# OpenRL-Lab/openrl

Hardware: AMD Instinct MI355X
Metric: env-steps/sec (collect+PPO update), 4096-env CartPole-shape (higher is better)
Workload: dtype f32

## Files before the change

include/orl_hip.h:

```cpp
#ifndef ORL_HIP_H
#define ORL_HIP_H

#include <stdint.h>

#ifdef __cplusplus
extern "C" {
#endif

#define ORL_VERSION 306

#define ORL_E_INVALID (-1)
#define ORL_E_UNSUPPORTED (-2)

#define ORL_HEAD_VALUE 0
#define ORL_HEAD_CATEGORICAL 1
#define ORL_HEAD_GAUSSIAN 2

typedef struct orl_net_desc {
  int32_t obs_dim;
  int32_t hidden;
  int32_t n_out;
  int32_t head_kind;
} orl_net_desc;

// ... 50 lines not shown
                          const uint8_t* bad_transition, const float* next_action_masks, float* h_policy_next,
                          float* h_critic_next, int hidden, void* stream);

#define ORL_COPY_MAX 8
typedef struct orl_copy_desc {
  const float* src[ORL_COPY_MAX];
  float* dst[ORL_COPY_MAX];
  int64_t n[ORL_COPY_MAX];
  int32_t count;
} orl_copy_desc;
int orl_multi_copy(const orl_copy_desc* desc, void* stream);

#define ORL_GATHER_MAX 12
typedef struct orl_gather_desc {
  const float* src[ORL_GATHER_MAX];
  float* dst[ORL_GATHER_MAX];
  int32_t width[ORL_GATHER_MAX];
  int32_t count;
} orl_gather_desc;
int orl_gather_minibatch(const orl_gather_desc* desc, const int64_t* idx, int n_rows, void* stream);

int orl_perm_feistel(int64_t* idx, int64_t n, uint64_t seed, uint64_t stream_id, void* stream);
int orl_perm_feistel_vn(int64_t* idx, int64_t n, uint64_t seed, uint64_t stream_id, float* vn_state,
                        const double* moments, double beta, void* stream);

int orl_act_step(const orl_net_desc* pnet, const float* ptheta, const orl_net_desc* cnet,
                 const float* ctheta, const float* policy_obs, const float* critic_obs,
                 const float* action_masks, int B, int deterministic, uint64_t seed, uint64_t row0,
                 uint64_t rng_step, const uint64_t* rng_step_dev, const float* forced_u, float* values,
                 float* actions, float* logp, void* stream);
int orl_act_step_grouped(const orl_net_desc* pnet, const float* pthetas, int64_t theta_stride, int rows_per_group,
                         const float* policy_obs, const float* action_masks, int B, int deterministic, uint64_t seed,
                         uint64_t row0, uint64_t rng_step, const uint64_t* rng_step_dev, float* actions, float* logp,
                         void* stream);

int orl_act_step_pool(const orl_net_desc* pnet, const float* pthetas, int64_t theta_stride, int n_policies,
                      const int32_t* opp_index, const float* policy_obs, const float* action_masks, int B,
                      int deterministic, uint64_t seed, uint64_t row0, uint64_t rng_step, const uint64_t* rng_step_dev,
                      float* actions, float* logp, void* stream);
int orl_opponent_sample(int32_t* opp_index, const uint8_t* dones, int N, int n_filled, int last_slot, int strategy,
                        int per_tile, uint64_t seed, uint64_t draw_id, const uint64_t* draw_id_dev, void* stream);


int orl_evaluate_actions(const orl_net_desc* pnet, const float* ptheta, const orl_net_desc* cnet,
                         const float* ctheta, const float* policy_obs, const float* critic_obs,
                         const float* actions, const float* action_masks, const float* active_masks, int B,
                         float* values, float* action_log_probs, float* entropy_rows, float* dist_entropy,
                         void* stream);

typedef struct orl_ppo_hparams {
  float clip_param;
  float entropy_coef;
  float value_loss_coef;
  float huber_delta;
  float dual_clip_coeff;
  float max_grad_norm;
  int32_t use_clipped_value_loss;
  int32_t use_huber_loss;
  int32_t use_value_active_masks;
  int32_t use_policy_active_masks;
  int32_t use_valuenorm;
  int32_t dual_clip_ppo;
  int32_t use_max_grad_norm;
  int32_t reserved;
} orl_ppo_hparams;

int orl_raw_grad_count(const orl_net_desc* net);
#define ORL_N_STATS 16
int orl_ppo_max_blocks(void);

int orl_ppo_fwd_bwd(const orl_net_desc* pnet, const float* ptheta, const orl_net_desc* cnet,
                    const float* ctheta, const float* records, int rec_width, const int64_t* idx,
                    int mb, const float* vn_state, const orl_ppo_hparams* hp, float* partials,
                    int* n_blocks_out, void* stream);

typedef struct orl_adam_state {
  float* theta;
  float* grad;
  float* m;
  float* v;
  float lr, eps, weight_decay;
  int32_t step;
} orl_adam_state;

int orl_ppo_reduce(const float* partials, int n_blocks, int width, float* sums, void* stream);
int orl_ppo_reduce_pair(const float* partials, int n_blocks_policy, int width_policy, int n_blocks_critic,
                        int width_critic, float* sums, void* stream);
int orl_ppo_apply(const orl_net_desc* pnet, const orl_net_desc* cnet, const float* sums,
                  const orl_ppo_hparams* hp, const orl_adam_state* padam, const orl_adam_state* cadam,
                  float* train_info_accum, void* stream);
int orl_ppo_apply_perm(const orl_net_desc* pnet, const orl_net_desc* cnet, const float* sums,
                       const orl_ppo_hparams* hp, const orl_adam_state* padam, const orl_adam_state* cadam,
                       float* train_info_accum, int64_t* next_idx, int64_t n, uint64_t seed, uint64_t stream_id,
                       float* vn_state, const double* moments, double beta, void* stream);

typedef struct orl_comm orl_comm;
#define ORL_IPC_HANDLE_BYTES 64
int orl_comm_create(int rank, int world, int64_t capacity_floats, orl_comm** comm_out, unsigned char* handle_out);
int orl_comm_connect(orl_comm* comm, const unsigned char* all_handles);
int orl_comm_destroy(orl_comm* comm);
int orl_comm_error(orl_comm* comm, void* stream);
int orl_comm_error_copy(orl_comm* comm, int* err_out_dev, void* stream);
int orl_allreduce_small(orl_comm* comm, float* data, int n, void* stream);
int orl_ppo_reduce_pair_comm(orl_comm* comm, const float* partials, int n_blocks_policy, int width_policy,
                             int n_blocks_critic, int width_critic, float* sums, void* stream);
int orl_ppo_apply_comm(orl_comm* comm, const orl_net_desc* pnet, const orl_net_desc* cnet, float* sums,
                       const orl_ppo_hparams* hp, const orl_adam_state* padam, const orl_adam_state* cadam,
                       float* train_info_accum, int64_t* next_idx, int64_t n, uint64_t seed, uint64_t stream_id,
                       float* vn_state, const double* moments, double beta, void* stream);

int orl_ppo_reduce_apply(orl_comm* comm, const float* partials, int n_blocks_policy, int width_policy,
                         int n_blocks_critic, int width_critic, float* sums, const orl_net_desc* pnet,
                         const orl_net_desc* cnet, const orl_ppo_hparams* hp, const orl_adam_state* padam,
                         const orl_adam_state* cadam, float* train_info_accum, int64_t* next_idx, int64_t n, uint64_t seed,
                         uint64_t stream_id, float* vn_state, const double* moments, double beta, uint32_t* sync_ctr,
                         void* stream);

int orl_ppo_step(orl_comm* comm, const float* partials, int n_blocks_policy, int width_policy, int n_blocks_critic,
                 int width_critic, float* sums, const orl_net_desc* pnet, const orl_net_desc* cnet,
                 const orl_ppo_hparams* hp, const orl_adam_state* padam, const orl_adam_state* cadam,
                 float* train_info_accum, int64_t* next_idx, int64_t n, uint64_t seed, uint64_t stream_id, float* vn_state,
                 const double* moments, double beta, uint32_t* sync_ctr, void* stream);

int orl_valuenorm_update(float* vn_state, const double* moments, double beta, void* stream);
int orl_minibatch_moments(const float* records, int rec_width, int ret_col, const int64_t* idx, int mb,
                          double* scratch, double* moments, void* stream);

#define ORL_ENV_SYNTH 0
#define ORL_ENV_CARTPOLE 1
#define ORL_ENV_TTT 2
#define ORL_ENV_TTT_POOL 3
#define ORL_ENV_PENDULUM 5
#define ORL_ENV_ACROBOT 6
#define ORL_ENV_MOUNTAINCAR 7
#define ORL_ENV_MOUNTAINCAR_CONT 8

typedef struct orl_rollout_args {
  orl_buffer_ptrs buf;
  float* value_preds;
  float* actions;
  float* action_log_probs;
  float* env_state;
  float* ep_stats;
  int32_t env_kind;
  int32_t episode_limit;
  uint64_t env_seed;
  uint64_t act_seed;
  uint64_t rng_step0;
  const float* opp_thetas;
  int64_t opp_theta_stride;
  int32_t opp_group_rows;
  int32_t opp_reserved;
  uint64_t opp_seed;
  uint64_t opp_rng_step0;
  const int32_t* opp_index;
  int32_t opp_per_reset;
  int32_t opp_n_policies;
  int32_t opp_n_filled;
  int32_t opp_last_slot;
  int32_t opp_strategy;
  int32_t opp_pad;
  uint64_t opp_sample_seed;
  uint64_t opp_draw_id0;
} orl_rollout_args;

int orl_build_experiments(void);
// ... 221 lines not shown
```

openrl_amd/_native.py:

```python
from __future__ import annotations

import ctypes as C
import os
from typing import Optional

import torch

_HERE = os.path.dirname(os.path.abspath(__file__))
LIB_PATH = os.path.join(_HERE, "csrc", "liborl_hip.so")

ORL_HEAD_VALUE, ORL_HEAD_CATEGORICAL, ORL_HEAD_GAUSSIAN = 0, 1, 2
ORL_ENV_SYNTH, ORL_ENV_CARTPOLE, ORL_ENV_TTT, ORL_ENV_TTT_POOL, ORL_ENV_MPE_SPREAD = 0, 1, 2, 3, 4
ORL_ENV_PENDULUM = 5
ORL_ENV_ACROBOT, ORL_ENV_MOUNTAINCAR = 6, 7
ORL_ENV_MOUNTAINCAR_CONT = 8
ORL_GATHER_MAX = 12
ORL_IPC_HANDLE_BYTES = 64
ORL_VERSION = 306
ORL_N_STATS = 16

c_f32p = C.c_void_p


class NativeError(RuntimeError):
    pass


class NetDesc(C.Structure):
    _fields_ = [("obs_dim", C.c_int32), ("hidden", C.c_int32), ("n_out", C.c_int32), ("head_kind", C.c_int32)]


class PackSrc(C.Structure):
    _fields_ = [("policy_obs", C.c_void_p), ("critic_obs", C.c_void_p), ("actions", C.c_void_p),
                ("action_log_probs", C.c_void_p), ("value_preds", C.c_void_p), ("returns", C.c_void_p),
                ("active_masks", C.c_void_p), ("action_masks", C.c_void_p),
                ("Dp", C.c_int32), ("Dc", C.c_int32), ("a", C.c_int32), ("K", C.c_int32)]


class BufferPtrs(C.Structure):
    _fields_ = [("policy_obs", C.c_void_p), ("critic_obs", C.c_void_p), ("rewards", C.c_void_p),
                ("masks", C.c_void_p), ("bad_masks", C.c_void_p), ("active_masks", C.c_void_p),
                ("action_masks", C.c_void_p),
                ("T", C.c_int32), ("N", C.c_int32), ("A", C.c_int32), ("Dp", C.c_int32), ("Dc", C.c_int32),
                ("K", C.c_int32)]


class CopyDesc(C.Structure):
    _fields_ = [("src", C.c_void_p * 8), ("dst", C.c_void_p * 8), ("n", C.c_int64 * 8), ("count", C.c_int32)]


class GatherDesc(C.Structure):
    _fields_ = [("src", C.c_void_p * ORL_GATHER_MAX), ("dst", C.c_void_p * ORL_GATHER_MAX),
                ("width", C.c_int32 * ORL_GATHER_MAX), ("count", C.c_int32)]


class PPOHParams(C.Structure):
    _fields_ = [("clip_param", C.c_float), ("entropy_coef", C.c_float), ("value_loss_coef", C.c_float),
                ("huber_delta", C.c_float), ("dual_clip_coeff", C.c_float), ("max_grad_norm", C.c_float),
                ("use_clipped_value_loss", C.c_int32), ("use_huber_loss", C.c_int32),
                ("use_value_active_masks", C.c_int32), ("use_policy_active_masks", C.c_int32),
                ("use_valuenorm", C.c_int32), ("dual_clip_ppo", C.c_int32), ("use_max_grad_norm", C.c_int32),
                ("reserved", C.c_int32)]


class AdamState(C.Structure):
    _fields_ = [("theta", C.c_void_p), ("grad", C.c_void_p), ("m", C.c_void_p), ("v", C.c_void_p),
                ("lr", C.c_float), ("eps", C.c_float), ("weight_decay", C.c_float), ("step", C.c_int32)]


class RolloutArgs(C.Structure):
    _fields_ = [("buf", BufferPtrs), ("value_preds", C.c_void_p), ("actions", C.c_void_p),
                ("action_log_probs", C.c_void_p), ("env_state", C.c_void_p), ("ep_stats", C.c_void_p),
                ("env_kind", C.c_int32), ("episode_limit", C.c_int32), ("env_seed", C.c_uint64),
                ("act_seed", C.c_uint64), ("rng_step0", C.c_uint64), ("opp_thetas", C.c_void_p),
                ("opp_theta_stride", C.c_int64), ("opp_group_rows", C.c_int32), ("opp_reserved", C.c_int32),
                ("opp_seed", C.c_uint64), ("opp_rng_step0", C.c_uint64), ("opp_index", C.c_void_p),
                ("opp_per_reset", C.c_int32), ("opp_n_policies", C.c_int32), ("opp_n_filled", C.c_int32),
                ("opp_last_slot", C.c_int32), ("opp_strategy", C.c_int32), ("opp_pad", C.c_int32),
                ("opp_sample_seed", C.c_uint64), ("opp_draw_id0", C.c_uint64)]


class RnnBatch(C.Structure):
    _fields_ = [("records", C.c_void_p), ("rows", C.c_void_p), ("masks", C.c_void_p), ("h_policy", C.c_void_p),
                ("h_critic", C.c_void_p), ("rec_width", C.c_int32), ("n_chunks", C.c_int32), ("L", C.c_int32),
                ("n_chunks_critic", C.c_int32), ("rows_critic", C.c_void_p)]


class RnnRolloutArgs(C.Structure):
    _fields_ = [("buf", BufferPtrs), ("value_preds", C.c_void_p), ("actions", C.c_void_p),
                ("action_log_probs", C.c_void_p), ("rnn_states", C.c_void_p), ("rnn_states_critic", C.c_void_p),
                ("env_state", C.c_void_p), ("ep_stats", C.c_void_p), ("obs_policy_out", C.c_void_p),
                ("obs_critic_out", C.c_void_p), ("next_value", C.c_void_p), ("env_kind", C.c_int32),
                ("world_length", C.c_int32), ("deterministic", C.c_int32), ("reserved", C.c_int32),
                ("env_seed", C.c_uint64), ("act_seed", C.c_uint64), ("rng_step0", C.c_uint64),
                ("rng_step_dev", C.c_void_p), ("sync_flags", C.c_void_p), ("env_step0", C.c_uint64)]


class HeadDesc(C.Structure):
    _fields_ = [("kind", C.c_int32), ("n_out", C.c_int32), ("n_heads", C.c_int32), ("nvec", C.c_int32 * 8)]


ORL_GEN_MLP_MAX_LAYERS = 14


class GenMlpLayer(C.Structure):
    _fields_ = [("W", C.c_void_p), ("bias", C.c_void_p), ("gamma", C.c_void_p), ("beta", C.c_void_p),
                ("n_in", C.c_int32), ("n_out", C.c_int32), ("act", C.c_int32), ("reserved", C.c_int32)]


class GenMlpDesc(C.Structure):
    _fields_ = [("n_layers", C.c_int32), ("n_heads", C.c_int32), ("fn_gamma", C.c_void_p), ("fn_beta", C.c_void_p),
                ("layer", GenMlpLayer * ORL_GEN_MLP_MAX_LAYERS)]


ORL_GT_MAX_LAYERS = 4


class GtDesc(C.Structure):
    _fields_ = [("theta", C.c_void_p), ("D", C.c_int32), ("H", C.c_int32), ("n_layers", C.c_int32), ("n_heads", C.c_int32),
                ("o_fn_g", C.c_int32), ("o_fn_be", C.c_int32),
                ("oW", C.c_int32 * ORL_GT_MAX_LAYERS), ("ob", C.c_int32 * ORL_GT_MAX_LAYERS),
                ("og", C.c_int32 * ORL_GT_MAX_LAYERS), ("obe", C.c_int32 * ORL_GT_MAX_LAYERS),
                ("act", C.c_int32 * ORL_GT_MAX_LAYERS),
                ("head_oW", C.c_int32 * 2), ("head_ob", C.c_int32 * 2), ("head_n", C.c_int32 * 2)]


class GtLoss(C.Structure):
    _fields_ = [("head", HeadDesc), ("logstd", C.c_void_p), ("den", C.c_void_p), ("vn_state", C.c_void_p),
                ("hp", PPOHParams), ("Dp", C.c_int32), ("Dc", C.c_int32), ("a_w", C.c_int32), ("K", C.c_int32),
                ("policy_head", C.c_int32), ("value_head", C.c_int32), ("policy_grad", C.c_int32), ("reserved", C.c_int32)]


ORL_ACT_NONE, ORL_ACT_TANH, ORL_ACT_RELU, ORL_ACT_LEAKY_RELU, ORL_ACT_ELU = -1, 0, 1, 2, 3
ORL_HEAD_MULTI_DISCRETE = 3
ORL_HEAD_MIXED = 4

_ABI_STRUCTS = (NetDesc, PackSrc, BufferPtrs, CopyDesc, GatherDesc, PPOHParams, AdamState, RolloutArgs, RnnBatch,
                RnnRolloutArgs, GenMlpDesc, GtDesc, GtLoss)

_P = C.c_void_p
_SIGNATURES = {
    "orl_version": (C.c_int, []),
    "orl_build_experiments": (C.c_int, []),
    "orl_tower_split_terms": (C.c_int, []),
    "orl_abi_struct_size": (C.c_int, [C.c_int]),
    "orl_last_error_string": (C.c_char_p, []),
    "orl_param_count": (C.c_int, [C.POINTER(NetDesc)]),
    "orl_raw_grad_count": (C.c_int, [C.POINTER(NetDesc)]),
    "orl_gae_scan": (C.c_int, [_P, _P, _P, _P, _P, _P, _P, C.c_int, C.c_int, C.c_double, C.c_double, C.c_int,
                               _P, _P, _P, C.POINTER(C.c_int), _P]),
    "orl_gae_max_partials": (C.c_int, [C.c_int, C.c_int]),
    "orl_adv_stats": (C.c_int, [_P, _P, _P, _P, C.c_int, C.c_int, _P, _P, C.POINTER(C.c_int), _P]),
    "orl_record_width": (C.c_int, [C.c_int, C.c_int, C.c_int, C.c_int]),
    "orl_adv_normalize_pack": (C.c_int, [_P, _P, C.c_int, C.c_int, C.c_int, C.c_int, _P, C.POINTER(PackSrc), _P, _P]),
    "orl_buffer_insert": (C.c_int, [C.POINTER(BufferPtrs), C.c_int, _P, _P, _P, _P, _P, _P, _P]),
    "orl_buffer_insert_rnn": (C.c_int, [C.POINTER(BufferPtrs), C.c_int, _P, _P, _P, _P, _P, _P, _P, _P, C.c_int, _P]),
    "orl_multi_copy": (C.c_int, [C.POINTER(CopyDesc), _P]),
    "orl_gather_minibatch": (C.c_int, [C.POINTER(GatherDesc), _P, C.c_int, _P]),
    "orl_perm_feistel": (C.c_int, [_P, C.c_int64, C.c_uint64, C.c_uint64, _P]),
    "orl_perm_feistel_vn": (C.c_int, [_P, C.c_int64, C.c_uint64, C.c_uint64, _P, _P, C.c_double, _P]),
    "orl_act_step": (C.c_int, [C.POINTER(NetDesc), _P, C.POINTER(NetDesc), _P, _P, _P, _P, C.c_int, C.c_int,
                               C.c_uint64, C.c_uint64, C.c_uint64, _P, _P, _P, _P, _P, _P]),
    "orl_ttt_state_width": (C.c_int, []),
    "orl_ttt_reset": (C.c_int, [_P, _P, _P, _P, C.c_int, C.c_uint64, _P]),
    "orl_ttt_step": (C.c_int, [_P, _P, _P, _P, _P, _P, _P, C.c_int, C.c_uint64, _P]),
    "orl_ttt_agent_move": (C.c_int, [_P, _P, _P, _P, _P, _P, C.c_int, _P]),
    "orl_ttt_opponent_move": (C.c_int, [_P, _P, _P, _P, _P, _P, _P, C.c_int, C.c_uint64, _P]),
    "orl_critic_values": (C.c_int, [C.POINTER(NetDesc), _P, _P, C.c_int64, _P, _P]),
    "orl_act_step_grouped": (C.c_int, [C.POINTER(NetDesc), _P, C.c_int64, C.c_int, _P, _P, C.c_int, C.c_int, C.c_uint64,
                                       C.c_uint64, C.c_uint64, _P, _P, _P, _P]),
    "orl_act_step_pool": (C.c_int, [C.POINTER(NetDesc), _P, C.c_int64, C.c_int, _P, _P, _P, C.c_int, C.c_int, C.c_uint64,
                                    C.c_uint64, C.c_uint64, _P, _P, _P, _P]),
    "orl_opponent_sample": (C.c_int, [_P, _P, C.c_int, C.c_int, C.c_int, C.c_int, C.c_int, C.c_uint64, C.c_uint64, _P,
                                      _P]),
    "orl_evaluate_actions": (C.c_int, [C.POINTER(NetDesc), _P, C.POINTER(NetDesc), _P, _P, _P, _P, _P, _P, C.c_int, _P,
                                       _P, _P, _P, _P]),
    "orl_ppo_max_blocks": (C.c_int, []),
    "orl_ppo_fwd_bwd": (C.c_int, [C.POINTER(NetDesc), _P, C.POINTER(NetDesc), _P, _P, C.c_int, _P, C.c_int, _P,
                                  C.POINTER(PPOHParams), _P, C.POINTER(C.c_int), _P]),
    "orl_ppo_reduce": (C.c_int, [_P, C.c_int, C.c_int, _P, _P]),
    "orl_ppo_reduce_pair": (C.c_int, [_P, C.c_int, C.c_int, C.c_int, C.c_int, _P, _P]),
    "orl_ppo_apply": (C.c_int, [C.POINTER(NetDesc), C.POINTER(NetDesc), _P, C.POINTER(PPOHParams),
                                C.POINTER(AdamState), C.POINTER(AdamState), _P, _P]),
    "orl_ppo_apply_perm": (C.c_int, [C.POINTER(NetDesc), C.POINTER(NetDesc), _P, C.POINTER(PPOHParams),
                                     C.POINTER(AdamState), C.POINTER(AdamState), _P, _P, C.c_int64, C.c_uint64,
                                     C.c_uint64, _P, _P, C.c_double, _P]),
    "orl_comm_create": (C.c_int, [C.c_int, C.c_int, C.c_int64, C.POINTER(_P), _P]),
    "orl_comm_connect": (C.c_int, [_P, _P]),
    "orl_comm_destroy": (C.c_int, [_P]),
    "orl_comm_error": (C.c_int, [_P, _P]),
    "orl_comm_error_copy": (C.c_int, [_P, _P, _P]),
    "orl_allreduce_small": (C.c_int, [_P, _P, C.c_int, _P]),
    "orl_ppo_reduce_pair_comm": (C.c_int, [_P, _P, C.c_int, C.c_int, C.c_int, C.c_int, _P, _P]),
    "orl_ppo_apply_comm": (C.c_int, [_P, C.POINTER(NetDesc), C.POINTER(NetDesc), _P, C.POINTER(PPOHParams),
                                     C.POINTER(AdamState), C.POINTER(AdamState), _P, _P, C.c_int64, C.c_uint64,
                                     C.c_uint64, _P, _P, C.c_double, _P]),
    "orl_ppo_reduce_apply": (C.c_int, [_P, _P, C.c_int, C.c_int, C.c_int, C.c_int, _P, C.POINTER(NetDesc),
                                       C.POINTER(NetDesc), C.POINTER(PPOHParams), C.POINTER(AdamState),
                                       C.POINTER(AdamState), _P, _P, C.c_int64, C.c_uint64, C.c_uint64, _P, _P, C.c_double,
                                       _P, _P]),
    "orl_ppo_step": (C.c_int, [_P, _P, C.c_int, C.c_int, C.c_int, C.c_int, _P, C.POINTER(NetDesc),
                               C.POINTER(NetDesc), C.POINTER(PPOHParams), C.POINTER(AdamState),
                               C.POINTER(AdamState), _P, _P, C.c_int64, C.c_uint64, C.c_uint64, _P, _P, C.c_double,
                               _P, _P]),
    "orl_gen_rollout_fused": (C.c_int, [_P, _P, _P, _P, _P, _P, _P, _P, _P, C.c_int, C.c_int, C.c_uint64, C.c_uint64,
                                        C.c_uint64, C.c_uint64, C.c_int, _P]),
    "orl_gemm": (C.c_int, [_P, C.c_int64, C.c_int64, _P, C.c_int64, C.c_int64, _P, C.c_int64, C.c_int, C.c_int, C.c_int,
                           C.c_int, _P, _P]),
    "orl_row_fwd": (C.c_int, [_P, _P, C.c_int, _P, _P, C.c_int, C.c_int, _P, _P, _P, _P, _P]),
    "orl_row_bwd": (C.c_int, [_P, _P, _P, _P, _P, C.c_int, C.c_int, C.c_int, _P, _P, C.c_int, C.POINTER(C.c_int), _P]),
    "orl_gen_layer_fwd": (C.c_int, [_P, C.c_int, C.c_int, _P, _P, C.c_int, _P, _P, C.c_int, _P, _P, _P, _P]),
    "orl_gt_supported": (C.c_int, [C.POINTER(GtDesc)]),
    "orl_gt_image_floats": (C.c_int64, [C.POINTER(GtDesc)]),
    "orl_gt_raw_floats": (C.c_int64, [C.POINTER(GtDesc)]),
    "orl_gt_prep": (C.c_int, [C.POINTER(GtDesc), _P, _P]),
    "orl_gt_fwd": (C.c_int, [C.POINTER(GtDesc), _P, _P, C.c_int, C.c_int, _P, C.c_int, _P, _P, _P]),
    "orl_gt_bwd": (C.c_int, [C.POINTER(GtDesc), _P, _P, C.c_int, C.c_int, _P, C.c_int, _P, _P, _P, C.c_int64, _P, _P, _P]),
    "orl_gt_train": (C.c_int, [C.POINTER(GtDesc), _P, _P, C.c_int, C.c_int, _P, C.c_int, C.POINTER(GtLoss), _P, C.c_int64, _P, _P,
                               _P, _P]),
    "orl_gen_mlp_fwd": (C.c_int, [C.POINTER(GenMlpDesc), _P, C.c_int, _P, _P, _P, _P]),
    "orl_gen_act": (C.c_int, [C.POINTER(GenMlpDesc), _P, C.POINTER(GenMlpDesc), _P, C.c_int, _P, _P, C.POINTER(HeadDesc), _P,
                              _P, C.c_int, C.c_uint64, C.c_uint64, C.c_uint64, _P, _P, C.c_int, _P, _P, _P]),
    "orl_gen_layer_bwd": (C.c_int, [_P, _P, _P, _P, C.c_int, C.c_int, C.c_int, _P, C.c_int, _P, _P, _P, C.c_int,
                                    C.POINTER(C.c_int), _P]),
    "orl_gen_wgrad": (C.c_int, [_P, _P, C.c_int, C.c_int, C.c_int, _P, _P, C.c_int64, _P]),
    "orl_gen_colsum": (C.c_int, [_P, C.c_int, C.c_int, _P, C.c_int, _P, C.c_int, _P, C.c_int, _P]),
    "orl_gather_cols": (C.c_int, [_P, C.c_int, C.c_int, C.c_int, _P, C.c_int, _P, _P]),
    "orl_gen_denoms": (C.c_int, [_P, C.c_int, C.c_int, C.c_int, C.c_int, _P, C.c_int, _P, _P, _P]),
    "orl_gen_policy_loss": (C.c_int, [C.POINTER(HeadDesc), _P, _P, _P, C.c_int, C.c_int, C.c_int, C.c_int, C.c_int, _P,
                                      C.c_int, _P, C.POINTER(PPOHParams), _P, _P, C.c_int, C.POINTER(C.c_int), _P, _P,
                                      _P]),
    "orl_gen_value_loss": (C.c_int, [_P, _P, C.c_int, C.c_int, C.c_int, C.c_int, C.c_int, _P, C.c_int, _P, _P,
                                     C.POINTER(PPOHParams), _P, _P, C.c_int, C.POINTER(C.c_int), _P]),
    "orl_gen_sample": (C.c_int, [C.POINTER(HeadDesc), _P, _P, _P, C.c_int, C.c_int, C.c_uint64, C.c_uint64, C.c_uint64,
                                 _P, _P, C.c_int, _P, _P, _P]),
    "orl_gen_adam": (C.c_int, [C.POINTER(AdamState), C.c_int64, C.c_float, C.c_int, C.c_int, _P, _P, C.c_int, C.c_int,
                               _P]),
    "orl_gen_matmul": (C.c_int, [_P, C.c_int, C.c_int, _P, C.c_int, _P, _P]),
    "orl_gen_colsum_rows": (C.c_int, [_P, C.c_int, C.c_int, _P, _P, C.c_int64, _P]),
    "orl_gen_gru_gate_fwd": (C.c_int, [_P, _P, _P, _P, C.c_int, C.c_int, _P, _P, _P, _P]),
    "orl_gen_gru_gate_bwd": (C.c_int, [_P, _P, _P, C.c_int, C.c_int, _P, _P, _P, _P]),
    "orl_gen_lstm_gate_fwd": (C.c_int, [_P, _P, _P, _P, C.c_int, C.c_int, _P, _P, _P, _P, _P, _P]),
    "orl_gen_lstm_gate_bwd": (C.c_int, [_P, _P, _P, _P, C.c_int, C.c_int, _P, _P, _P]),
    "orl_gen_row_affine": (C.c_int, [_P, _P, _P, _P, C.c_int, C.c_int, _P, _P]),
    "orl_vec_add": (C.c_int, [_P, _P, C.c_int64, _P]),
    "orl_gen_info": (C.c_int, [_P, _P, _P, C.POINTER(PPOHParams), C.c_float, C.c_float, _P, _P]),
    "orl_valuenorm_update": (C.c_int, [_P, _P, C.c_double, _P]),
    "orl_minibatch_moments": (C.c_int, [_P, C.c_int, C.c_int, _P, C.c_int, _P, _P, _P]),
    "orl_env_state_width": (C.c_int, [C.c_int]),
    "orl_env_reset": (C.c_int, [C.c_int, _P, _P, _P, C.c_int, C.c_int, C.c_uint64, C.c_int, _P]),
    "orl_env_step": (C.c_int, [C.c_int, _P, _P, _P, C.c_int, _P, _P, _P, C.c_int, C.c_int, C.c_uint64, C.c_int,
                               C.c_uint64, _P]),
    "orl_env_step_dev": (C.c_int, [C.c_int, _P, _P, _P, C.c_int, _P, _P, _P, C.c_int, C.c_int, C.c_uint64, C.c_int,
                                   C.c_uint64, _P, _P]),
    "orl_rollout_fused": (C.c_int, [C.POINTER(NetDesc), _P, C.POINTER(NetDesc), _P, C.POINTER(RolloutArgs), _P, _P]),
    "orl_mpe_state_width": (C.c_int, []),
    "orl_mpe_reset": (C.c_int, [_P, _P, _P, _P, C.c_int, C.c_uint64, _P]),
    "orl_mpe_step": (C.c_int, [_P, _P, _P, _P, _P, _P, _P, C.c_int, C.c_uint64, C.c_int, _P]),
    "orl_rnn_param_count": (C.c_int, [C.POINTER(NetDesc)]),
    "orl_rnn_raw_grad_count": (C.c_int, [C.POINTER(NetDesc)]),
    "orl_rnn_act_step": (C.c_int, [C.POINTER(NetDesc), _P, C.POINTER(NetDesc), _P, _P, _P, _P, _P, _P, _P, C.c_int,
                                   C.c_int, C.c_uint64, C.c_uint64, C.c_uint64, _P, _P, _P, _P, _P, _P, _P, _P]),
    "orl_rnn_eval_step": (C.c_int, [C.POINTER(NetDesc), _P, C.POINTER(NetDesc), _P, _P, _P, _P, _P, _P, _P, _P, C.c_int, _P,
                                    _P, _P, _P, _P, _P]),
    "orl_rnn_rollout_fused": (C.c_int, [C.POINTER(NetDesc), _P, C.POINTER(NetDesc), _P, C.POINTER(RnnRolloutArgs), _P]),
    "orl_rnn_chunk_rows": (C.c_int, [_P, C.c_int, C.c_int, C.c_int, C.c_int, _P, _P]),
    "orl_rnn_chunk_rows_v3": (C.c_int, [_P, C.c_int, C.c_int, C.c_int, C.c_int, C.c_int, C.c_int, _P, _P]),
    "orl_rnn_jrpo_records": (C.c_int, [_P, _P, C.c_int, C.c_int, C.c_int, C.c_int, _P, C.c_int, C.c_int, C.c_int, _P, _P]),
    "orl_rnn_workspace_floats": (C.c_int64, [C.POINTER(NetDesc), C.POINTER(NetDesc), C.c_int, C.c_int]),
# ... 117 lines not shown
```

openrl_amd/algorithms/ppo.py:

```python
from __future__ import annotations

from typing import Dict, Union

import numpy as np
import torch

from .. import _native as nat
from .. import distributed as dist_utils
from .. import ops, ops_rnn
from .base_algorithm import BaseAlgorithm

INFO_KEYS = ("value_loss", "policy_loss", "dist_entropy", "actor_grad_norm", "critic_grad_norm", "ratio")


class DeviceTrainInfo(dict):

    def __init__(self, keys, device_values: torch.Tensor, after_sync=None, scale=None):
        super().__init__()
        self._keys, self._dev, self._after_sync, self._scale = tuple(keys), device_values, after_sync, scale

    def _materialize(self) -> None:
        if self._dev is not None:
            raw, self._dev = self._dev.cpu().numpy(), None
            if self._scale is not None:
# ... 11 lines not shown

    def __iter__(self):
        self._materialize()
        return super().__iter__()

    def __len__(self):
        self._materialize()
        return super().__len__()

    def __contains__(self, k):
        self._materialize()
        return super().__contains__(k)

    def __repr__(self):
        self._materialize()
        return super().__repr__()

    def __eq__(self, other):
        self._materialize()
        return super().__eq__(other)

    def get(self, k, default=None):
        self._materialize()
        return super().get(k, default)

    def keys(self):
        self._materialize()
        return super().keys()

    def values(self):
        self._materialize()
        return super().values()

    def items(self):
        self._materialize()
        return super().items()

    def copy(self):
        self._materialize()
        return dict(self)

    def pop(self, *a):
        self._materialize()
        return super().pop(*a)

    def update(self, *a, **k):
        self._materialize()
        return super().update(*a, **k)

    def __setitem__(self, k, v):
        self._materialize()
        super().__setitem__(k, v)

    def __delitem__(self, k):
        self._materialize()
        super().__delitem__(k)


class PPOAlgorithm(BaseAlgorithm):
    info_keys = INFO_KEYS

    def __init__(self, cfg, init_module, agent_num: int = 1, device: Union[str, torch.device] = "cuda:0") -> None:
        if cfg.use_deepspeed or cfg.use_amp:
            raise NotImplementedError("deepspeed / amp are not built in this engine")
        if cfg.use_joint_action_loss and not cfg.use_recurrent_policy:
            raise NotImplementedError("use_joint_action_loss is built for recurrent policies (recurrent_generator_v3, "
                                      "the only generator the reference pairs it with, ppo.py:363-372)")
        super().__init__(cfg, init_module, agent_num, device)
        self.naive_recurrent = bool(cfg.use_naive_recurrent_policy) and not bool(cfg.use_recurrent_policy)
        self.train_list = [self.train_ppo]
        self.hp = ops.make_hparams(cfg, recurrent=bool(getattr(self.algo_module, "recurrent", False)))
        self.generic = bool(getattr(self.algo_module, "generic", False))
        self.use_joint_action_loss = bool(cfg.use_joint_action_loss)
        self.perm_mode = getattr(cfg, "amd_perm_mode", "reference")
        self._perm_counter = 0
        self._vn_in_perm = False
        self.last_indices = None
        self._info = torch.zeros(8, dtype=torch.float32, device=self.device)
        self._moments = torch.zeros(3, dtype=torch.float64, device=self.device)
        self._mom_scratch = torch.zeros(512, dtype=torch.float64, device=self.device)
        self._adv_stats = torch.zeros(11, dtype=torch.float64, device=self.device)
        self._moments_mb = self._moments
        self._full_batch_moments = False
        if self.generic:
            self.recurrent = bool(getattr(self.algo_module, "recurrent", False))
            self._rnn_rows = None
            self.fuse_next_perm = False
            self._comm = None
            self._gen_den4 = torch.zeros(4, dtype=torch.float32, device=self.device)
            self._gen_den = self._gen_den4[:2]
            self._gen_den_c = self._gen_den4[2:]
            self._gen_den_scratch = torch.zeros(257, dtype=torch.float32, device=self.device)
            self._gen_scratch = torch.zeros(256, dtype=torch.float32, device=self.device)
            self._gen_flat = self._gen_sums = None
            self._gen_den_stamp = None
            self._comm_watch = None
            if self.world_size > 1:
                nets = [m for m in self.algo_module.models.values()]
                n = sum(int(m.n_params) for m in nets) + 40
                self._gen_flat = torch.zeros(n, dtype=torch.float32, device=self.device)
                o = 0
                for m in nets:
                    m.grad = self._gen_flat[o:o + int(m.n_params)]
                    o += int(m.n_params)
                self._gen_sums = (self._gen_flat[o:o + 20], self._gen_flat[o + 20:o + 40])
                self._comm = dist_utils.make_small_allreduce(n, self.device, getattr(cfg, "amd_collective", "p2p")) \
                    if n <= self.P2P_MAX_FLOATS else None
                if self._comm is not None:
                    self._comm_watch = nat.DeviceErrorWatch("orl_comm: a peer's contribution did not arrive within 10 s - "
                                                            "the optimiser step ran on a partial gradient sum")
            return
        p, c = self.algo_module.models["policy"], self.algo_module.models["critic"]
        self.recurrent = bool(getattr(self.algo_module, "recurrent", False))
        raw = ops_rnn.rnn_raw_grad_count if self.recurrent else ops.raw_grad_count
        self._raw_p = raw(p.net) + ops.N_STATS
        self._raw_c = raw(c.net) + ops.N_STATS
        mb = ops.ppo_max_blocks()
        dev = self.device
        self._partials = None if self.recurrent else torch.empty(mb * (self._raw_p + self._raw_c), dtype=torch.float32,
                                                                 device=dev)
        self._rnn_ws = None
        self._rnn_rows = None
        self._rnn_scratch = torch.zeros(512, dtype=torch.float32, device=dev) if self.recurrent else None
        self._sums = torch.zeros(self._raw_p + self._raw_c, dtype=torch.float32, device=dev)
        self._optim_step = str(getattr(cfg, "amd_optim_step", "two_launch"))
        self._fused_step = self._optim_step in ("fused", "step")
        self._sync_ctr = torch.zeros(4, dtype=torch.int32, device=dev)
        self._comm = dist_utils.make_small_allreduce(self._sums.numel(), dev, getattr(cfg, "amd_collective", "p2p")) \
            if self.world_size > 1 else None
        self.fuse_next_perm = True
        self._comm_watch = nat.DeviceErrorWatch("orl_comm: a peer's contribution did not arrive within 10 s - the "
                                                "optimiser step ran on a partial gradient sum") \
            if self._comm is not None else None

    P2P_MAX_FLOATS = 1 << 16

    def _allreduce_vec(self, t: torch.Tensor) -> torch.Tensor:
        if self.world_size > 1:
            if self._comm is not None and t.dtype == torch.float32 and t.numel() <= self._comm.capacity:
                self._comm.allreduce_(t)
            else:
                dist_utils.allreduce_(t)
        return t

    def _advantages_and_records(self, buffer) -> None:
        T, N, A = buffer.episode_length, buffer.n_rollout_threads, buffer.num_agents
        L = N * A
        vn = self.algo_module.get_critic_value_normalizer() if (self._use_popart or self._use_valuenorm) else None
        vn_state = vn.state if vn is not None else None
        if not (buffer._adv_fresh and (getattr(buffer, "_adv_vn", None) is vn_state)):
            buffer.n_partials = ops.adv_stats(buffer.returns, buffer.value_preds, buffer.active_masks, vn_state, T, L,
                                              buffer.advantages, buffer.stat_partials)
        partials, n_part = buffer.stat_partials, buffer.n_partials
        if self.world_size > 1:
            row = dist_utils.allreduce_stat_rows(partials[:n_part])
            partials, n_part = row, 1
        ops.adv_normalize_pack(buffer.advantages, partials, n_part, T, L, self._use_adv_normalize, self._adv_stats,
                               buffer.pack_src(), buffer.ensure_records())
        buffer._adv_fresh = False

    def _update_minibatch(self, buffer, idx, mb: int, turn_on: bool, next_perm=None):
        if self.generic:
            from .ppo_generic import update_minibatch_generic

            return update_minibatch_generic(self, buffer, idx, mb, turn_on)
        mod = self.algo_module
        p, c = mod.models["policy"], mod.models["critic"]
        po, co = mod.optimizers["policy"], mod.optimizers["critic"]
        rec = buffer.records
        vn = mod.get_critic_value_normalizer() if self._use_valuenorm else None
        vn_state = None
        if vn is not None:
            if self._full_batch_moments:
                pass
            else:
                ret_col = buffer.Dp + buffer.Dc + 2 * buffer.act_shape + 2
                ops.minibatch_moments(rec, ret_col, idx, mb, self._mom_scratch, self._moments)
                if self.world_size > 1:
                    dist_utils.allreduce_(self._moments)
            if self._vn_in_perm:
                self._vn_in_perm = False
            else:
                ops.valuenorm_update(vn.state, self._moments, vn.beta)
            vn_state = vn.state
        ev = getattr(self, "profile_events", None)
        if ev is not None:
            e0, e1 = torch.cuda.Event(enable_timing=True), torch.cuda.Event(enable_timing=True)
            e0.record()
        nb_p, nb_c = ops.ppo_fwd_bwd(p.net, p.theta, c.net, c.theta, rec, idx, mb, vn_state, self.hp, self._partials)
        if ev is not None:
            e1.record()
            ev.append((e0, e1))
        comm = self._comm
        fused = self._fused_step and (self.world_size == 1 or comm is not None)
        if not fused:
            ops.ppo_reduce_pair(self._partials, nb_p, self._raw_p, nb_c, self._raw_c, self._sums, comm=comm)
            if self.world_size > 1 and comm is None:
                dist_utils.allreduce_(self._sums)
        po.step_count += 1 if turn_on else 0
        co.step_count += 1
        hp = self.hp
        first = getattr(self, "_info_first", False)
        if not turn_on or first:
            hp = nat.PPOHParams.from_buffer_copy(self.hp)
            if not turn_on:
                hp.reserved |= 1
            if first:
                hp.reserved |= 32
                self._info_first = False
        if fused:
            return ops.ppo_reduce_apply(self._partials, nb_p, self._raw_p, nb_c, self._raw_c, self._sums, p.net, c.net, hp,
                                        po.native_state(max(po.step_count, 1)), co.native_state(co.step_count),
                                        self._info, self._sync_ctr, next_perm, comm=comm,
                                        entry="orl_ppo_reduce_apply" if self._optim_step == "fused" else "orl_ppo_step")
        return ops.ppo_apply(p.net, c.net, self._sums, hp, po.native_state(max(po.step_count, 1)),
                             co.native_state(co.step_count), self._info, next_perm, comm=comm)

    def _update_minibatch_jrpo(self, buffer, chunks, n_chunks: int, turn_on: bool) -> None:
        if self.generic:
            return self._update_minibatch_jrpo_generic(buffer, chunks, n_chunks, turn_on)
        mod = self.algo_module
        p, c = mod.models["policy"], mod.models["critic"]
        po, co = mod.optimizers["policy"], mod.optimizers["critic"]
        T, N, A, L = buffer.episode_length, buffer.n_rollout_threads, buffer.num_agents, self.data_chunk_length
        lanes, H = N * A, p.net.hidden
        rec = buffer.records
        Dp, Dc, a_w, K = buffer.Dp, buffer.Dc, buffer.act_shape, buffer.K
        ns = n_chunks * A
        dev = self.device
        if getattr(self, "_jr", None) is None or self._jr["ns"] < ns or self._jr["L"] != L:
            f = lambda *sh: torch.empty(*sh, dtype=torch.float32, device=dev)
            self._jr = dict(ns=ns, L=L, rows_p=torch.empty(L * ns, dtype=torch.int64, device=dev),
                            rows_c=torch.empty(L * n_chunks, dtype=torch.int64, device=dev), x=f(ns, Dp), act=f(ns, a_w),
                            mk=f(ns), am=f(ns, K) if K else None, h=f(ns, H), logp=f(L * ns, a_w), rec2=torch.empty_like(rec))
        j = self._jr
        rows_p, rows_c = j["rows_p"][:L * ns], j["rows_c"][:L * n_chunks]
        ops_rnn.rnn_chunk_rows_v3(chunks, n_chunks, L, T, N, A, False, rows_p)
        ops_rnn.rnn_chunk_rows_v3(chunks, n_chunks, L, T, N, A, True, rows_c)
        vn = mod.get_critic_value_normalizer() if self._use_valuenorm else None
        vn_state = None
        if vn is not None:
            ret_col = Dp + Dc + 2 * a_w + 2
            ops.minibatch_moments(rec, ret_col, rows_c, n_chunks * L, self._mom_scratch, self._moments_mb)
            if self.world_size > 1:
                dist_utils.allreduce_(self._moments_mb)
            ops.valuenorm_update(vn.state, self._moments_mb, vn.beta)
            self._vn_in_perm = False
            vn_state = vn.state
        from .. import ops_gen

        x, act, mk, am, h = j["x"][:ns], j["act"][:ns], j["mk"][:ns], (j["am"][:ns] if K else None), j["h"][:ns]
        o_act = Dp + Dc
        masks_flat = buffer.masks.view(-1, 1)
        hflat = buffer.rnn_states.view(-1, H)
        ops_gen.gather_cols(hflat, 0, H, rows_p[:ns], ns, h)
        for s in range(L):
            r = rows_p[s * ns:(s + 1) * ns]
            ops_gen.gather_cols(rec, 0, Dp, r, ns, x)
            ops_gen.gather_cols(rec, o_act, a_w, r, ns, act)
            ops_gen.gather_cols(masks_flat, 0, 1, r, ns, mk.view(ns, 1))
            if K:
                ops_gen.gather_cols(rec, o_act + 2 * a_w + 4, K, r, ns, am)
            ops_rnn.rnn_eval_step(p.net, p.theta, None, None, x, None, h, None, mk, am, act, ns, None,
                                  j["logp"][s * ns:(s + 1) * ns], None, h, None)
        rec2 = j["rec2"]
        if self._jr.get("stamp") is not buffer.records or self._jr.get("fresh") != self._jrpo_epoch_id:
            rec2.copy_(rec)
            self._jr["stamp"], self._jr["fresh"] = buffer.records, self._jrpo_epoch_id
        ops_rnn.rnn_jrpo_records(rec, rec2, Dp, Dc, a_w, rows_p, n_chunks, L, A, j["logp"])
        need = ops_rnn.rnn_workspace_floats(p.net, c.net, ns, L)
        if self._rnn_ws is None or self._rnn_ws.numel() < need:
            self._rnn_ws = torch.empty(need, dtype=torch.float32, device=dev)
        ops_rnn.rnn_ppo_fwd_bwd(p.net, p.theta, c.net, c.theta, rec2, rows_p, buffer.masks, buffer.rnn_states,
                                buffer.rnn_states_critic, ns, L, vn_state, self.hp, self._rnn_ws, self._sums,
                                rows_critic=rows_c, n_chunks_critic=n_chunks)
        if self.world_size > 1:
            if self._comm is not None:
                self._comm.allreduce_(self._sums)
            else:
                dist_utils.allreduce_(self._sums)
        po.step_count += 1 if turn_on else 0
        co.step_count += 1
        hp = self.hp
        if not turn_on:
            hp = nat.PPOHParams.from_buffer_copy(self.hp)
            hp.reserved |= 1
        ops_rnn.rnn_ppo_apply(p.net, c.net, self._sums, hp, po.native_state(max(po.step_count, 1)),
                              co.native_state(co.step_count), self._info, self._rnn_scratch)

    def _update_minibatch_jrpo_generic(self, buffer, chunks, n_chunks: int, turn_on: bool) -> None:
        from .. import ops_gen
        from .ppo_generic import update_minibatch_generic
# ... 72 lines not shown
                ops.minibatch_moments(rec, ret_col, rows, n_chunks * L, self._mom_scratch, self._moments)
                if self.world_size > 1:
                    dist_utils.allreduce_(self._moments)
            if self._vn_in_perm:
                self._vn_in_perm = False
            else:
                ops.valuenorm_update(vn.state, self._moments, vn.beta)
            vn_state = vn.state
        need = ops_rnn.rnn_workspace_floats(p.net, c.net, n_chunks, L)
        if self._rnn_ws is None or self._rnn_ws.numel() < need:
            self._rnn_ws = torch.empty(need, dtype=torch.float32, device=self.device)
        ev = getattr(self, "profile_events", None)
        if ev is not None:
            e0, e1 = torch.cuda.Event(enable_timing=True), torch.cuda.Event(enable_timing=True)
            e0.record()
        ops_rnn.rnn_ppo_fwd_bwd(p.net, p.theta, c.net, c.theta, rec, rows, buffer.masks, buffer.rnn_states,
                                buffer.rnn_states_critic, n_chunks, L, vn_state, self.hp, self._rnn_ws, self._sums)
        if ev is not None:
            e1.record()
            ev.append((e0, e1))
        if self.world_size > 1:
            if self._comm is not None:
                self._comm.allreduce_(self._sums)
            else:
                dist_utils.allreduce_(self._sums)
        po.step_count += 1 if turn_on else 0
        co.step_count += 1
        hp = self.hp
        if not turn_on:
            hp = nat.PPOHParams.from_buffer_copy(self.hp)
            hp.reserved |= 1
        ops_rnn.rnn_ppo_apply(p.net, c.net, self._sums, hp, po.native_state(max(po.step_count, 1)),
                              co.native_state(co.step_count), self._info, self._rnn_scratch)

    def _chunk_batches(self, M: int):
        L = self.data_chunk_length
        if self.use_joint_action_loss:
            M = M // self.agent_num
        assert M >= L, "PPO requires n_rollout_threads * num_agents * episode_length >= data_chunk_length"
        data_chunks = M // L
        mbs = data_chunks // self.num_mini_batch
        if self.perm_mode == "device":
            n, seed, sid, vn = self._perm_job(data_chunks)
            self._vn_in_perm = vn is not None
            rand = ops.perm_feistel(n, seed, sid, self.device, vn)
        elif self.perm_mode == "identity":
            rand = torch.arange(data_chunks, dtype=torch.int64, device=self.device)
        else:
            rand = torch.randperm(data_chunks).to(self.device, non_blocking=True)
        return [rand[i * mbs:(i + 1) * mbs] for i in range(self.num_mini_batch)], mbs

    def _perm_job(self, M: int):
        self._perm_counter += 1
        vn = None
        if self._full_batch_moments and self._use_valuenorm:
            v = self.algo_module.get_critic_value_normalizer()
            vn = (v.state, self._moments, v.beta)
        return M, int(self.cfg.seed), self._perm_counter, vn

    def _minibatch_indices(self, M: int, perm=None):
        mbs = M // self.num_mini_batch
        n_batches = M // mbs
        if self.perm_mode == "identity":
            if self.num_mini_batch == 1:
                return [None], mbs
            order = torch.arange(M, dtype=torch.int64, device=self.device)
            return [order[b * mbs:(b + 1) * mbs] for b in range(n_batches)], mbs
        if perm is not None:
            self._vn_in_perm = self._full_batch_moments and self._use_valuenorm
        elif self.perm_mode == "device":
            n, seed, sid, vn = self._perm_job(M)
            self._vn_in_perm = vn is not None
            perm = ops.perm_feistel(n, seed, sid, self.device, vn)
        else:
            perm = torch.randperm(M).to(self.device, non_blocking=True)
        return [perm[b * mbs:(b + 1) * mbs] for b in range(n_batches)], mbs

    def train_ppo(self, buffer, turn_on: bool = True) -> Dict[str, float]:
        if self.naive_recurrent:
            self.data_chunk_length = buffer.episode_length
        if getattr(self, "_comm_watch", None) is not None:
            self._comm_watch.poll()
        self._advantages_and_records(buffer)
        M = buffer.episode_length * buffer.n_rollout_threads * buffer.num_agents
        self._full_batch_moments = self.num_mini_batch == 1 and (not self.recurrent or M % self.data_chunk_length == 0)
        self._moments = self._adv_stats[8:11] if self._full_batch_moments else self._moments_mb
        self._info = torch.empty(8, dtype=torch.float32, device=self.device)
        num_updates = self.ppo_epoch * self.num_mini_batch
        if num_updates <= 0:
            raise ValueError("train_ppo: ppo_epoch * num_mini_batch must be positive (got %d x %d)"
                             % (self.ppo_epoch, self.num_mini_batch))
        self._info_first = not (self.generic or self.recurrent)
        if not self._info_first:
            self._info.zero_()
        self.last_indices = []
        next_perm = None
        self._jrpo_epoch_id = getattr(self, "_jrpo_epoch_id", 0) + 1
        if self.use_joint_action_loss:
            self._full_batch_moments = False
            self._moments = self._moments_mb
        for epoch in range(self.ppo_epoch):
            if self.recurrent:
                batches, mbs = self._chunk_batches(M)
                for chunks in batches:
                    self.last_indices.append(chunks)
                    self._update_minibatch_rnn(buffer, chunks, mbs, turn_on)
                continue
            batches, mbs = self._minibatch_indices(M, next_perm)
            next_perm = None
            for k, idx in enumerate(batches):
                self.last_indices.append(idx)
                job = None
                if (self.fuse_next_perm and k == len(batches) - 1 and epoch + 1 < self.ppo_epoch
                        and self.perm_mode == "device"):
                    job = self._perm_job(M)
                next_perm = self._update_minibatch(buffer, idx, mbs, turn_on, job)
        self._info_first = False
        keys = self.info_keys
        scale = np.full(len(keys), np.float32(1.0) / np.float32(num_updates), dtype=np.float32)
        if self.use_joint_action_loss:
            scale[1] /= np.float32(buffer.num_agents * buffer.act_shape)
        watch = getattr(self, "_comm_watch", None)
        if watch is None:
            return DeviceTrainInfo(keys, self._info[:len(keys)], scale=scale)
        watch.post(self._comm.error_flag())
        return DeviceTrainInfo(keys, self._info[:len(keys)], after_sync=lambda: watch.poll(wait=True), scale=scale)

    def train(self, buffer, turn_on: bool = True) -> Dict[str, float]:
        if len(self.train_list) == 1:
            return self.train_list[0](buffer, turn_on)
        train_info = {}
        for train_func in self.train_list:
            train_info.update(train_func(buffer, turn_on))
        return train_info
```

openrl_amd/configs/config.py:

```python
from __future__ import annotations

import argparse
from typing import Any, List, Optional

from ._flag_table import FLAGS

AMD_FLAGS = [
    ("amd_perm_mode", "str", "reference", "opt", ["reference", "device", "identity"]),
    ("amd_rollout_mode", "str", "auto", "opt", ["auto", "fused", "stepwise"]),
    ("amd_rollout_kernel", "str", "chain", "opt", ["chain", "lockstep"]),
    ("amd_use_graph", "bool", True, "opt", None),
    ("amd_collective", "str", "p2p", "opt", ["p2p", "rccl"]),
    ("amd_rnn_rollout_chase", "bool", True, "opt", None),
    ("amd_tower_gemm", "str", "split", "opt", ["split", "fp32", "split_two_image"]),
    ("amd_rnn_gemm", "str", "fp32", "opt", ["fp32", "fp32_recompute", "split", "split_w4"]),
    ("amd_optim_step", "str", "two_launch", "opt", ["two_launch", "step", "fused"]),
    ("amd_gen_update", "str", "fused", "opt", ["fused", "layerwise"]),
]


def _str2bool(v: Any) -> bool:
    if isinstance(v, bool):
        return v
    s = str(v).strip().lower()
    if s in ("1", "true", "t", "yes", "y"):
        return True
    if s in ("0", "false", "f", "no", "n"):
        return False
    raise argparse.ArgumentTypeError("expected a boolean, got %r" % (v,))


def _identity(v):
    return v


_TYPES = {"int": int, "float": float, "str": str, "bool": _str2bool, "any": _identity}


class _YamlConfigAction(argparse.Action):

    def __call__(self, parser, namespace, values, option_string=None):
        import yaml

        with open(values, "r") as fh:
            text = fh.read()
        try:
            head = yaml.safe_load(text.split("\n\n")[0]) if text.lstrip().startswith("globals:") else None
        except Exception:
            head = None
        if isinstance(head, dict) and "globals" in head:
            import jinja2

            text = jinja2.Template(text).render(**head["globals"])
        data = yaml.safe_load(text) or {}
        data.pop("globals", None)
        types = {a.dest: a.type for a in parser._actions if a.type is not None}
        for k, v in _flatten(data).items():
            conv = types.get(k)
            if conv is not None and isinstance(v, (str, int, float, bool)) and v is not None:
                v = conv(v)
            setattr(namespace, k, v)
        setattr(namespace, self.dest, values)


def _flatten(d, prefix=""):
    out = {}
    for k, v in d.items():
        key = prefix + str(k)
        if isinstance(v, dict) and key in ("selfplay_api", "reward_class", "vec_info_class", "env"):
            out.update(_flatten(v, key + "."))
        else:
            out[key] = v
    return out


def create_config_parser() -> argparse.ArgumentParser:
    parser = argparse.ArgumentParser(description="openrl_amd", formatter_class=argparse.RawDescriptionHelpFormatter)
    parser.add_argument("--config", action=_YamlConfigAction, default=None)
    for name, tname, default, kind, choices in list(FLAGS) + AMD_FLAGS:
        if kind == "flag":
            parser.add_argument("--" + name, dest=name, action="store_false" if default is True else "store_true",
                                default=default)
        elif kind == "pos":
            parser.add_argument(name, type=_TYPES[tname], default=default, nargs="?")
        else:
            kw = dict(dest=name, type=_TYPES[tname], default=default)
            if choices:
                kw["choices"] = choices
            parser.add_argument("--" + name, **kw)
    return parser


def default_cfg(argv: Optional[List[str]] = None):
    return create_config_parser().parse_args(list(argv or []))
```

openrl_amd/csrc/orl_apply.hip:

```cpp
#include <stdlib.h>
#include <string.h>
#include "orl_common.h"
#include "orl_perm.h"
#include "orl_comm.h"
#include "orl_mlp.h"
#undef ORL_PROF
#include "orl_ppo_tower.h"

namespace orl {

__global__ __launch_bounds__(256) void ppo_reduce_kernel(const float* __restrict__ partials, int n_blocks, int width,
                                                         float* __restrict__ sums) {
  __shared__ float sh[4][64];
  const int col = blockIdx.x * 64 + (threadIdx.x & 63);
  const int rg = threadIdx.x >> 6;
  float s0 = 0.f, s1 = 0.f;
  if (col < width) {
    int b = rg;
    for (; b + 4 < n_blocks; b += 8) {
      s0 += partials[(size_t)b * width + col];
      s1 += partials[(size_t)(b + 4) * width + col];
    }
    if (b < n_blocks) s0 += partials[(size_t)b * width + col];
  }
  sh[rg][threadIdx.x & 63] = s0 + s1;
  __syncthreads();
  if (rg == 0 && col < width)
    sums[col] = (sh[0][threadIdx.x] + sh[1][threadIdx.x]) + (sh[2][threadIdx.x] + sh[3][threadIdx.x]);
}

struct ApplyTower {
  orl_net_desc net;
  orl_adam_state ad;
  int sums_off;
};

__device__ inline void stage_dma(float* lds_dst, const float* __restrict__ src, int n) {
  const int lane = threadIdx.x & 63;
#pragma unroll 1
  for (int e0 = (threadIdx.x & ~63); e0 < n; e0 += blockDim.x) {
    if (e0 + lane < n)
      __builtin_amdgcn_global_load_lds((const __attribute__((address_space(1))) void*)(src + e0 + lane),
                                       (__attribute__((address_space(3))) void*)(lds_dst + e0), 4, 0, 0);
  }
}

__device__ inline float block_sum_1024(float v, float* sh) {
  v = wave_sum_dpp(v);
  const int w = threadIdx.x >> 6;
  if ((threadIdx.x & 63) == 0) sh[w] = v;
  __syncthreads();
  float t = 0.f;
  for (int k = 0; k < 16; ++k) t += sh[k];
  __syncthreads();
  return t;
}

__device__ inline float raw_to_grad(const float* __restrict__ raw, const float* __restrict__ theta,
                                    const TowerLayout& tl, const RawLayout& rl, int p, float inv_den) {
  const int H = HID;
  float g;
  if (p < tl.ob1) g = raw[rl.odW1 + (p - tl.oW1)];
  else if (p < tl.og1) g = raw[rl.odb1 + (p - tl.ob1)];
  else if (p < tl.obe1) {
    const int i = p - tl.og1;
    g = 0.f;
#pragma unroll 8
    for (int o = 0; o < H; ++o) g += theta[tl.oW2 + o * H + i] * raw[rl.oG + o * H + i];
  } else if (p < tl.oW2) {
    const int i = p - tl.obe1;
    g = 0.f;
#pragma unroll 8
    for (int o = 0; o < H; ++o) g += theta[tl.oW2 + o * H + i] * raw[rl.odb2 + o];
  } else if (p < tl.ob2) {
    const int e = p - tl.oW2, o = e / H, i = e - o * H;
    g = theta[tl.og1 + i] * raw[rl.oG + e] + theta[tl.obe1 + i] * raw[rl.odb2 + o];
  } else if (p < tl.og2) g = raw[rl.odb2 + (p - tl.ob2)];
  else if (p < tl.obe2) {
    const int f = p - tl.og2;
    g = 0.f;
    for (int c = 0; c < tl.n_out; ++c) g += theta[tl.oW3 + c * H + f] * raw[rl.oS3 + c * H + f];
  } else if (p < tl.oW3) {
    const int f = p - tl.obe2;
    g = 0.f;
    for (int c = 0; c < tl.n_out; ++c) g += theta[tl.oW3 + c * H + f] * raw[rl.odb3 + c];
  } else if (p < tl.ob3) {
    const int e = p - tl.oW3, c = e / H, f = e - c * H;
    g = theta[tl.og2 + f] * raw[rl.oS3 + e] + theta[tl.obe2 + f] * raw[rl.odb3 + c];
  } else if (p < tl.ologstd) g = raw[rl.odb3 + (p - tl.ob3)];
  else g = raw[rl.odlogstd + (p - tl.ologstd)];
  return g * inv_den;
}

__device__ inline bool apply_tower_block(const int t, const ApplyTower& P, const ApplyTower& Cc, float* __restrict__ sums,
                                         const orl_ppo_hparams& hp, float* __restrict__ info, const int stage_mv,
                                         const CommDev& CM, const int use_comm, float* s_apply, float* sh,
                                         unsigned* __restrict__ wait_ctr = nullptr, const unsigned wait_target = 0u) {
  const TowerLayout tlp(P.net), tlc(Cc.net);
  const RawLayout rlp(P.net), rlc(Cc.net);
  float norms[2] = {0.f, 0.f};
  float* raw = s_apply;
  const float* st;
  float den_p = 1.f, den_v = 1.f;
  const bool policy_off = t == 0 && (hp.reserved & 1);
  bool params_staged = false;
  {
    const RawLayout& rl0 = t == 0 ? rlp : rlc;
    const int off = t == 0 ? P.sums_off : Cc.sums_off;
    const int nraw = rl0.total + ORL_N_STATS;
    if (wait_ctr != nullptr) {
      if (!policy_off) {
        const ApplyTower& W0 = t == 0 ? P : Cc;
        const TowerLayout& tl0 = t == 0 ? tlp : tlc;
        float* th0 = s_apply + rl0.total + ORL_N_STATS;
        stage_dma(th0, W0.ad.theta, tl0.total);
        if (stage_mv) {
          stage_dma(th0 + 2 * tl0.total, W0.ad.m, tl0.total);
          stage_dma(th0 + 3 * tl0.total, W0.ad.v, tl0.total);
        }
        params_staged = true;
      }
      __shared__ int s_wait_ok;
      if (threadIdx.x == 0) {
        int ok = 1;
        unsigned spins = 0;
        while (__hip_atomic_load(wait_ctr, __ATOMIC_RELAXED, __HIP_MEMORY_SCOPE_AGENT) < wait_target) {
          __builtin_amdgcn_s_sleep(2);
          if (++spins > (1u << 22)) { ok = 0; break; }
        }
        s_wait_ok = ok;
        if (ok) __hip_atomic_store(wait_ctr, 0u, __ATOMIC_RELAXED, __HIP_MEMORY_SCOPE_AGENT);
      }
      __syncthreads();
      if (!s_wait_ok) {
        if (threadIdx.x == 0 && info != nullptr)
          for (int k = 0; k < 6; ++k) info[k] = __builtin_bit_cast(float, 0x7fc00000u);
        return false;
      }
#pragma unroll 1
      for (int e = threadIdx.x; e < nraw; e += blockDim.x) {
        float v = __hip_atomic_load(sums + off + e, __ATOMIC_RELAXED, __HIP_MEMORY_SCOPE_SYSTEM);
        if (use_comm) {
          v = comm_sum(CM, off + e, v);
          sums[off + e] = v;
        }
        raw[e] = v;
      }
    } else if (use_comm) {
#pragma unroll 1
      for (int e = threadIdx.x; e < nraw; e += blockDim.x) {
        const float v = comm_sum(CM, off + e, sums[off + e]);
        sums[off + e] = v;
        raw[e] = v;
      }
    } else {
      stage_dma(raw, sums + off, nraw);
    }
    st = raw + rl0.total;
  }
  {
    const ApplyTower& W = t == 0 ? P : Cc;
    const TowerLayout& tl = t == 0 ? tlp : tlc;
    const RawLayout& rl = t == 0 ? rlp : rlc;
    if (policy_off) {
      asm volatile("s_waitcnt vmcnt(0)" ::: "memory");
      __syncthreads();
      den_p = hp.use_policy_active_masks ? st[ST_ACTIVE_SUM] : st[ST_ROWS];
      const float* stp = st;
      for (int p = threadIdx.x; p < tl.total; p += blockDim.x) W.ad.grad[p] = 0.f;
      if (threadIdx.x == 0 && info != nullptr) {
        if (hp.reserved & 32) info[1] = info[2] = info[3] = info[5] = 0.f;
        info[1] += stp[ST_PLOSS_SUM] / den_p;
        float ent_den0 = den_p;
        if (!hp.use_policy_active_masks && P.net.head_kind == ORL_HEAD_GAUSSIAN) ent_den0 = den_p * (float)P.net.n_out;
        info[2] += stp[ST_ENT_SUM] / ent_den0;
        const float aw0 = P.net.head_kind == ORL_HEAD_GAUSSIAN ? (float)P.net.n_out : 1.f;
        info[5] += stp[ST_RATIO_SUM] / (stp[ST_ROWS] * aw0);
      }
      return true;
    }
    float* th_s = s_apply + rl.total + ORL_N_STATS;
    float* g_s = th_s + tl.total;
    float* m_s = g_s + tl.total;
    float* v_s = m_s + tl.total;
    if (!params_staged) {
      stage_dma(th_s, W.ad.theta, tl.total);
      if (stage_mv) {
        stage_dma(m_s, W.ad.m, tl.total);
        stage_dma(v_s, W.ad.v, tl.total);
      }
    }
    const double b1d = 0.9, b2d = 0.999;
    const float b2 = (float)b2d, omb1 = (float)(1.0 - b1d), omb2 = (float)(1.0 - b2d);
    const double bc1 = 1.0 - powi_d(b1d, (long long)W.ad.step);
    const double bc2 = 1.0 - powi_d(b2d, (long long)W.ad.step);
    const float step_size = (float)((double)W.ad.lr / bc1);
    const float bc2_sqrt = (float)sqrt(bc2);
    asm volatile("s_waitcnt vmcnt(0)" ::: "memory");
    __syncthreads();
    den_p = hp.use_policy_active_masks ? st[ST_ACTIVE_SUM] : st[ST_ROWS];
    den_v = hp.use_value_active_masks ? st[ST_ACTIVE_SUM] : st[ST_ROWS];
    const float inv_den = 1.0f / (t == 0 ? den_p : den_v);
    float ss = 0.f;
#pragma unroll 1
    for (int p = threadIdx.x; p < tl.total; p += blockDim.x) {
      const float g = raw_to_grad(raw, th_s, tl, rl, p, inv_den);
      g_s[p] = g;
      ss += g * g;
    }
    const float total = sqrtf(block_sum_1024(ss, sh));
    norms[t] = total;
    float coef = 1.f;
    if (hp.use_max_grad_norm) coef = fminf(hp.max_grad_norm / (total + 1e-6f), 1.f);
    auto adam = [&](int p, float m, float v) {
      float g = g_s[p] * coef;
      W.ad.grad[p] = g;
      float th = th_s[p];
      if (W.ad.weight_decay != 0.f) g += W.ad.weight_decay * th;
      m = m + (g - m) * omb1;
      v = v * b2 + omb2 * (g * g);
      const float denom = sqrtf(v) / bc2_sqrt + W.ad.eps;
      th = th - step_size * (m / denom);
      W.ad.m[p] = m; W.ad.v[p] = v; W.ad.theta[p] = th;
    };
    if (stage_mv) {
#pragma unroll 1
      for (int p = threadIdx.x; p < tl.total; p += blockDim.x) adam(p, m_s[p], v_s[p]);
    } else {
#pragma unroll 1
      for (int p = threadIdx.x; p < tl.total; p += blockDim.x) adam(p, W.ad.m[p], W.ad.v[p]);
    }
  }
  if (threadIdx.x == 0 && info != nullptr) {
    const float* stp = st;
    const float* stc = st;
    const bool first = (hp.reserved & 32) != 0;
    auto acc = [&](int k, float x) {
      if (first) info[k] = x;
      else unsafeAtomicAdd(info + k, x);
    };
    if (t == 0) {
      float ent_den = den_p;
      if (!hp.use_policy_active_masks && P.net.head_kind == ORL_HEAD_GAUSSIAN) ent_den = den_p * (float)P.net.n_out;
      acc(1, stp[ST_PLOSS_SUM] / den_p);
      acc(2, stp[ST_ENT_SUM] / ent_den);
      acc(3, norms[0]);
      const float a_w = P.net.head_kind == ORL_HEAD_GAUSSIAN ? (float)P.net.n_out : 1.f;
      acc(5, stp[ST_RATIO_SUM] / (stp[ST_ROWS] * a_w));
    } else {
      acc(0, stc[ST_VLOSS_SUM] / den_v);
      acc(4, norms[1]);
    }
  }
  return true;
}

__global__ __launch_bounds__(1024) void ppo_apply_kernel(ApplyTower P, ApplyTower Cc, float* __restrict__ sums,
                                                         orl_ppo_hparams hp, float* __restrict__ info, PermJob J,
                                                         int stage_mv, CommDev CM, int use_comm) {
  extern __shared__ __attribute__((aligned(16))) float s_apply[];
  if (blockIdx.x >= 2) {
    perm_job_block(J, (int)blockIdx.x - 2, (int)gridDim.x - 2);
    return;
  }
  __shared__ float sh[16];
  apply_tower_block((int)blockIdx.x, P, Cc, sums, hp, info, stage_mv, CM, use_comm, s_apply, sh);
}

template <bool PUBLISH = false>
__device__ inline void reduce_columns_block(const float* __restrict__ partials, int n_blocks, int width, int col0,
                                            float* __restrict__ out, int comm_off, const CommDev& CM, int use_comm,
                                            float (*sh)[64]) {
  const int lc = threadIdx.x & 63;
  const int col = col0 + lc;
  const int rg = threadIdx.x >> 6;
  float s0 = 0.f, s1 = 0.f, s2 = 0.f, s3 = 0.f;
  if (col < width) {
    if (n_blocks <= 256) {
      float v[16];
#pragma unroll
      for (int k = 0; k < 16; ++k) {
        const int b = rg + 16 * k;
        v[k] = b < n_blocks ? partials[(size_t)b * width + col] : 0.f;
      }
#pragma unroll
      for (int g = 0; g < 4; ++g) {
        if (rg + 64 * g + 48 < n_blocks) {
          s0 += v[4 * g]; s1 += v[4 * g + 1]; s2 += v[4 * g + 2]; s3 += v[4 * g + 3];
        } else {
#pragma unroll
          for (int k = 0; k < 4; ++k)
            if (rg + 64 * g + 16 * k < n_blocks) s0 += v[4 * g + k];
        }
      }
    } else {
      int b = rg;
      for (; b + 48 < n_blocks; b += 64) {
        s0 += partials[(size_t)b * width + col];
        s1 += partials[(size_t)(b + 16) * width + col];
        s2 += partials[(size_t)(b + 32) * width + col];
        s3 += partials[(size_t)(b + 48) * width + col];
      }
      for (; b < n_blocks; b += 16) s0 += partials[(size_t)b * width + col];
    }
  }
  sh[rg][lc] = (s0 + s1) + (s2 + s3);
  __syncthreads();
  if (rg == 0 && col < width) {
    float t[4];
#pragma unroll
    for (int k = 0; k < 4; ++k) t[k] = (sh[4 * k][lc] + sh[4 * k + 1][lc]) + (sh[4 * k + 2][lc] + sh[4 * k + 3][lc]);
    const float v = (t[0] + t[1]) + (t[2] + t[3]);
    if (PUBLISH) __hip_atomic_store(out + col, v, __ATOMIC_RELAXED, __HIP_MEMORY_SCOPE_SYSTEM);
    else out[col] = v;
    if (use_comm) {
      for (int p = 0; p < CM.world; ++p)
        if (p != CM.rank) comm_push(CM, p, comm_off + col, v);
    }
  }
}

#if ORL_BUILD_EXPERIMENTS
__global__ __launch_bounds__(1024) void ppo_reduce_apply_kernel(const float* __restrict__ pp, int nb_p, int wp, int gp,
                                                                const float* __restrict__ pc, int nb_c, int wc, int gc,
                                                                ApplyTower P, ApplyTower Cc, float* __restrict__ sums,
                                                                orl_ppo_hparams hp, float* __restrict__ info, PermJob J,
                                                                int stage_mv, CommDev CM, int use_comm,
                                                                unsigned* __restrict__ ctr) {
  extern __shared__ __attribute__((aligned(16))) float s_apply[];
  __shared__ float sh[16];
  __shared__ unsigned s_ticket;
  const int b = blockIdx.x;
  if (b < gp + gc) {
    const bool pol = b < gp;
    reduce_columns_block(pol ? pp : pc, pol ? nb_p : nb_c, pol ? wp : wc, (pol ? b : b - gp) * 64, pol ? sums : sums + wp,
                         pol ? 0 : wp, CM, use_comm, (float(*)[64])s_apply);
    if (threadIdx.x < 64) {
      __builtin_amdgcn_fence(__ATOMIC_RELEASE, "agent");
      if (threadIdx.x == 0) s_ticket = atomicAdd(ctr + (pol ? 0 : 1), 1u);
    }
    __syncthreads();
    if (s_ticket == (unsigned)((pol ? gp : gc) - 1)) {
      if (threadIdx.x == 0) ctr[pol ? 0 : 1] = 0u;
      __builtin_amdgcn_fence(__ATOMIC_ACQUIRE, "agent");
      apply_tower_block(pol ? 0 : 1, P, Cc, sums, hp, info, stage_mv, CM, use_comm, s_apply, sh);
      return;
    }
  }
  if (J.idx == nullptr) return;
  const unsigned shares = gridDim.x - 2u;
  __syncthreads();
  if (threadIdx.x == 0) s_ticket = atomicAdd(ctr + 2, 1u);
  __syncthreads();
  const unsigned k = s_ticket;
  if (k == shares - 1u && threadIdx.x == 0) ctr[2] = 0u;
  perm_job_block(J, (int)k, (int)shares);
}

#endif

__global__ __launch_bounds__(1024) void ppo_step_kernel(const float* __restrict__ pp, int nb_p, int wp, int gp,
                                                        const float* __restrict__ pc, int nb_c, int wc, int gc, ApplyTower P,
                                                        ApplyTower Cc, float* __restrict__ sums, orl_ppo_hparams hp,
                                                        float* __restrict__ info, PermJob J, int stage_mv, CommDev CM,
                                                        int use_comm, unsigned* __restrict__ ctr) {
  extern __shared__ __attribute__((aligned(16))) float s_apply[];
  __shared__ float sh[16];
  const int b = blockIdx.x;
  if (b < gp + gc) {
    const bool pol = b < gp;
    reduce_columns_block<true>(pol ? pp : pc, pol ? nb_p : nb_c, pol ? wp : wc, (pol ? b : b - gp) * 64, pol ? sums : sums + wp,
                               pol ? 0 : wp, CM, use_comm, (float(*)[64])s_apply);
    if (threadIdx.x < 64) {
      asm volatile("s_waitcnt vmcnt(0)" ::: "memory");
      if (threadIdx.x == 0) __hip_atomic_fetch_add(ctr + (pol ? 0 : 1), 1u, __ATOMIC_RELAXED, __HIP_MEMORY_SCOPE_AGENT);
    }
    return;
  }
  if (b < gp + gc + 2) {
    const int t = b - gp - gc;
    apply_tower_block(t, P, Cc, sums, hp, info, stage_mv, CM, use_comm, s_apply, sh, ctr + t, (unsigned)(t == 0 ? gp : gc));
    return;
  }
  perm_job_block(J, b - (gp + gc + 2), (int)gridDim.x - (gp + gc + 2));
}

__global__ __launch_bounds__(1024) void ppo_reduce_pair_kernel(const float* __restrict__ pp, int nb_p, int wp, int gp,
                                                               const float* __restrict__ pc, int nb_c, int wc,
                                                               float* __restrict__ sums, CommDev CM, int use_comm) {
  __shared__ float sh[16][64];
  const bool pol = (int)blockIdx.x < gp;
  reduce_columns_block(pol ? pp : pc, pol ? nb_p : nb_c, pol ? wp : wc, (pol ? blockIdx.x : blockIdx.x - gp) * 64,
                       pol ? sums : sums + wp, pol ? 0 : wp, CM, use_comm, sh);
}

static int check_tower(const orl_net_desc* n, const char* who) {
  if (!n) return fail(ORL_E_INVALID, "%s: null net descriptor", who);
  if (n->hidden != HID) return fail(ORL_E_UNSUPPORTED, "%s: hidden_size %d not built (only 64)", who, n->hidden);
  if (n->obs_dim < 1 || n->obs_dim > 64) return fail(ORL_E_UNSUPPORTED, "%s: obs_dim %d outside [1,64]", who, n->obs_dim);
  if (n->n_out < 1 || n->n_out > 16) return fail(ORL_E_UNSUPPORTED, "%s: n_out %d outside [1,16]", who, n->n_out);
  return 0;
}


}

using namespace orl;

extern "C" {

int orl_ppo_reduce(const float* partials, int n_blocks, int width, float* sums, void* stream) {
  ORL_REQUIRE(partials && sums && n_blocks > 0 && width > 0, "orl_ppo_reduce: bad arguments");
  const int grid = (width + 63) / 64;
  hipLaunchKernelGGL(ppo_reduce_kernel, dim3(grid), dim3(256), 0, (hipStream_t)stream, partials, n_blocks, width, sums);
  return launch_status("orl_ppo_reduce");
}

static int launch_apply(const char* what, const orl_net_desc* pnet, const orl_net_desc* cnet, float* sums,
                        const orl_ppo_hparams* hp, const orl_adam_state* padam, const orl_adam_state* cadam,
                        float* train_info_accum, const PermJob& J, void* stream, orl_comm* comm = nullptr) {
  int rc = check_tower(pnet, what);
  if (rc) return rc;
  rc = check_tower(cnet, what);
  if (rc) return rc;
  ORL_REQUIRE(sums && hp && padam && cadam, "%s: null pointer", what);
  ORL_REQUIRE(padam->theta && padam->grad && padam->m && padam->v && cadam->theta && cadam->grad && cadam->m && cadam->v,
              "%s: null optimizer buffer", what);
  ORL_REQUIRE(padam->step >= 1 && cadam->step >= 1, "%s: Adam step counts are 1-based", what);
  ApplyTower P, Cc;
  P.net = *pnet; P.ad = *padam; P.sums_off = 0;
  Cc.net = *cnet; Cc.ad = *cadam; Cc.sums_off = RawLayout(*pnet).total + ORL_N_STATS;
  auto need = [&](int k) {
    const size_t lp = (size_t)(RawLayout(*pnet).total + ORL_N_STATS + k * TowerLayout(*pnet).total) * sizeof(float);
    const size_t lc = (size_t)(RawLayout(*cnet).total + ORL_N_STATS + k * TowerLayout(*cnet).total) * sizeof(float);
    return lp > lc ? lp : lc;
  };
  const int stage_mv = need(4) <= 160 * 1024;
  const size_t lds = need(stage_mv ? 4 : 2);
  ORL_REQUIRE(lds <= 160 * 1024, "%s: tower needs %zu B of LDS", what, lds);
  int perm_blocks = 0;
  if (J.idx != nullptr) {
    perm_blocks = (int)((J.n + 1023) / 1024);
    if (perm_blocks > 254) perm_blocks = 254;
  }
  CommDev CM;
  memset(&CM, 0, sizeof(CM));
  int use_comm = 0;
  if (comm != nullptr) {
    const int total = Cc.sums_off + RawLayout(*cnet).total + ORL_N_STATS;
    ORL_REQUIRE(total <= orl_comm_capacity(comm), "%s: the sums vector (%d floats) exceeds the comm's capacity %d", what,
                total, orl_comm_capacity(comm));
    rc = orl_comm_current(comm, &CM);
    if (rc) return rc;
    use_comm = CM.world > 1;
  }
  (void)hipFuncSetAttribute((const void*)ppo_apply_kernel, hipFuncAttributeMaxDynamicSharedMemorySize, (int)lds);
  hipLaunchKernelGGL(ppo_apply_kernel, dim3(2 + perm_blocks), dim3(1024), lds, (hipStream_t)stream, P, Cc, sums, *hp,
                     train_info_accum, J, stage_mv, CM, use_comm);
  return launch_status(what);
}

int orl_ppo_apply(const orl_net_desc* pnet, const orl_net_desc* cnet, const float* sums, const orl_ppo_hparams* hp,
                  const orl_adam_state* padam, const orl_adam_state* cadam, float* train_info_accum, void* stream) {
  PermJob J;
  memset(&J, 0, sizeof(J));
  return launch_apply("orl_ppo_apply", pnet, cnet, (float*)sums, hp, padam, cadam, train_info_accum, J, stream);
}

int orl_ppo_apply_comm(orl_comm* comm, const orl_net_desc* pnet, const orl_net_desc* cnet, float* sums,
                       const orl_ppo_hparams* hp, const orl_adam_state* padam, const orl_adam_state* cadam,
                       float* train_info_accum, int64_t* next_idx, int64_t n, uint64_t seed, uint64_t stream_id,
                       float* vn_state, const double* moments, double beta, void* stream) {
  ORL_REQUIRE(comm, "orl_ppo_apply_comm: null comm");
  PermJob J;
  memset(&J, 0, sizeof(J));
  if (next_idx != nullptr) {
    ORL_REQUIRE(n > 0 && n <= ((int64_t)1 << 62), "orl_ppo_apply_comm: bad permutation arguments");
    ORL_REQUIRE(!vn_state || moments, "orl_ppo_apply_comm: vn_state needs moments");
    J = make_perm_job(next_idx, n, seed, stream_id, vn_state, moments, beta);
  }
  return launch_apply("orl_ppo_apply_comm", pnet, cnet, sums, hp, padam, cadam, train_info_accum, J, stream, comm);
}

int orl_ppo_apply_perm(const orl_net_desc* pnet, const orl_net_desc* cnet, const float* sums, const orl_ppo_hparams* hp,
                       const orl_adam_state* padam, const orl_adam_state* cadam, float* train_info_accum,
                       int64_t* next_idx, int64_t n, uint64_t seed, uint64_t stream_id, float* vn_state,
                       const double* moments, double beta, void* stream) {
  ORL_REQUIRE(next_idx && n > 0 && n <= ((int64_t)1 << 62), "orl_ppo_apply_perm: bad permutation arguments");
  ORL_REQUIRE(!vn_state || moments, "orl_ppo_apply_perm: vn_state needs moments");
  const PermJob J = make_perm_job(next_idx, n, seed, stream_id, vn_state, moments, beta);
  return launch_apply("orl_ppo_apply_perm", pnet, cnet, (float*)sums, hp, padam, cadam, train_info_accum, J, stream);
}

int orl_ppo_reduce_apply(orl_comm* comm, const float* partials, int n_blocks_policy, int width_policy,
                         int n_blocks_critic, int width_critic, float* sums, const orl_net_desc* pnet,
                         const orl_net_desc* cnet, const orl_ppo_hparams* hp, const orl_adam_state* padam,
                         const orl_adam_state* cadam, float* train_info_accum, int64_t* next_idx, int64_t n, uint64_t seed,
                         uint64_t stream_id, float* vn_state, const double* moments, double beta, uint32_t* sync_ctr,
                         void* stream) {
  const char* what = "orl_ppo_reduce_apply";
#if !ORL_BUILD_EXPERIMENTS
  return fail(ORL_E_UNSUPPORTED, "%s: the ticketed one-launch optimiser step lost its A/B (15.7 us against 4.4 + 9.3 us for "
              "orl_ppo_reduce_pair + orl_ppo_apply) and is only present in an ORL_BUILD_EXPERIMENTS library", what);
#else
  int rc = check_tower(pnet, what);
  if (rc) return rc;
  rc = check_tower(cnet, what);
  if (rc) return rc;
  ORL_REQUIRE(partials && sums && hp && padam && cadam && sync_ctr, "%s: null pointer", what);
  ORL_REQUIRE(n_blocks_policy > 0 && n_blocks_critic > 0, "%s: bad arguments", what);
  ORL_REQUIRE(padam->theta && padam->grad && padam->m && padam->v && cadam->theta && cadam->grad && cadam->m && cadam->v,
              "%s: null optimizer buffer", what);
  ORL_REQUIRE(padam->step >= 1 && cadam->step >= 1, "%s: Adam step counts are 1-based", what);
  ApplyTower P, Cc;
  P.net = *pnet; P.ad = *padam; P.sums_off = 0;
  Cc.net = *cnet; Cc.ad = *cadam; Cc.sums_off = RawLayout(*pnet).total + ORL_N_STATS;
  ORL_REQUIRE(width_policy == Cc.sums_off && width_critic == RawLayout(*cnet).total + ORL_N_STATS,
              "%s: partial widths %d / %d do not match the towers' raw vectors (%d / %d)", what, width_policy, width_critic,
              Cc.sums_off, RawLayout(*cnet).total + ORL_N_STATS);
  PermJob J;
  memset(&J, 0, sizeof(J));
  if (next_idx != nullptr) {
    ORL_REQUIRE(n > 0 && n <= ((int64_t)1 << 62), "%s: bad permutation arguments", what);
    ORL_REQUIRE(!vn_state || moments, "%s: vn_state needs moments", what);
    J = make_perm_job(next_idx, n, seed, stream_id, vn_state, moments, beta);
  }
  auto need = [&](int k) {
    const size_t lp = (size_t)(RawLayout(*pnet).total + ORL_N_STATS + k * TowerLayout(*pnet).total) * sizeof(float);
    const size_t lc = (size_t)(RawLayout(*cnet).total + ORL_N_STATS + k * TowerLayout(*cnet).total) * sizeof(float);
    return lp > lc ? lp : lc;
  };
  const int stage_mv = need(4) <= 156 * 1024;
  const size_t lds = need(stage_mv ? 4 : 2);
  ORL_REQUIRE(lds <= 156 * 1024 && lds >= 16 * 64 * sizeof(float), "%s: tower needs %zu B of LDS", what, lds);
  const int gp = (width_policy + 63) / 64, gc = (width_critic + 63) / 64;
  int extra = 0;
  if (J.idx != nullptr) {
    extra = (int)((J.n + 1023) / 1024) - (gp + gc - 2);
    if (extra > 256 - gp - gc) extra = 256 - gp - gc;
    if (extra < (gp + gc == 2 ? 1 : 0)) extra = gp + gc == 2 ? 1 : 0;
  }
  CommDev CM;
  memset(&CM, 0, sizeof(CM));
  int use_comm = 0;
  if (comm != nullptr) {
    ORL_REQUIRE(width_policy + width_critic <= orl_comm_capacity(comm), "%s: %d floats exceed the comm's capacity %d", what,
                width_policy + width_critic, orl_comm_capacity(comm));
    rc = orl_comm_next(comm, &CM);
    if (rc) return rc;
    use_comm = CM.world > 1;
  }
  (void)hipFuncSetAttribute((const void*)ppo_reduce_apply_kernel, hipFuncAttributeMaxDynamicSharedMemorySize, (int)lds);
  hipLaunchKernelGGL(ppo_reduce_apply_kernel, dim3(gp + gc + extra), dim3(1024), lds, (hipStream_t)stream, partials,
                     n_blocks_policy, width_policy, gp, partials + (size_t)PPO_MAX_BLOCKS * width_policy, n_blocks_critic,
                     width_critic, gc, P, Cc, sums, *hp, train_info_accum, J, stage_mv, CM, use_comm, sync_ctr);
  return launch_status(what);
#endif
}

int orl_ppo_step(orl_comm* comm, const float* partials, int n_blocks_policy, int width_policy, int n_blocks_critic,
                 int width_critic, float* sums, const orl_net_desc* pnet, const orl_net_desc* cnet,
                 const orl_ppo_hparams* hp, const orl_adam_state* padam, const orl_adam_state* cadam,
                 float* train_info_accum, int64_t* next_idx, int64_t n, uint64_t seed, uint64_t stream_id, float* vn_state,
                 const double* moments, double beta, uint32_t* sync_ctr, void* stream) {
  const char* what = "orl_ppo_step";
  int rc = check_tower(pnet, what);
  if (rc) return rc;
  rc = check_tower(cnet, what);
  if (rc) return rc;
  ORL_REQUIRE(partials && sums && hp && padam && cadam && sync_ctr, "%s: null pointer", what);
  ORL_REQUIRE(n_blocks_policy > 0 && n_blocks_critic > 0, "%s: bad arguments", what);
  ORL_REQUIRE(padam->theta && padam->grad && padam->m && padam->v && cadam->theta && cadam->grad && cadam->m && cadam->v,
              "%s: null optimizer buffer", what);
  ORL_REQUIRE(padam->step >= 1 && cadam->step >= 1, "%s: Adam step counts are 1-based", what);
  ApplyTower P, Cc;
  P.net = *pnet; P.ad = *padam; P.sums_off = 0;
  Cc.net = *cnet; Cc.ad = *cadam; Cc.sums_off = RawLayout(*pnet).total + ORL_N_STATS;
  ORL_REQUIRE(width_policy == Cc.sums_off && width_critic == RawLayout(*cnet).total + ORL_N_STATS,
              "%s: partial widths %d / %d do not match the towers' raw vectors (%d / %d)", what, width_policy, width_critic,
              Cc.sums_off, RawLayout(*cnet).total + ORL_N_STATS);
  PermJob J;
  memset(&J, 0, sizeof(J));
  if (next_idx != nullptr) {
    ORL_REQUIRE(n > 0 && n <= ((int64_t)1 << 62), "%s: bad permutation arguments", what);
    ORL_REQUIRE(!vn_state || moments, "%s: vn_state needs moments", what);
    J = make_perm_job(next_idx, n, seed, stream_id, vn_state, moments, beta);
  }
  auto need = [&](int k) {
    const size_t lp = (size_t)(RawLayout(*pnet).total + ORL_N_STATS + k * TowerLayout(*pnet).total) * sizeof(float);
    const size_t lc = (size_t)(RawLayout(*cnet).total + ORL_N_STATS + k * TowerLayout(*cnet).total) * sizeof(float);
    return lp > lc ? lp : lc;
  };
  const int stage_mv = need(4) <= 160 * 1024;
  const size_t lds = need(stage_mv ? 4 : 2);
  ORL_REQUIRE(lds <= 160 * 1024 && lds >= 16 * 64 * sizeof(float), "%s: tower needs %zu B of LDS", what, lds);
  const int gp = (width_policy + 63) / 64, gc = (width_critic + 63) / 64;
  int perm_blocks = 0;
  if (J.idx != nullptr) {
    perm_blocks = (int)((J.n + 1023) / 1024);
    const int room = 254 - (gp + gc) > 8 ? 254 - (gp + gc) : 8;
    if (perm_blocks > room) perm_blocks = room;
  }
  CommDev CM;
  memset(&CM, 0, sizeof(CM));
  int use_comm = 0;
  if (comm != nullptr) {
    ORL_REQUIRE(width_policy + width_critic <= orl_comm_capacity(comm), "%s: %d floats exceed the comm's capacity %d", what,
                width_policy + width_critic, orl_comm_capacity(comm));
    rc = orl_comm_next(comm, &CM);
    if (rc) return rc;
    use_comm = CM.world > 1;
  }
  (void)hipFuncSetAttribute((const void*)ppo_step_kernel, hipFuncAttributeMaxDynamicSharedMemorySize, (int)lds);
  hipLaunchKernelGGL(ppo_step_kernel, dim3(gp + gc + 2 + perm_blocks), dim3(1024), lds, (hipStream_t)stream, partials,
                     n_blocks_policy, width_policy, gp, partials + (size_t)PPO_MAX_BLOCKS * width_policy, n_blocks_critic,
                     width_critic, gc, P, Cc, sums, *hp, train_info_accum, J, stage_mv, CM, use_comm, sync_ctr);
  return launch_status(what);
}

static int launch_reduce_pair(const char* what, orl_comm* comm, const float* partials, int n_blocks_policy,
                              int width_policy, int n_blocks_critic, int width_critic, float* sums, void* stream) {
  ORL_REQUIRE(partials && sums && n_blocks_policy > 0 && n_blocks_critic > 0 && width_policy > 0 && width_critic > 0,
              "%s: bad arguments", what);
  CommDev CM;
  memset(&CM, 0, sizeof(CM));
  int use_comm = 0;
  if (comm != nullptr) {
    ORL_REQUIRE(width_policy + width_critic <= orl_comm_capacity(comm), "%s: %d floats exceed the comm's capacity %d",
                what, width_policy + width_critic, orl_comm_capacity(comm));
    const int rc = orl_comm_next(comm, &CM);
    if (rc) return rc;
    use_comm = CM.world > 1;
  }
  const int gp = (width_policy + 63) / 64, gc = (width_critic + 63) / 64;
  hipLaunchKernelGGL(ppo_reduce_pair_kernel, dim3(gp + gc), dim3(1024), 0, (hipStream_t)stream, partials,
                     n_blocks_policy, width_policy, gp, partials + (size_t)PPO_MAX_BLOCKS * width_policy,
                     n_blocks_critic, width_critic, sums, CM, use_comm);
  return launch_status(what);
}

int orl_ppo_reduce_pair(const float* partials, int n_blocks_policy, int width_policy, int n_blocks_critic,
                        int width_critic, float* sums, void* stream) {
  return launch_reduce_pair("orl_ppo_reduce_pair", nullptr, partials, n_blocks_policy, width_policy, n_blocks_critic,
                            width_critic, sums, stream);
}

int orl_ppo_reduce_pair_comm(orl_comm* comm, const float* partials, int n_blocks_policy, int width_policy,
                             int n_blocks_critic, int width_critic, float* sums, void* stream) {
  ORL_REQUIRE(comm, "orl_ppo_reduce_pair_comm: null comm");
  return launch_reduce_pair("orl_ppo_reduce_pair_comm", comm, partials, n_blocks_policy, width_policy, n_blocks_critic,
                            width_critic, sums, stream);
}

}
```

openrl_amd/csrc/orl_ppo.hip:

```cpp
#include "orl_common.h"
#include "orl_mlp.h"
#include "orl_ppo_tower.h"

#ifndef ORL_TOWER_FIRST_VARIANT
#define ORL_TOWER_FIRST_VARIANT -1
#endif
#ifndef ORL_TOWER_TR
#define ORL_TOWER_TR 1
#endif
#ifndef ORL_ND_REM
#define ORL_ND_REM 4
#endif
#ifndef ORL_PAIR_WP_WIDE
#define ORL_PAIR_WP_WIDE 1.10
#endif
#ifndef ORL_PAIR_WP_WIDE_GAUSS
#define ORL_PAIR_WP_WIDE_GAUSS 1.30
#endif
#ifndef ORL_TOWER_TR_ND0
#define ORL_TOWER_TR_ND0 0
#endif
#ifndef ORL_TOWER_WGRAD_SPLIT
#define ORL_TOWER_WGRAD_SPLIT 1
#endif
#ifndef ORL_PAIR_WAVES
#define ORL_PAIR_WAVES 8
#endif

namespace orl {

static int check_tower(const orl_net_desc* n, const char* who) {
  if (!n) return fail(ORL_E_INVALID, "%s: null net descriptor", who);
  if (n->hidden != HID) return fail(ORL_E_UNSUPPORTED, "%s: hidden_size %d not built (only 64)", who, n->hidden);
  if (n->obs_dim < 1 || n->obs_dim > 64) return fail(ORL_E_UNSUPPORTED, "%s: obs_dim %d outside [1,64]", who, n->obs_dim);
  if (n->n_out < 1 || n->n_out > 16) return fail(ORL_E_UNSUPPORTED, "%s: n_out %d outside [1,16]", who, n->n_out);
  return 0;
}

template <int HEAD, int NO, int ND>
static int launch_tower_w(const PpoArgs& A, int waves, size_t lds, hipStream_t s) {
  const int n_tiles = (A.mb + TILE_B - 1) / TILE_B;
  int grid = (n_tiles + waves - 1) / waves;
  if (grid > PPO_MAX_BLOCKS) grid = PPO_MAX_BLOCKS;
  (void)hipFuncSetAttribute((const void*)ppo_tower_kernel<HEAD, NO, ND>, hipFuncAttributeMaxDynamicSharedMemorySize,
                            (int)lds);
  hipLaunchKernelGGL((ppo_tower_kernel<HEAD, NO, ND>), dim3(grid), dim3(waves * 64), lds, s, A);
  return grid;
}

template <int HEAD, int NO, int ND>
static int launch_tower(const PpoArgs& A, hipStream_t s) {
  constexpr int NOP = NO > 4 ? 16 : ((NO + 3) & ~3);
  static const int kWaves[4] = {8, 6, 4, 2};
  for (int k = 0; k < 4; ++k) {
    const int waves = kWaves[k];
#ifdef ORL_TOWER_MAXWAVES
    if (waves > ORL_TOWER_MAXWAVES) continue;
#endif
    for (int w2t = 1; w2t >= (ND == 0 ? 1 : 0); --w2t) {
      PpoArgs B = A;
      const int ring_nch = ring_chunks(B, ND > 0);
      const size_t lds = tower_lds_floats(A.net, A.R, NOP, waves, HEAD == ORL_HEAD_GAUSSIAN, w2t != 0, false, ring_nch) *
                         sizeof(float);
      if (lds > 160 * 1024) continue;
      B.use_w2t = w2t;
      B.lds_floats = (int)(lds / sizeof(float));
      const int grid = launch_tower_w<HEAD, NO, ND>(B, waves, lds, s);
      const int rc = launch_status("orl_ppo_fwd_bwd");
      return rc ? -1000 - rc : grid;
    }
  }
  fail(ORL_E_UNSUPPORTED, "orl_ppo_fwd_bwd: tower (obs %d, record %d floats) does not fit 160 KiB of LDS", A.net.obs_dim,
       A.R);
  return ORL_E_UNSUPPORTED;
}

template <int HEADP, int NOP_, int ND>
static int launch_pair_nd(const PpoArgs& P, const PpoArgs& Cc, int* gp_out, int* gc_out, hipStream_t s) {
  constexpr int NOPP = NOP_ > 4 ? 16 : ((NOP_ + 3) & ~3);
#if !ORL_BUILD_EXPERIMENTS
  if (P.hp.reserved & (4 | 8))
    return -1000 - fail(ORL_E_UNSUPPORTED, "orl_ppo_fwd_bwd: hparams.reserved & %d selects a comparison build (fp32-MFMA / two-image "
                        "tower pair) that this library was built without (ORL_BUILD_EXPERIMENTS)", P.hp.reserved & (4 | 8));
#endif
  for (int var = (P.hp.reserved & 4) ? 1 : ORL_TOWER_FIRST_VARIANT; var < 3; ++var) {
    const bool spt = var == -1;
    const bool sp = var <= 0;
    const int w2t = var == 0 || var == 1;
    if (var == 2 && ND == 0) break;
    if (spt && !(ND > 0 ? ORL_TOWER_TR : ORL_TOWER_TR_ND0)) continue;
    if (spt && (P.hp.reserved & 8)) continue;
    PpoArgs P2 = P, C2 = Cc;
    const int nch_p = ring_chunks(P2, ND > 0), nch_c = ring_chunks(C2, ND > 0);
    const size_t lp = tower_lds_floats(P.net, P.R, NOPP, ORL_PAIR_WAVES, HEADP == ORL_HEAD_GAUSSIAN, w2t != 0, sp, nch_p) *
                      sizeof(float);
    const size_t lc = tower_lds_floats(Cc.net, Cc.R, 4, ORL_PAIR_WAVES, false, w2t != 0, sp, nch_c) * sizeof(float);
    const size_t lds = lp > lc ? lp : lc;
    if (lds > 160 * 1024) continue;
    P2.use_w2t = w2t; C2.use_w2t = w2t;
    P2.lds_floats = C2.lds_floats = (int)(lds / sizeof(float));
    const int n_tiles = (P.mb + TILE_B - 1) / TILE_B;
    int gp = (n_tiles + 7) / 8, gc = gp;
    if (gp > PPO_MAX_BLOCKS) gp = gc = PPO_MAX_BLOCKS;
    const double w_p = NOP_ > 4 ? (HEADP == ORL_HEAD_GAUSSIAN ? ORL_PAIR_WP_WIDE_GAUSS : ORL_PAIR_WP_WIDE) : 1.05;
    const bool side_by_side = w_p < 1.1 || n_tiles <= 12 * 8 * PPO_MAX_BLOCKS;
    if (gp + gc > PPO_MAX_BLOCKS && side_by_side) {
      double best = 1e30;
      int best_g = PPO_MAX_BLOCKS / 2;
      for (int d = 0; d <= PPO_MAX_BLOCKS / 4; ++d) {
        for (int sgn = 1; sgn >= -1; sgn -= 2) {
          const int g = PPO_MAX_BLOCKS / 2 + sgn * d;
          const double tp = (double)((n_tiles + 8 * g - 1) / (8 * g)) * w_p;
          const double tc = (double)((n_tiles + 8 * (PPO_MAX_BLOCKS - g) - 1) / (8 * (PPO_MAX_BLOCKS - g)));
          const double t = tp > tc ? tp : tc;
          if (t < best - 1e-9) { best = t; best_g = g; }
          if (d == 0) break;
        }
      }
      gp = best_g;
      gc = PPO_MAX_BLOCKS - best_g;
    }
    constexpr bool HAVE_SPT = ND > 0 ? (ORL_TOWER_TR != 0) : (ORL_TOWER_TR_ND0 != 0);
    constexpr bool HAVE_SP2 = ND == 0 || ORL_BUILD_EXPERIMENTS;
    constexpr bool HAVE_FB = ND > 0 || ORL_BUILD_EXPERIMENTS;
    bool launched = false;
    if (spt) {
      if constexpr (HAVE_SPT) {
        (void)hipFuncSetAttribute((const void*)ppo_tower_pair_kernel<HEADP, NOP_, ND, 3>,
                                  hipFuncAttributeMaxDynamicSharedMemorySize, (int)lds);
        hipLaunchKernelGGL((ppo_tower_pair_kernel<HEADP, NOP_, ND, 3>), dim3(gp + gc), dim3(64 * ORL_PAIR_WAVES), lds, s, P2, C2, gp);
        launched = true;
      }
    } else if (sp) {
      if constexpr (HAVE_SP2) {
        (void)hipFuncSetAttribute((const void*)ppo_tower_pair_kernel<HEADP, NOP_, ND, 2>,
                                  hipFuncAttributeMaxDynamicSharedMemorySize, (int)lds);
        hipLaunchKernelGGL((ppo_tower_pair_kernel<HEADP, NOP_, ND, 2>), dim3(gp + gc), dim3(64 * ORL_PAIR_WAVES), lds, s, P2, C2, gp);
        launched = true;
      }
    } else {
      if (P.hp.reserved & 4) {
#if ORL_BUILD_EXPERIMENTS
        (void)hipFuncSetAttribute((const void*)ppo_tower_pair_kernel<HEADP, NOP_, ND, 0>,
                                  hipFuncAttributeMaxDynamicSharedMemorySize, (int)lds);
        hipLaunchKernelGGL((ppo_tower_pair_kernel<HEADP, NOP_, ND, 0>), dim3(gp + gc), dim3(64 * ORL_PAIR_WAVES), lds, s, P2, C2, gp);
        launched = true;
#endif
      } else if constexpr (HAVE_FB) {
        (void)hipFuncSetAttribute((const void*)ppo_tower_pair_kernel<HEADP, NOP_, ND, ORL_TOWER_WGRAD_SPLIT>,
                                  hipFuncAttributeMaxDynamicSharedMemorySize, (int)lds);
        hipLaunchKernelGGL((ppo_tower_pair_kernel<HEADP, NOP_, ND, ORL_TOWER_WGRAD_SPLIT>), dim3(gp + gc), dim3(64 * ORL_PAIR_WAVES), lds, s, P2, C2, gp);
        launched = true;
      }
    }
    if (!launched) continue;
    const int rc = launch_status("orl_ppo_fwd_bwd(pair)");
    if (rc) return -1000 - rc;
    *gp_out = gp; *gc_out = gc;
    return 1;
  }
  return 0;
}

template <int HEADP, int NOP_>
static int try_launch_pair(const PpoArgs& P, const PpoArgs& Cc, int* gp_out, int* gc_out, hipStream_t s) {
#ifdef ORL_TOWER_MAXWAVES
  return 0;
#endif
  auto nd_of = [](const PpoArgs& A) {
    const int D = A.net.obs_dim;
    return (D <= 4 && (A.o_x & 3) == 0) ? 0 : D <= 16 + ORL_ND_REM ? 1 : D <= 32 + ORL_ND_REM ? 2 : 4;
  };
  const int nd = nd_of(P);
  if (nd != nd_of(Cc)) return 0;
  if (nd == 0) return launch_pair_nd<HEADP, NOP_, 0>(P, Cc, gp_out, gc_out, s);
  if (nd == 1) return launch_pair_nd<HEADP, NOP_, 1>(P, Cc, gp_out, gc_out, s);
  if (nd == 2) return launch_pair_nd<HEADP, NOP_, 2>(P, Cc, gp_out, gc_out, s);
  return 0;
}

template <int HEAD, int NO>
static int launch_tower_nd(const PpoArgs& A, hipStream_t s) {
  const int D = A.net.obs_dim;
  if (D <= 4 && (A.o_x & 3) == 0) return launch_tower<HEAD, NO, 0>(A, s);
  if (D <= 16 + ORL_ND_REM) return launch_tower<HEAD, NO, 1>(A, s);
  if (D <= 32 + ORL_ND_REM) return launch_tower<HEAD, NO, 2>(A, s);
  return launch_tower<HEAD, NO, 4>(A, s);
}

}

using namespace orl;

extern "C" {

int orl_ppo_max_blocks(void) { return PPO_MAX_BLOCKS; }

#ifdef ORL_PROF
int orl_debug_prof(unsigned long long* out16) {
  unsigned long long zero[24] = {0};
  hipDeviceSynchronize();
  hipMemcpyFromSymbol(out16, HIP_SYMBOL(g_orl_prof), sizeof(zero));
  hipMemcpyToSymbol(HIP_SYMBOL(g_orl_prof), zero, sizeof(zero));
  return 0;
}
#endif

int orl_ppo_fwd_bwd(const orl_net_desc* pnet, const float* ptheta, const orl_net_desc* cnet, const float* ctheta,
                    const float* records, int rec_width, const int64_t* idx, int mb, const float* vn_state,
                    const orl_ppo_hparams* hp, float* partials, int* n_blocks_out, void* stream) {
  int rc = check_tower(pnet, "orl_ppo_fwd_bwd(policy)");
  if (rc) return rc;
  rc = check_tower(cnet, "orl_ppo_fwd_bwd(critic)");
  if (rc) return rc;
  ORL_REQUIRE(ptheta && ctheta && records && hp && partials, "orl_ppo_fwd_bwd: null pointer");
  ORL_REQUIRE(mb > 0, "orl_ppo_fwd_bwd: empty minibatch");
  ORL_REQUIRE(cnet->head_kind == ORL_HEAD_VALUE && cnet->n_out == 1, "orl_ppo_fwd_bwd: critic must be a value head");
  ORL_REQUIRE(pnet->head_kind == ORL_HEAD_CATEGORICAL || pnet->head_kind == ORL_HEAD_GAUSSIAN,
              "orl_ppo_fwd_bwd: policy head kind %d not built", pnet->head_kind);
  const int a_w = pnet->head_kind == ORL_HEAD_CATEGORICAL ? 1 : pnet->n_out;
  const int Dp = pnet->obs_dim, Dc = cnet->obs_dim;
  const int o_co = Dp, o_ac = o_co + Dc, o_lp = o_ac + a_w, o_adv = o_lp + a_w;
  PpoArgs A;
  A.records = records; A.idx = idx; A.vn_state = vn_state; A.hp = *hp; A.R = rec_width;
  A.o_act = o_ac; A.o_lp = o_lp; A.o_adv = o_adv; A.o_vp = o_adv + 1; A.o_rt = o_adv + 2; A.o_am = o_adv + 3;
  A.o_mk = o_adv + 4; A.a_w = a_w; A.mb = mb; A.use_w2t = 1; A.lds_floats = 0;
  A.K = pnet->head_kind == ORL_HEAD_CATEGORICAL ? pnet->n_out : 0;
  ORL_REQUIRE(orl_record_width(Dp, Dc, a_w, A.K) == rec_width, "orl_ppo_fwd_bwd: record width %d != %d", rec_width,
              orl_record_width(Dp, Dc, a_w, A.K));
  hipStream_t s = (hipStream_t)stream;
  const RawLayout rlp(*pnet);

  {
    PpoArgs P = A, Cc = A;
    P.net = *pnet; P.theta = ptheta; P.o_x = 0; P.partials = partials;
    Cc.net = *cnet; Cc.theta = ctheta; Cc.o_x = o_co;
    Cc.partials = partials + (size_t)PPO_MAX_BLOCKS * (rlp.total + ORL_N_STATS);
    int g1 = 0, g2 = 0, pr = 0;
    const int no_ = pnet->n_out;
    if (pnet->head_kind == ORL_HEAD_CATEGORICAL) {
      if (no_ <= 2) pr = try_launch_pair<ORL_HEAD_CATEGORICAL, 2>(P, Cc, &g1, &g2, s);
      else if (no_ <= 8) pr = try_launch_pair<ORL_HEAD_CATEGORICAL, 8>(P, Cc, &g1, &g2, s);
      else pr = try_launch_pair<ORL_HEAD_CATEGORICAL, 16>(P, Cc, &g1, &g2, s);
    } else {
      if (no_ <= 8) pr = try_launch_pair<ORL_HEAD_GAUSSIAN, 8>(P, Cc, &g1, &g2, s);
      else pr = try_launch_pair<ORL_HEAD_GAUSSIAN, 16>(P, Cc, &g1, &g2, s);
    }
    if (pr < 0) return -(pr + 1000);
    if (pr > 0) {
      if (n_blocks_out) { n_blocks_out[0] = g1; n_blocks_out[1] = g2; }
      return 0;
    }
  }
  A.net = *pnet; A.theta = ptheta; A.o_x = 0; A.partials = partials;
  const int no = pnet->n_out;
  int gp;
  if (pnet->head_kind == ORL_HEAD_CATEGORICAL) {
    if (no <= 2) gp = launch_tower_nd<ORL_HEAD_CATEGORICAL, 2>(A, s);
    else if (no <= 8) gp = launch_tower_nd<ORL_HEAD_CATEGORICAL, 8>(A, s);
    else gp = launch_tower_nd<ORL_HEAD_CATEGORICAL, 16>(A, s);
  } else {
    if (no <= 8) gp = launch_tower_nd<ORL_HEAD_GAUSSIAN, 8>(A, s);
    else gp = launch_tower_nd<ORL_HEAD_GAUSSIAN, 16>(A, s);
  }
  if (gp <= 0) return gp <= -1000 ? -(gp + 1000) : gp;
  A.net = *cnet; A.theta = ctheta; A.o_x = o_co;
  A.partials = partials + (size_t)PPO_MAX_BLOCKS * (rlp.total + ORL_N_STATS);
  const int gc = launch_tower_nd<ORL_HEAD_VALUE, 1>(A, s);
  if (gc <= 0) return gc <= -1000 ? -(gc + 1000) : gc;
  if (n_blocks_out) { n_blocks_out[0] = gp; n_blocks_out[1] = gc; }
  return 0;
}

}
```

openrl_amd/csrc/orl_ppo_tower.h:

```cpp
#pragma once
#include "orl_common.h"
#include "orl_mlp.h"

namespace orl {

#ifndef ORL_USE_SETPRIO
#define ORL_USE_SETPRIO 2
#endif
#if ORL_USE_SETPRIO >= 1
#define ORL_PRIO(x) __builtin_amdgcn_s_setprio(x)
#else
#define ORL_PRIO(x) ((void)0)
#endif
#if ORL_USE_SETPRIO >= 2
#define ORL_PRIO2(x)                                                           \
  do {                                                                         \
    if constexpr (ND == 0 || ORL_USE_SETPRIO >= 3) __builtin_amdgcn_s_setprio(x); \
  } while (0)
#else
#define ORL_PRIO2(x) ((void)0)
#endif

#ifdef ORL_PROF
__device__ unsigned long long g_orl_prof[24];
#define ORL_T(k)                                                                  \
  do {                                                                            \
    if (prof_on) {                                                                \
      const unsigned long long t_now = __builtin_readcyclecounter();              \
      if (l == 0) atomicAdd(&prof_lds[k], t_now - t_last);                        \
      t_last = t_now;                                                             \
    }                                                                             \
  } while (0)
#elif defined(ORL_MARK)
#define ORL_T(k) asm volatile("; ORL_PHASE " #k ::: "memory")
#else
#define ORL_T(k) ((void)0)
#endif

#ifndef ORL_TOWER_RUNSCALE
#define ORL_TOWER_RUNSCALE 1
#endif
#ifndef ORL_DMA_WAIT_DEP
#define ORL_DMA_WAIT_DEP 1
#endif
#ifndef ORL_WGRAD_HALVES
#define ORL_WGRAD_HALVES 1
#endif
#ifndef ORL_HMM_XH2_RELOAD
#define ORL_HMM_XH2_RELOAD 0
#endif
#ifndef ORL_DB3_ROWLANE
#define ORL_DB3_ROWLANE 1
#endif
constexpr int PPO_MAX_BLOCKS = 256;
constexpr int TS = 68;
constexpr int SLAB = TILE_B * TS;

struct PpoArgs {
  orl_net_desc net;
  const float* theta;
  const float* records;
  const int64_t* idx;
  const float* vn_state;
  float* partials;
  orl_ppo_hparams hp;
  int R;
  int o_x;
  int o_act, o_lp, o_adv, o_vp, o_rt, o_am, o_mk;
  int a_w;
  int K;
  int mb;
  int use_w2t;
  int c0_beg, c0_n, c1_beg;
  int lds_floats;
};

__host__ __device__ inline int ring_chunks(PpoArgs& A, bool compact) {
  const int nch = A.R >> 2;
  if (!compact) { A.c0_beg = 0; A.c0_n = nch; A.c1_beg = nch; return nch; }
  const int DP = (A.net.obs_dim + 3) & ~3;
  const int first_tail = A.net.head_kind == ORL_HEAD_VALUE ? A.o_vp : A.o_act;
  A.c0_beg = A.o_x >> 2;
  int c0_end = ((A.o_x + DP - 1) >> 2) + 1;
  if (c0_end > nch) c0_end = nch;
  A.c0_n = c0_end - A.c0_beg;
  A.c1_beg = first_tail >> 2;
  if (A.c1_beg < c0_end) A.c1_beg = c0_end;
  return A.c0_n + (nch - A.c1_beg);
}

__device__ inline float huber_or_mse(float e, float d, int use_huber, float& de) {
  if (use_huber) {
    const float ae = fabsf(e);
    if (ae <= d) { de = e; return e * e * 0.5f; }
    de = e > 0.f ? d : -d;
    return d * (ae - d * 0.5f);
  }
  de = e;
  return e * e * 0.5f;
}

__device__ inline void store_slab_T(float* __restrict__ slab, const f32x4 (&x)[4], int j, int q) {
#pragma unroll
  for (int m = 0; m < 4; ++m) *(f32x4*)(slab + j * TS + 16 * m + 4 * q) = x[m];
}
__device__ inline void load_slab_T(const float* __restrict__ slab, f32x4 (&x)[4], int j, int q) {
#pragma unroll
  for (int m = 0; m < 4; ++m) x[m] = *(const f32x4*)(slab + j * TS + 16 * m + 4 * q);
}

__device__ inline void ln_bwd_T(f32x4 (&d)[4], const f32x4 (&xhat)[4], float rstd) {
  float s1 = lane_sum16(d), s2 = lane_dot16(d, xhat);
  row_allsum2(s1, s2);
  const float k1 = -s1 * (1.0f / 64.0f) * rstd, k2 = -s2 * (1.0f / 64.0f) * rstd;
#pragma unroll
  for (int m = 0; m < 4; ++m) d[m] = xhat[m] * k2 + (d[m] * rstd + k1);
}

__device__ inline void mm64_T_wt(const float* __restrict__ Ws, const f32x4 (&in)[4], f32x4 (&acc)[4], int j, int q) {
  float a[2][4];
#pragma unroll
  for (int mo = 0; mo < 4; ++mo) a[0][mo] = Ws[(4 * q) * W2S + j + 16 * mo];
#pragma unroll
  for (int k = 0; k < 16; ++k) {
    const int mi = k >> 2, r = k & 3;
    if (k < 15) {
      const float* row = Ws + (16 * ((k + 1) >> 2) + 4 * q + ((k + 1) & 3)) * W2S + j;
#pragma unroll
      for (int mo = 0; mo < 4; ++mo) a[(k + 1) & 1][mo] = row[16 * mo];
    }
#pragma unroll
    for (int mo = 0; mo < 4; ++mo) acc[mo] = ORL_MFMA(a[k & 1][mo], in[mi][r], acc[mo]);
  }
}

template <int HEAD, int NO, int ND, int SP_ = 0>
__device__ __forceinline__ void ppo_tower_body(const PpoArgs& A, const int bid, const int nblk) {
  extern __shared__ __attribute__((aligned(16))) float smem[];
#ifdef ORL_PROF
  const unsigned long long t_entry = __builtin_readcyclecounter();
#endif
  const TowerLayout tl(A.net);
  const RawLayout rl(A.net);
  constexpr bool HMM = NO > 4;
  constexpr bool SP = SP_ >= 2;
  constexpr bool SPT = SP_ == 3;
  constexpr bool SPW = SP_ >= 1;
  const bool w2t = SPT ? false : (ND == 0 || SP || A.use_w2t);
  const TowerLds tw(ND == 0 ? 4 : A.net.obs_dim, NO <= 4 ? 4 : A.net.n_out, HEAD == ORL_HEAD_GAUSSIAN, w2t, HMM, SP);
  const int DP = tw.DP;
  const int D = A.net.obs_dim;
  const int n_out = A.net.n_out;
  constexpr int NOP = HMM ? 16 : ((NO + 3) & ~3);
  const int wave = threadIdx.x >> 6, l = threadIdx.x & 63, j = l & 15, q = l >> 4;
  const int nch = ND == 0 ? (A.R >> 2) : A.c0_n + ((A.R >> 2) - A.c1_beg);
  const int rts = ND == 0 ? ((nch + 3) >> 2) * 256 : nch * 64;
  const int per_wave = 2 * SLAB + 2 * rts + TILE_B * NOP;
  float* wl = smem + tw.total + wave * per_wave;
  float* X1 = wl;
  float* SS = wl + SLAB;
  float* RR = wl + 2 * SLAB;
  float* DH = RR + 2 * rts;

  const float* lw = smem;
  const orl_ppo_hparams hp = A.hp;

  f32x4 G[4][4];
#pragma unroll
  for (int a = 0; a < 4; ++a)
#pragma unroll
    for (int b = 0; b < 4; ++b) G[a][b] = f32x4{0.f, 0.f, 0.f, 0.f};
  f32x16 GS[2][2];
#pragma unroll
  for (int a = 0; a < 2; ++a)
#pragma unroll
    for (int b = 0; b < 2; ++b)
#pragma unroll
      for (int r = 0; r < 16; ++r) GS[a][b][r] = 0.f;
  float a_db2s[2] = {0.f, 0.f};
  constexpr bool W1S = SPW && ND == 1;
  f32x16 G1S[2];
#pragma unroll
  for (int a = 0; a < 2; ++a)
#pragma unroll
    for (int r = 0; r < 16; ++r) G1S[a][r] = 0.f;
  float a_db1s[2] = {0.f, 0.f};
  constexpr int NDA = ND > 0 ? ND : 1;
  f32x4 G1[4][NDA];
#pragma unroll
  for (int a = 0; a < 4; ++a)
#pragma unroll
    for (int b = 0; b < NDA; ++b) G1[a][b] = f32x4{0.f, 0.f, 0.f, 0.f};
  float w1v[4] = {0.f, 0.f, 0.f, 0.f};
  float a_db2 = 0.f, a_db1 = 0.f, a_db3 = 0.f, a_dls = 0.f;
  float a_db3r[NO];
#pragma unroll
  for (int c = 0; c < NO; ++c) a_db3r[c] = 0.f;
  constexpr int NS3 = HMM ? 1 : NO;
  float a_S3[NS3];
#pragma unroll
  for (int c = 0; c < NS3; ++c) a_S3[c] = 0.f;
  f32x4 S3acc[4];
#pragma unroll
  for (int mi = 0; mi < 4; ++mi) S3acc[mi] = f32x4{0.f, 0.f, 0.f, 0.f};
  float st_active = 0.f, st_rows = 0.f, st_loss = 0.f, st_ent = 0.f, st_ratio = 0.f;

  float vn_mean = 0.f, vn_sd = 1.f;
  if (HEAD == ORL_HEAD_VALUE && hp.use_valuenorm && A.vn_state != nullptr) {
    const float deb = fmaxf(A.vn_state[2], 1e-5f);
    vn_mean = A.vn_state[0] / deb;
    const float msq = A.vn_state[1] / deb;
    vn_sd = sqrtf(fmaxf(msq - vn_mean * vn_mean, 1e-2f));
  }

  const int n_tiles = (A.mb + TILE_B - 1) / TILE_B;
  const int nwv = blockDim.x >> 6;
  const int wave_g = bid * nwv + wave;
  const int n_waves = nblk * nwv;

  auto row_of = [&](int t) -> long long {
    const int ii = t * TILE_B + j;
    if (t >= n_tiles || ii >= A.mb) return 0;
    return (A.idx != nullptr) ? A.idx[ii] : (long long)ii;
  };
  auto issue_dma = [&](float* slot, long long row) {
    const float* src = A.records + (size_t)row * A.R;
#pragma unroll 1
    for (int g = 0; 4 * g < nch; ++g) {
      const int c = 4 * g + q;
      const int rc = ND == 0 ? c : (c < A.c0_n ? A.c0_beg + c : A.c1_beg + (c - A.c0_n));
      const unsigned lds_dst = __builtin_amdgcn_readfirstlane(
          (unsigned)(size_t)(__attribute__((address_space(3))) float*)(slot + g * 256));
      if (c < nch) {
        unsigned keep;
        asm volatile("s_mov_b32 %0, m0\n\ts_mov_b32 m0, %2\n\ts_nop 0\n\tglobal_load_lds_dwordx4 %1, off\n\t"
                     "s_mov_b32 m0, %0"
                     : "=&s"(keep)
                     : "v"(src + 4 * rc), "s"(lds_dst)
                     : "memory");
      }
    }
  };
  long long row_next = 0;
  int ring = 0;
  row_next = row_of(wave_g);
  issue_dma(RR, row_next);
  row_next = row_of(wave_g + n_waves);
  stage_tower(smem, A.theta, tl, tw, w2t, threadIdx.x, blockDim.x, HMM, SP, true);
  __syncthreads();
  constexpr bool F16W = SPW && ORL_TOWER_F16;
  constexpr bool F16G = SP && ORL_TOWER_F16;
  const int kw = F16G ? (int)smem[tw.wsc] : 0;
  const float w_scale = F16G ? smem[tw.wsc + 1] : 1.f, ln2_eps = F16G ? smem[tw.wsc + 3] : 1e-5f;
  int LS = 1000;
  int e_run = 0;

#ifdef ORL_PROF
  __shared__ unsigned long long prof_lds[16];
  const bool prof_on = bid == 0 && wave == 0;
  if (prof_on && l < 16) prof_lds[l] = 0ull;
  unsigned long long t_last = __builtin_readcyclecounter();
  const unsigned long long t_loop0 = t_last;
#endif
  for (int tile = wave_g; tile < n_tiles; tile += n_waves) {
    const int i = tile * TILE_B + j;
    const bool valid = i < A.mb;
    const float* RT = RR + ring * rts;
#if !defined(ORL_PROBE_NO_DMA_WAIT)
    if constexpr (ND == 0 && ORL_DMA_WAIT_DEP) asm volatile("s_waitcnt vmcnt(0)" : "+v"(RT));
    else asm volatile("s_waitcnt vmcnt(0)" ::: "memory");
#endif
    const long long row_cur = row_next;
    row_next = row_of(tile + 2 * n_waves);
    issue_dma(RR + (ring ^ 1) * rts, row_cur);
    ring ^= 1;
    const float* RTX = ND == 0 ? RT : RT - 64 * A.c0_beg;
    const float* RTT = ND == 0 ? RT : RT + 64 * (A.c0_n - A.c1_beg);
#define REC(col) RTT[(((col) >> 2) << 6) + (j << 2) + ((col) & 3)]
#define RECX(col) RTX[(((col) >> 2) << 6) + (j << 2) + ((col) & 3)]
#define REC_R(r, col) RTX[(((col) >> 2) << 6) + ((r) << 2) + ((col) & 3)]

    ORL_T(0);
    float rstd1, rstd2;
    unsigned long long relu_mask[16];
    float hd[NO];
    f32x4 hv = f32x4{0.f, 0.f, 0.f, 0.f};
    f32x4 xh2[4];
    {
      f32x4 z[4];
      load_vec_T(lw + tw.b1, q, z);
      if constexpr (ND == 0 || ND > 2) {
        fc1_T(lw + tw.W1, DP, [&](int s) -> float { return RECX(A.o_x + 4 * s + q); }, z, j, q);
      } else {
        constexpr int MAXS = 4 * ND + 1;
        const int nks = DP >> 2;
        float bq[MAXS], aq[MAXS][4];
#pragma unroll
        for (int s = 0; s < MAXS; ++s) {
          const bool on = s < nks;
          bq[s] = on ? RECX(A.o_x + 4 * s + q) : 0.f;
#pragma unroll
          for (int m = 0; m < 4; ++m) aq[s][m] = on ? lw[tw.W1 + (16 * m + j) * DP + 4 * s + q] : 0.f;
        }
#pragma unroll
        for (int s = 0; s < MAXS; ++s) {
          if (s < nks) {
#pragma unroll
            for (int m = 0; m < 4; ++m) z[m] = ORL_MFMA(aq[s][m], bq[s], z[m]);
          }
        }
      }
#pragma unroll
      for (int m = 0; m < 4; ++m)
#pragma unroll
        for (int r = 0; r < 4; ++r) {
          relu_mask[4 * m + r] = __builtin_amdgcn_ballot_w64(z[m][r] > 0.f);
          z[m][r] = fmaxf(z[m][r], 0.f);
        }
      ln_normalize_T(z, rstd1);
      store_slab_T(X1, z, j, q);
      load_vec_T(lw + tw.b2, q, xh2);
      ORL_T(1);
      ORL_PRIO(1);
      if constexpr (F16G) {
        u32x4 xs[2][2];
        split_Th(z, xs);
        mm64_T_h2((const unsigned short*)(lw + tw.W2), xs, xh2, j, q);
      } else if constexpr (SP) {
        u32x4 xs[2][3];
        split_T(z, xs);
        mm64_T_split((const unsigned short*)(lw + tw.W2), xs, xh2, j, q);
// ... 810 lines not shown
          for (int bo = 0; bo < 2; ++bo)
#pragma unroll
            for (int r = 0; r < 16; ++r) acc[w_idx(bo, r)] = first ? G1S[bo][r] : old[bo][r] + G1S[bo][r];
        }
      } else if (ND == 0) {
#pragma unroll
        for (int k = 0; k < 4; ++k)
          if (k < D) put(rl.odW1 + f * D + k, w1v[k]);
      } else {
#pragma unroll
        for (int mf = 0; mf < 4; ++mf)
#pragma unroll
          for (int mk = 0; mk < NDA; ++mk)
#pragma unroll
            for (int r = 0; r < 4; ++r) {
              const int kk = 16 * mk + j;
              if (kk < D) put(rl.odW1 + (16 * mf + 4 * q + r) * D + kk, G1[mf][mk][r]);
            }
#pragma unroll
        for (int k = 0; k < 4; ++k)
          if (16 * ND + k < D) put(rl.odW1 + f * D + 16 * ND + k, w1v[k]);
      }
      if (l == 0) {
        put(rl.total + ST_ACTIVE_SUM, st_active);
        put(rl.total + ST_ROWS, st_rows);
        if (HEAD == ORL_HEAD_VALUE) put(rl.total + ST_VLOSS_SUM, st_loss);
        else {
          put(rl.total + ST_PLOSS_SUM, st_loss);
          put(rl.total + ST_ENT_SUM, st_ent);
          put(rl.total + ST_RATIO_SUM, st_ratio);
        }
      }
    }
    __syncthreads();
  }
#ifdef ORL_PROF
  if (prof_on && l == 18) atomicAdd(&g_orl_prof[18], __builtin_readcyclecounter() - t_loop1);
#endif
  float* out = A.partials + (size_t)bid * PW;
  if (frag_g) {
    for (int k = threadIdx.x; k < GN / 4; k += blockDim.x) {
      const int Rq = k >> 6, ln = k & 63;
      f32x4 v[NREG_MAX];
#pragma unroll
      for (int w = 0; w < NREG_MAX; ++w)
        v[w] = w < nwv ? *(const f32x4*)(gimg + (size_t)w * GN + Rq * 256 + ln * 4) : f32x4{0.f, 0.f, 0.f, 0.f};
      f32x4 t = v[0];
#pragma unroll
      for (int w = 1; w < NREG_MAX; ++w) t += v[w];
      const int o0 = 32 * (Rq >> 3) + 8 * (Rq & 3) + 4 * (ln >> 5), i = 32 * ((Rq >> 2) & 1) + (ln & 31);
#pragma unroll
      for (int rr = 0; rr < 4; ++rr) out[(o0 + rr) * HID + i] = t[rr];
    }
  }
#pragma unroll 2
  for (int e = IOFF + threadIdx.x; e < PW; e += blockDim.x) {
    float v[NREG_MAX];
#pragma unroll
    for (int g = 0; g < NREG_MAX; ++g) v[g] = g < NREG ? img0[(size_t)g * PWI + e - IOFF] : 0.f;
    float t = v[0];
#pragma unroll
    for (int g = 1; g < NREG_MAX; ++g) t += v[g];
    out[e] = t;
  }
#ifdef ORL_PROF
  if (prof_on && l == 15) atomicAdd(&g_orl_prof[15], __builtin_readcyclecounter() - t_loop1);
#endif
}

template <int HEAD, int NO, int ND>
__global__ __launch_bounds__(512, 2) void ppo_tower_kernel(PpoArgs A) {
  ppo_tower_body<HEAD, NO, ND>(A, (int)blockIdx.x, (int)gridDim.x);
}

#ifndef ORL_PAIR_WAVES
#define ORL_PAIR_WAVES 8
#endif
template <int HEADP, int NOP_, int ND, int SP = 0>
__global__ __launch_bounds__(64 * ORL_PAIR_WAVES, (ORL_PAIR_WAVES + 3) / 4) void ppo_tower_pair_kernel(PpoArgs P, PpoArgs Cc, int gp) {
  if ((int)blockIdx.x < gp) ppo_tower_body<HEADP, NOP_, ND, SP>(P, (int)blockIdx.x, gp);
  else ppo_tower_body<ORL_HEAD_VALUE, 1, ND, SP>(Cc, (int)blockIdx.x - gp, (int)gridDim.x - gp);
}

inline size_t tower_lds_floats(const orl_net_desc& net, int R, int nop, int waves, bool gaussian, bool w2t = true,
                               bool split = false, int ring_nch = -1) {
  const TowerLds tw(net.obs_dim, net.n_out, gaussian, w2t, nop == 16, split);
  const RawLayout rl(net);
  if (ring_nch < 0) ring_nch = R >> 2;
  const int rts = net.obs_dim <= 4 ? (((R >> 2) + 3) >> 2) * 256 : ring_nch * 64;
  const size_t per_wave = 2 * SLAB + 2 * rts + TILE_B * nop;
  size_t fl = (size_t)tw.total + (size_t)waves * per_wave;
  const size_t pw = (size_t)rl.total + ORL_N_STATS;
  const size_t need_acc = pw;
  const size_t all_waves = (size_t)waves * pw;
  if (fl < all_waves && all_waves * sizeof(float) <= 160 * 1024) fl = all_waves;
  return fl > need_acc ? fl : need_acc;
}

}
```

openrl_amd/ops.py:

```python
from __future__ import annotations

import ctypes as C
from dataclasses import dataclass
from typing import List, Optional, Sequence, Tuple

import torch

from . import _native as nat
from ._native import (AdamState, BufferPtrs, GatherDesc, NetDesc, PackSrc, PPOHParams, RolloutArgs, fptr, ptr,
                      stream_ptr)

HEAD_VALUE, HEAD_CATEGORICAL, HEAD_GAUSSIAN = nat.ORL_HEAD_VALUE, nat.ORL_HEAD_CATEGORICAL, nat.ORL_HEAD_GAUSSIAN
ENV_SYNTH, ENV_CARTPOLE, ENV_PENDULUM = nat.ORL_ENV_SYNTH, nat.ORL_ENV_CARTPOLE, nat.ORL_ENV_PENDULUM
ENV_ACROBOT, ENV_MOUNTAINCAR = nat.ORL_ENV_ACROBOT, nat.ORL_ENV_MOUNTAINCAR
ENV_MOUNTAINCAR_CONT = nat.ORL_ENV_MOUNTAINCAR_CONT
N_STATS = nat.ORL_N_STATS


def _lib():
    return nat.load()


def net_desc(obs_dim: int, n_out: int, head_kind: int, hidden: int = 64) -> NetDesc:
    return NetDesc(int(obs_dim), int(hidden), int(n_out), int(head_kind))
# ... 105 lines not shown
    d.count = len(srcs)
    rc = _lib().orl_gather_minibatch(C.byref(d), ptr(idx), n, stream_ptr(dev))
    nat.check(rc, "orl_gather_minibatch")
    return outs


def perm_feistel(n: int, seed: int, stream_id: int, device, vn=None) -> torch.Tensor:
    dev = nat.require_gpu(device)
    idx = torch.empty(n, dtype=torch.int64, device=dev)
    if vn is None:
        rc = _lib().orl_perm_feistel(ptr(idx), n, seed & (2 ** 64 - 1), stream_id & (2 ** 64 - 1), stream_ptr(dev))
    else:
        rc = _lib().orl_perm_feistel_vn(ptr(idx), n, seed & (2 ** 64 - 1), stream_id & (2 ** 64 - 1), fptr(vn[0]),
                                        ptr(vn[1]), float(vn[2]), stream_ptr(dev))
    nat.check(rc, "orl_perm_feistel")
    return idx


def act_step(pnet: NetDesc, ptheta, cnet: Optional[NetDesc], ctheta, policy_obs, critic_obs, action_masks, B: int,
             deterministic: bool, seed: int, row0: int, rng_step: int, forced_u, values, actions, logp,
             rng_step_dev=None) -> None:
    dev = _dev(policy_obs if policy_obs is not None else critic_obs)
    rc = _lib().orl_act_step(C.byref(pnet), fptr(ptheta), C.byref(cnet) if cnet is not None else None, fptr(ctheta),
                             fptr(policy_obs), fptr(critic_obs), fptr(action_masks), B, int(bool(deterministic)),
                             seed & (2 ** 64 - 1), row0, rng_step, ptr(rng_step_dev), fptr(forced_u), fptr(values),
                             fptr(actions), fptr(logp), stream_ptr(dev))
    nat.check(rc, "orl_act_step")


def act_step_grouped(pnet: NetDesc, pthetas, rows_per_group: int, policy_obs, action_masks, B: int, deterministic: bool,
                     seed: int, row0: int, rng_step: int, actions, logp, rng_step_dev=None) -> None:
    dev = _dev(policy_obs)
    rc = _lib().orl_act_step_grouped(C.byref(pnet), fptr(pthetas), pthetas.stride(0), rows_per_group, fptr(policy_obs),
                                     fptr(action_masks), B, int(bool(deterministic)), seed & (2 ** 64 - 1), row0,
                                     rng_step, ptr(rng_step_dev), fptr(actions), fptr(logp), stream_ptr(dev))
    nat.check(rc, "orl_act_step_grouped")


def act_step_pool(pnet: NetDesc, pthetas, opp_index, policy_obs, action_masks, B: int, deterministic: bool, seed: int,
                  row0: int, rng_step: int, actions, logp, rng_step_dev=None) -> None:
    dev = _dev(policy_obs)
    assert opp_index.dtype == torch.int32
    rc = _lib().orl_act_step_pool(C.byref(pnet), fptr(pthetas), pthetas.stride(0), pthetas.shape[0], ptr(opp_index),
                                  fptr(policy_obs), fptr(action_masks), B, int(bool(deterministic)),
                                  seed & (2 ** 64 - 1), row0, rng_step, ptr(rng_step_dev), fptr(actions), fptr(logp),
                                  stream_ptr(dev))
    nat.check(rc, "orl_act_step_pool")


def opponent_sample(opp_index, dones, n_filled: int, last_slot: int, strategy: int, per_tile: bool, seed: int,
                    draw_id: int, draw_id_dev=None) -> None:
    dev = _dev(opp_index)
    rc = _lib().orl_opponent_sample(ptr(opp_index), ptr(dones), opp_index.numel(), n_filled, last_slot, strategy,
                                    int(bool(per_tile)), seed & (2 ** 64 - 1), draw_id, ptr(draw_id_dev),
                                    stream_ptr(dev))
    nat.check(rc, "orl_opponent_sample")


def critic_values(cnet: NetDesc, ctheta, critic_obs, values) -> None:
    dev = _dev(critic_obs)
    rows = critic_obs.numel() // cnet.obs_dim
    rc = _lib().orl_critic_values(C.byref(cnet), fptr(ctheta), fptr(critic_obs), rows, fptr(values), stream_ptr(dev))
    nat.check(rc, "orl_critic_values")


def evaluate_actions(pnet, ptheta, cnet, ctheta, policy_obs, critic_obs, actions, action_masks, active_masks, B: int,
                     values, logp, ent_rows, dist_entropy) -> None:
    dev = _dev(policy_obs)
    rc = _lib().orl_evaluate_actions(C.byref(pnet), fptr(ptheta), C.byref(cnet) if cnet is not None else None,
                                     fptr(ctheta), fptr(policy_obs), fptr(critic_obs), fptr(actions),
                                     fptr(action_masks), fptr(active_masks), B, fptr(values), fptr(logp),
                                     fptr(ent_rows), fptr(dist_entropy), stream_ptr(dev))
    nat.check(rc, "orl_evaluate_actions")


def ppo_fwd_bwd(pnet, ptheta, cnet, ctheta, records, idx, mb: int, vn_state, hp: PPOHParams, partials):
    dev = _dev(records)
    nb = (C.c_int * 2)(0, 0)
    rc = _lib().orl_ppo_fwd_bwd(C.byref(pnet), fptr(ptheta), C.byref(cnet), fptr(ctheta), fptr(records),
                                records.shape[1], ptr(idx), mb, fptr(vn_state), C.byref(hp), fptr(partials),
                                nb, stream_ptr(dev))
    nat.check(rc, "orl_ppo_fwd_bwd")
    return nb[0], nb[1]


def ppo_reduce(partials_ptr: int, n_blocks: int, width: int, sums_ptr: int, dev) -> None:
    rc = _lib().orl_ppo_reduce(partials_ptr, n_blocks, width, sums_ptr, stream_ptr(dev))
    nat.check(rc, "orl_ppo_reduce")


def ppo_reduce_pair(partials, nb_p: int, width_p: int, nb_c: int, width_c: int, sums, comm=None) -> None:
    dev = _dev(sums)
    if comm is None:
        rc = _lib().orl_ppo_reduce_pair(fptr(partials), nb_p, width_p, nb_c, width_c, fptr(sums), stream_ptr(dev))
    else:
        rc = _lib().orl_ppo_reduce_pair_comm(comm.handle, fptr(partials), nb_p, width_p, nb_c, width_c, fptr(sums),
                                             stream_ptr(dev))
    nat.check(rc, "orl_ppo_reduce_pair")


def ppo_apply(pnet, cnet, sums, hp: PPOHParams, padam: AdamState, cadam: AdamState, train_info_accum,
              next_perm=None, comm=None):
    dev = _dev(sums)
    if comm is not None:
        idx, n, seed, stream_id, vn = None, 0, 0, 0, None
        if next_perm is not None:
            n, seed, stream_id, vn = next_perm
            idx = torch.empty(n, dtype=torch.int64, device=dev)
        rc = _lib().orl_ppo_apply_comm(comm.handle, C.byref(pnet), C.byref(cnet), fptr(sums), C.byref(hp),
                                       C.byref(padam), C.byref(cadam), fptr(train_info_accum), ptr(idx), n,
                                       seed & (2 ** 64 - 1), stream_id & (2 ** 64 - 1), fptr(vn[0]) if vn else None,
                                       ptr(vn[1]) if vn else None, float(vn[2]) if vn else 0.0, stream_ptr(dev))
        nat.check(rc, "orl_ppo_apply_comm")
        return idx
    if next_perm is None:
        rc = _lib().orl_ppo_apply(C.byref(pnet), C.byref(cnet), fptr(sums), C.byref(hp), C.byref(padam),
                                  C.byref(cadam), fptr(train_info_accum), stream_ptr(dev))
        nat.check(rc, "orl_ppo_apply")
        return None
    n, seed, stream_id, vn = next_perm
    idx = torch.empty(n, dtype=torch.int64, device=dev)
    rc = _lib().orl_ppo_apply_perm(C.byref(pnet), C.byref(cnet), fptr(sums), C.byref(hp), C.byref(padam),
                                   C.byref(cadam), fptr(train_info_accum), ptr(idx), n, seed & (2 ** 64 - 1),
                                   stream_id & (2 ** 64 - 1), fptr(vn[0]) if vn else None, ptr(vn[1]) if vn else None,
                                   float(vn[2]) if vn else 0.0, stream_ptr(dev))
    nat.check(rc, "orl_ppo_apply_perm")
    return idx


def ppo_reduce_apply(partials, nb_p: int, width_p: int, nb_c: int, width_c: int, sums, pnet, cnet, hp: PPOHParams,
                     padam: AdamState, cadam: AdamState, train_info_accum, sync_ctr, next_perm=None, comm=None,
                     entry: str = "orl_ppo_reduce_apply"):
    dev = _dev(sums)
    idx, n, seed, stream_id, vn = None, 0, 0, 0, None
    if next_perm is not None:
        n, seed, stream_id, vn = next_perm
        idx = torch.empty(n, dtype=torch.int64, device=dev)
    rc = getattr(_lib(), entry)(comm.handle if comm is not None else None, fptr(partials), nb_p, width_p, nb_c,
                                width_c, fptr(sums), C.byref(pnet), C.byref(cnet), C.byref(hp), C.byref(padam),
                                C.byref(cadam), fptr(train_info_accum), ptr(idx), n, seed & (2 ** 64 - 1),
                                stream_id & (2 ** 64 - 1), fptr(vn[0]) if vn else None, ptr(vn[1]) if vn else None,
                                float(vn[2]) if vn else 0.0, ptr(sync_ctr), stream_ptr(dev))
    nat.check(rc, entry)
    return idx


def valuenorm_update(vn_state, moments, beta: float = 0.99999) -> None:
    dev = _dev(vn_state)
    rc = _lib().orl_valuenorm_update(fptr(vn_state), ptr(moments), float(beta), stream_ptr(dev))
    nat.check(rc, "orl_valuenorm_update")


def minibatch_moments(records, ret_col: int, idx, mb: int, scratch, moments) -> None:
    dev = _dev(records)
    rc = _lib().orl_minibatch_moments(fptr(records), records.shape[1], ret_col, ptr(idx), mb, ptr(scratch),
                                      ptr(moments), stream_ptr(dev))
    nat.check(rc, "orl_minibatch_moments")


def env_state_width(env_kind: int) -> int:
    n = _lib().orl_env_state_width(env_kind)
    if n < 0:
        nat.check(n, "orl_env_state_width")
    return n


# ... 42 lines not shown
```

Baseline: 257.4 million.

## Fold pending Adam step into next PPO fwd/bwd launch via double-buffered state

```diff
diff --git a/include/orl_hip.h b/include/orl_hip.h
--- a/include/orl_hip.h
+++ b/include/orl_hip.h
@@ -156,6 +156,26 @@
   float lr, eps, weight_decay;
   int32_t step;
 } orl_adam_state;
+
+typedef struct orl_adam_src {
+  const float* theta;
+  const float* m;
+  const float* v;
+} orl_adam_src;
+
+int orl_ppo_step_foldable(const orl_net_desc* pnet, const orl_net_desc* cnet, int rec_width);
+int orl_ppo_fwd_bwd_step(const orl_net_desc* pnet, const orl_net_desc* cnet, const float* records, int rec_width,
+                         const int64_t* idx, int mb, const float* vn_state, const orl_ppo_hparams* hp, float* partials,
+                         int* n_blocks_out, const float* sums, const float* step_coef, const orl_ppo_hparams* step_hp,
+                         const orl_adam_state* padam, const orl_adam_state* cadam, const orl_adam_src* psrc,
+                         const orl_adam_src* csrc, float* train_info_accum, void* stream);
+int orl_ppo_reduce_pair_step(const float* partials, int n_blocks_policy, int width_policy, int n_blocks_critic,
+                             int width_critic, float* sums, const orl_adam_state* padam, const orl_adam_state* cadam,
+                             float* step_coef, int64_t* next_idx, int64_t n, uint64_t seed, uint64_t stream_id,
+                             float* vn_state, const double* moments, double beta, void* stream);
+int orl_ppo_apply_from(const orl_net_desc* pnet, const orl_net_desc* cnet, const float* sums, const orl_ppo_hparams* hp,
+                       const orl_adam_state* padam, const orl_adam_state* cadam, const orl_adam_src* psrc,
+                       const orl_adam_src* csrc, float* train_info_accum, void* stream);
 
 int orl_ppo_reduce(const float* partials, int n_blocks, int width, float* sums, void* stream);
 int orl_ppo_reduce_pair(const float* partials, int n_blocks_policy, int width_policy, int n_blocks_critic,
diff --git a/openrl_amd/_native.py b/openrl_amd/_native.py
--- a/openrl_amd/_native.py
+++ b/openrl_amd/_native.py
@@ -66,6 +66,10 @@
 class AdamState(C.Structure):
     _fields_ = [("theta", C.c_void_p), ("grad", C.c_void_p), ("m", C.c_void_p), ("v", C.c_void_p),
                 ("lr", C.c_float), ("eps", C.c_float), ("weight_decay", C.c_float), ("step", C.c_int32)]
+
+
+class AdamSrc(C.Structure):
+    _fields_ = [("theta", C.c_void_p), ("m", C.c_void_p), ("v", C.c_void_p)]
 
 
 class RolloutArgs(C.Structure):
@@ -185,6 +189,17 @@
     "orl_ppo_apply_perm": (C.c_int, [C.POINTER(NetDesc), C.POINTER(NetDesc), _P, C.POINTER(PPOHParams),
                                      C.POINTER(AdamState), C.POINTER(AdamState), _P, _P, C.c_int64, C.c_uint64,
                                      C.c_uint64, _P, _P, C.c_double, _P]),
+    "orl_ppo_step_foldable": (C.c_int, [C.POINTER(NetDesc), C.POINTER(NetDesc), C.c_int]),
+    "orl_ppo_fwd_bwd_step": (C.c_int, [C.POINTER(NetDesc), C.POINTER(NetDesc), _P, C.c_int, _P, C.c_int, _P,
+                                       C.POINTER(PPOHParams), _P, C.POINTER(C.c_int), _P, _P, C.POINTER(PPOHParams),
+                                       C.POINTER(AdamState), C.POINTER(AdamState), C.POINTER(AdamSrc), C.POINTER(AdamSrc),
+                                       _P, _P]),
+    "orl_ppo_reduce_pair_step": (C.c_int, [_P, C.c_int, C.c_int, C.c_int, C.c_int, _P, C.POINTER(AdamState),
+                                           C.POINTER(AdamState), _P, _P, C.c_int64, C.c_uint64, C.c_uint64, _P, _P,
+                                           C.c_double, _P]),
+    "orl_ppo_apply_from": (C.c_int, [C.POINTER(NetDesc), C.POINTER(NetDesc), _P, C.POINTER(PPOHParams),
+                                     C.POINTER(AdamState), C.POINTER(AdamState), C.POINTER(AdamSrc), C.POINTER(AdamSrc),
+                                     _P, _P]),
     "orl_comm_create": (C.c_int, [C.c_int, C.c_int, C.c_int64, C.POINTER(_P), _P]),
     "orl_comm_connect": (C.c_int, [_P, _P]),
     "orl_comm_destroy": (C.c_int, [_P]),
diff --git a/openrl_amd/algorithms/ppo.py b/openrl_amd/algorithms/ppo.py
--- a/openrl_amd/algorithms/ppo.py
+++ b/openrl_amd/algorithms/ppo.py
@@ -117,6 +117,13 @@
         self._adv_stats = torch.zeros(11, dtype=torch.float64, device=self.device)
         self._moments_mb = self._moments
         self._full_batch_moments = False
+        self._apply_in_staging = bool(getattr(cfg, "amd_apply_in_staging", True))
+        self.apply_in_staging_active = False
+        self._pending = None
+        self._step_bufs = None
+        self._step_cur = 0
+        self._foldable = {}
+        self._step_coef = torch.zeros(16, dtype=torch.float32, device=self.device)
         if self.generic:
             self.recurrent = bool(getattr(self.algo_module, "recurrent", False))
             self._rnn_rows = None
@@ -194,6 +201,43 @@
                                buffer.pack_src(), buffer.ensure_records())
         buffer._adv_fresh = False
 
+    @staticmethod
+    def _adam_src(bufs) -> "nat.AdamSrc":
+        return nat.AdamSrc(nat.fptr(bufs[0]), nat.fptr(bufs[1]), nat.fptr(bufs[2]))
+
+    def _arm_apply_in_staging(self, buffer) -> None:
+        self.apply_in_staging_active = False
+        self._pending = None
+        self._step_cur = 0
+        if self.generic or self.recurrent or not self._apply_in_staging or self.world_size != 1:
+            return
+        if self._optim_step != "two_launch" or (self.hp.reserved & (4 | 8)):
+            return
+        mod = self.algo_module
+        p, c = mod.models["policy"], mod.models["critic"]
+        R = int(buffer.records.shape[1])
+        if R not in self._foldable:
+            self._foldable[R] = ops.ppo_step_foldable(p.net, c.net, R)
+        if not self._foldable[R]:
+            return
+        po, co = mod.optimizers["policy"], mod.optimizers["critic"]
+        canon = [(p.theta, po.exp_avg, po.exp_avg_sq), (c.theta, co.exp_avg, co.exp_avg_sq)]
+        sb = self._step_bufs
+        if sb is None or any(a is not b for x, y in zip(sb[0], canon) for a, b in zip(x, y)):
+            self._step_bufs = [canon, [tuple(torch.empty_like(t) for t in tw) for tw in canon]]
+        self.apply_in_staging_active = True
+
+    def _flush_pending_step(self) -> None:
+        if self._pending is None:
+            return
+        hp_s, pad, cad = self._pending
+        self._pending = None
+        p, c = self.algo_module.models["policy"], self.algo_module.models["critic"]
+        src = self._step_bufs[self._step_cur]
+        self._step_cur = 0
+        ops.ppo_apply_from(p.net, c.net, self._sums, hp_s, pad, cad, self._adam_src(src[0]), self._adam_src(src[1]),
+                           self._info)
+
     def _update_minibatch(self, buffer, idx, mb: int, turn_on: bool, next_perm=None):
         if self.generic:
             from .ppo_generic import update_minibatch_generic
@@ -222,13 +266,24 @@
         if ev is not None:
             e0, e1 = torch.cuda.Event(enable_timing=True), torch.cuda.Event(enable_timing=True)
             e0.record()
-        nb_p, nb_c = ops.ppo_fwd_bwd(p.net, p.theta, c.net, c.theta, rec, idx, mb, vn_state, self.hp, self._partials)
+        fold = self.apply_in_staging_active
+        if fold and self._pending is not None:
+            hp_s, pad, cad = self._pending
+            self._pending = None
+            src, dst = self._step_bufs[self._step_cur], self._step_bufs[1 - self._step_cur]
+            self._step_cur = 1 - self._step_cur
+            for ad, d in ((pad, dst[0]), (cad, dst[1])):
+                ad.theta, ad.m, ad.v = nat.fptr(d[0]), nat.fptr(d[1]), nat.fptr(d[2])
+            nb_p, nb_c = ops.ppo_fwd_bwd_step(p.net, c.net, rec, idx, mb, vn_state, self.hp, self._partials, self._sums,
+                                              self._step_coef, hp_s, pad, cad, self._adam_src(src[0]), self._adam_src(src[1]), self._info)
+        else:
+            nb_p, nb_c = ops.ppo_fwd_bwd(p.net, p.theta, c.net, c.theta, rec, idx, mb, vn_state, self.hp, self._partials)
         if ev is not None:
             e1.record()
             ev.append((e0, e1))
         comm = self._comm
         fused = self._fused_step and (self.world_size == 1 or comm is not None)
-        if not fused:
+        if not fold and not fused:
             ops.ppo_reduce_pair(self._partials, nb_p, self._raw_p, nb_c, self._raw_c, self._sums, comm=comm)
             if self.world_size > 1 and comm is None:
                 dist_utils.allreduce_(self._sums)
@@ -243,6 +298,12 @@
             if first:
                 hp.reserved |= 32
                 self._info_first = False
+        if fold:
+            pad, cad = po.native_state(max(po.step_count, 1)), co.native_state(co.step_count)
+            perm_idx = ops.ppo_reduce_pair_step(self._partials, nb_p, self._raw_p, nb_c, self._raw_c, self._sums, pad, cad,
+                                                self._step_coef, next_perm)
+            self._pending = (hp if hp is not self.hp else nat.PPOHParams.from_buffer_copy(self.hp), pad, cad)
+            return perm_idx
         if fused:
             return ops.ppo_reduce_apply(self._partials, nb_p, self._raw_p, nb_c, self._raw_c, self._sums, p.net, c.net, hp,
                                         po.native_state(max(po.step_count, 1)), co.native_state(co.step_count),
@@ -481,6 +542,7 @@
         if getattr(self, "_comm_watch", None) is not None:
             self._comm_watch.poll()
         self._advantages_and_records(buffer)
+        self._arm_apply_in_staging(buffer)
         M = buffer.episode_length * buffer.n_rollout_threads * buffer.num_agents
         self._full_batch_moments = self.num_mini_batch == 1 and (not self.recurrent or M % self.data_chunk_length == 0)
         self._moments = self._adv_stats[8:11] if self._full_batch_moments else self._moments_mb
@@ -514,6 +576,7 @@
                         and self.perm_mode == "device"):
                     job = self._perm_job(M)
                 next_perm = self._update_minibatch(buffer, idx, mbs, turn_on, job)
+        self._flush_pending_step()
         self._info_first = False
         keys = self.info_keys
         scale = np.full(len(keys), np.float32(1.0) / np.float32(num_updates), dtype=np.float32)
diff --git a/openrl_amd/configs/config.py b/openrl_amd/configs/config.py
--- a/openrl_amd/configs/config.py
+++ b/openrl_amd/configs/config.py
@@ -15,6 +15,7 @@
     ("amd_tower_gemm", "str", "split", "opt", ["split", "fp32", "split_two_image"]),
     ("amd_rnn_gemm", "str", "fp32", "opt", ["fp32", "fp32_recompute", "split", "split_w4"]),
     ("amd_optim_step", "str", "two_launch", "opt", ["two_launch", "step", "fused"]),
+    ("amd_apply_in_staging", "bool", False, "opt", None),
     ("amd_gen_update", "str", "fused", "opt", ["fused", "layerwise"]),
 ]
 
diff --git a/openrl_amd/csrc/orl_adam_step.h b/openrl_amd/csrc/orl_adam_step.h
--- /dev/null
+++ b/openrl_amd/csrc/orl_adam_step.h
@@ -0,0 +1,293 @@
+#pragma once
+#include "orl_common.h"
+#include "orl_mlp.h"
+
+namespace orl {
+
+#define ORL_STEP_FP _Pragma("clang fp reassociate(off)") _Pragma("clang fp reciprocal(off)") _Pragma("clang fp contract(off)")
+
+__device__ __forceinline__ float step_rn(float x) {
+  asm("" : "+v"(x));
+  return x;
+}
+
+__device__ inline float step_div(float a, float b) {
+  ORL_STEP_FP
+  bool f_den, f_num;
+  const float den = __builtin_amdgcn_div_scalef(a, b, false, &f_den);
+  const float num = __builtin_amdgcn_div_scalef(a, b, true, &f_num);
+  const float rcp = __builtin_amdgcn_rcpf(den);
+  const float nden = -den;
+  const float e0 = __builtin_fmaf(nden, rcp, 1.0f);
+  const float r1 = __builtin_fmaf(e0, rcp, rcp);
+  const float q0 = num * r1;
+  const float e1 = __builtin_fmaf(nden, q0, num);
+  const float q1 = __builtin_fmaf(e1, r1, q0);
+  const float e2 = __builtin_fmaf(nden, q1, num);
+  const float q = __builtin_amdgcn_div_fmasf(e2, r1, q1, f_num);
+  return __builtin_amdgcn_div_fixupf(q, b, a);
+}
+__device__ inline float step_sqrt(float x) {
+  ORL_STEP_FP
+  const bool scale = x < 0x1.0p-96f;
+  const float xs = scale ? x * 0x1.0p+32f : x;
+  float s = __builtin_amdgcn_sqrtf(xs);
+  const int si = __builtin_bit_cast(int, s);
+  const float s_dn = __builtin_bit_cast(float, si - 1), s_up = __builtin_bit_cast(float, si + 1);
+  const float r_dn = __builtin_fmaf(-s_dn, s, xs), r_up = __builtin_fmaf(-s_up, s, xs);
+  const unsigned xb = __builtin_bit_cast(unsigned, xs);
+  if (r_dn <= 0.f) s = s_dn;
+  if (r_up > 0.f) s = s_up;
+  if (scale) s = s * 0x1.0p-16f;
+  return ((xb << 1) == 0u || xb == 0x7f800000u) ? xs : s;
+}
+
+struct StepTower {
+  orl_net_desc net;
+  orl_adam_state ad;
+  const float* theta_src;
+  const float* m_src;
+  const float* v_src;
+  int sums_off;
+};
+
+struct PendingStep {
+  const float* sums;
+  const float* coef;
+  float* info;
+  orl_ppo_hparams hp;
+  StepTower P, Cc;
+  int th_off;
+};
+
+__device__ inline float step_wave_sum(float v) {
+  ORL_STEP_FP
+  v += __builtin_bit_cast(float, __builtin_amdgcn_update_dpp(0u, __builtin_bit_cast(unsigned, v), 0x121, 0xf, 0xf, false));
+  v += __builtin_bit_cast(float, __builtin_amdgcn_update_dpp(0u, __builtin_bit_cast(unsigned, v), 0x122, 0xf, 0xf, false));
+  v += __builtin_bit_cast(float, __builtin_amdgcn_update_dpp(0u, __builtin_bit_cast(unsigned, v), 0x124, 0xf, 0xf, false));
+  v += __builtin_bit_cast(float, __builtin_amdgcn_update_dpp(0u, __builtin_bit_cast(unsigned, v), 0x128, 0xf, 0xf, false));
+  float a = v, b = v;
+  asm volatile("s_nop 1\n\tv_permlane16_swap_b32 %0, %1\n\ts_nop 1" : "+v"(a), "+v"(b));
+  const float t = a + b;
+  a = t;
+  b = t;
+  asm volatile("s_nop 1\n\tv_permlane32_swap_b32 %0, %1\n\ts_nop 1" : "+v"(a), "+v"(b));
+  return a + b;
+}
+
+__device__ inline float step_sum16(const float* sh) {
+  ORL_STEP_FP
+  float t = 0.f;
+  for (int k = 0; k < 16; ++k) t += sh[k];
+  return t;
+}
+
+__device__ inline float raw_to_grad(const float* __restrict__ raw, const float* __restrict__ theta,
+                                    const TowerLayout& tl, const RawLayout& rl, int p, float inv_den) {
+  ORL_STEP_FP
+  const int H = HID;
+  float g;
+  if (p < tl.ob1) g = raw[rl.odW1 + (p - tl.oW1)];
+  else if (p < tl.og1) g = raw[rl.odb1 + (p - tl.ob1)];
+  else if (p < tl.obe1) {
+    const int i = p - tl.og1;
+    g = 0.f;
+#pragma unroll 8
+    for (int o = 0; o < H; ++o) g = __builtin_fmaf(theta[tl.oW2 + o * H + i], raw[rl.oG + o * H + i], g);
+  } else if (p < tl.oW2) {
+    const int i = p - tl.obe1;
+    g = 0.f;
+#pragma unroll 8
+    for (int o = 0; o < H; ++o) g = __builtin_fmaf(theta[tl.oW2 + o * H + i], raw[rl.odb2 + o], g);
+  } else if (p < tl.ob2) {
+    const int e = p - tl.oW2, o = e / H, i = e - o * H;
+    g = step_rn(theta[tl.og1 + i] * raw[rl.oG + e]) + step_rn(theta[tl.obe1 + i] * raw[rl.odb2 + o]);
+  } else if (p < tl.og2) g = raw[rl.odb2 + (p - tl.ob2)];
+  else if (p < tl.obe2) {
+    const int f = p - tl.og2;
+    g = 0.f;
+    for (int c = 0; c < tl.n_out; ++c) g = __builtin_fmaf(theta[tl.oW3 + c * H + f], raw[rl.oS3 + c * H + f], g);
+  } else if (p < tl.oW3) {
+    const int f = p - tl.obe2;
+    g = 0.f;
+    for (int c = 0; c < tl.n_out; ++c) g = __builtin_fmaf(theta[tl.oW3 + c * H + f], raw[rl.odb3 + c], g);
+  } else if (p < tl.ob3) {
+    const int e = p - tl.oW3, c = e / H, f = e - c * H;
+    g = step_rn(theta[tl.og2 + f] * raw[rl.oS3 + e]) + step_rn(theta[tl.obe2 + f] * raw[rl.odb3 + c]);
+  } else if (p < tl.ologstd) g = raw[rl.odb3 + (p - tl.ob3)];
+  else g = raw[rl.odlogstd + (p - tl.ologstd)];
+  return step_rn(g * inv_den);
+}
+
+struct AdamCoef {
+  float b2, omb1, omb2, step_size, bc2_sqrt;
+};
+__device__ inline AdamCoef adam_coef(float lr, int step) {
+  ORL_STEP_FP
+  const double b1d = 0.9, b2d = 0.999;
+  double p1 = 1.0, p2 = 1.0, q1 = b1d, q2 = b2d;
+  for (long long n = (long long)step; n > 0; n >>= 1) {
+    if (n & 1) { p1 *= q1; p2 *= q2; }
+    q1 *= q1;
+    q2 *= q2;
+  }
+  const double bc1 = 1.0 - p1, bc2 = 1.0 - p2;
+  AdamCoef K;
+  K.b2 = (float)b2d; K.omb1 = (float)(1.0 - b1d); K.omb2 = (float)(1.0 - b2d);
+  K.step_size = (float)((double)lr / bc1);
+  K.bc2_sqrt = (float)__builtin_sqrt(bc2);
+  return K;
+}
+
+__device__ inline float step_norm(float sum_sq) {
+  ORL_STEP_FP
+  return step_sqrt(sum_sq);
+}
+__device__ inline float clip_coef(const orl_ppo_hparams& hp, float total) {
+  ORL_STEP_FP
+  float coef = 1.f;
+  if (hp.use_max_grad_norm) coef = __builtin_fminf(step_div(hp.max_grad_norm, total + 1e-6f), 1.f);
+  return coef;
+}
+
+__device__ inline float adam_element(float gs, float coef, const orl_adam_state& ad, const AdamCoef& K, float& th, float& m,
+                                     float& v) {
+  ORL_STEP_FP
+  float g = step_rn(gs * coef);
+  const float g_out = g;
+  if (ad.weight_decay != 0.f) g = g + step_rn(ad.weight_decay * th);
+  m = m + step_rn((g - m) * K.omb1);
+  v = step_rn(v * K.b2) + step_rn(K.omb2 * step_rn(g * g));
+  const float denom = step_div(step_sqrt(v), K.bc2_sqrt) + ad.eps;
+  th = __builtin_fmaf(-step_div(m, denom), K.step_size, th);
+  return g_out;
+}
+
+__device__ inline void step_info(const int t, const orl_net_desc& pnet, const orl_ppo_hparams& hp, const float* st, float den_p,
+                                 float den_v, float norm, float* __restrict__ info) {
+  ORL_STEP_FP
+  const bool first = (hp.reserved & 32) != 0;
+  auto acc = [&](int k, float x) {
+    if (first) info[k] = x;
+    else unsafeAtomicAdd(info + k, x);
+  };
+  if (t == 0) {
+    float ent_den = den_p;
+    if (!hp.use_policy_active_masks && pnet.head_kind == ORL_HEAD_GAUSSIAN) ent_den = den_p * (float)pnet.n_out;
+    acc(1, step_div(st[ST_PLOSS_SUM], den_p));
+    acc(2, step_div(st[ST_ENT_SUM], ent_den));
+    acc(3, norm);
+    const float a_w = pnet.head_kind == ORL_HEAD_GAUSSIAN ? (float)pnet.n_out : 1.f;
+    acc(5, step_div(st[ST_RATIO_SUM], st[ST_ROWS] * a_w));
+  } else {
+    acc(0, step_div(st[ST_VLOSS_SUM], den_v));
+    acc(4, norm);
+  }
+}
+__device__ inline void step_info_policy_off(const orl_net_desc& pnet, const orl_ppo_hparams& hp, const float* stp, float den_p,
+                                            float* __restrict__ info) {
+  ORL_STEP_FP
+  if (hp.reserved & 32) info[1] = info[2] = info[3] = info[5] = 0.f;
+  info[1] += step_div(stp[ST_PLOSS_SUM], den_p);
+  float ent_den0 = den_p;
+  if (!hp.use_policy_active_masks && pnet.head_kind == ORL_HEAD_GAUSSIAN) ent_den0 = den_p * (float)pnet.n_out;
+  info[2] += step_div(stp[ST_ENT_SUM], ent_den0);
+  const float aw0 = pnet.head_kind == ORL_HEAD_GAUSSIAN ? (float)pnet.n_out : 1.f;
+  info[5] += step_div(stp[ST_RATIO_SUM], stp[ST_ROWS] * aw0);
+}
+
+constexpr int STEP_NT = 512;
+constexpr int STEP_KMAX = 12;
+
+__device__ inline void stage_dma(float* lds_dst, const float* __restrict__ src, int n) {
+  const int lane = threadIdx.x & 63;
+#pragma unroll 1
+  for (int e0 = (threadIdx.x & ~63); e0 < n; e0 += blockDim.x) {
+    if (e0 + lane < n)
+      __builtin_amdgcn_global_load_lds((const __attribute__((address_space(1))) void*)(src + e0 + lane),
+                                       (__attribute__((address_space(3))) void*)(lds_dst + e0), 4, 0, 0);
+  }
+}
+
+__device__ inline void pending_step_tower(const int t, const PendingStep& S, float* __restrict__ raw, float* __restrict__ g_s,
+                                          float* __restrict__ th_s, float* __restrict__ sh, const bool writer) {
+  ORL_STEP_FP
+  const StepTower& W = t == 0 ? S.P : S.Cc;
+  const orl_ppo_hparams& hp = S.hp;
+  const TowerLayout tl(W.net);
+  const RawLayout rl(W.net);
+  const int tid = threadIdx.x;
+  const bool policy_off = t == 0 && (hp.reserved & 1);
+  float m[STEP_KMAX], v[STEP_KMAX];
+#pragma unroll
+  for (int k = 0; k < STEP_KMAX; ++k) {
+    const int p = tid + k * STEP_NT;
+    const bool ok = p < tl.total && (writer || !policy_off);
+    m[k] = ok ? W.m_src[p] : 0.f;
+    v[k] = ok ? W.v_src[p] : 0.f;
+  }
+  stage_dma(raw, S.sums + W.sums_off, rl.total + ORL_N_STATS);
+  stage_dma(th_s, W.theta_src, tl.total);
+  AdamCoef K;
+  {
+    const float* kc = S.coef + 5 * t;
+    K.b2 = kc[0]; K.omb1 = kc[1]; K.omb2 = kc[2]; K.step_size = kc[3]; K.bc2_sqrt = kc[4];
+  }
+  asm volatile("s_waitcnt vmcnt(0)" ::: "memory");
+  __syncthreads();
+  const float* st = raw + rl.total;
+  const float den_p = hp.use_policy_active_masks ? st[ST_ACTIVE_SUM] : st[ST_ROWS];
+  const float den_v = hp.use_value_active_masks ? st[ST_ACTIVE_SUM] : st[ST_ROWS];
+  if (policy_off) {
+    if (writer) {
+#pragma unroll
+      for (int k = 0; k < STEP_KMAX; ++k) {
+        const int p = tid + k * STEP_NT;
+        if (p < tl.total) {
+          W.ad.grad[p] = 0.f;
+          W.ad.theta[p] = th_s[p]; W.ad.m[p] = m[k]; W.ad.v[p] = v[k];
+        }
+      }
+      if (tid == 0 && S.info != nullptr) step_info_policy_off(S.P.net, hp, st, den_p, S.info);
+    }
+    return;
+  }
+  const float inv_den = step_div(1.0f, t == 0 ? den_p : den_v);
+  float ss_a = 0.f, ss_b = 0.f;
+#pragma unroll 1
+  for (int p = tid; p < tl.total; p += 2 * STEP_NT) {
+    const float ga = raw_to_grad(raw, th_s, tl, rl, p, inv_den);
+    g_s[p] = ga;
+    ss_a = __builtin_fmaf(ga, ga, ss_a);
+    if (p + STEP_NT < tl.total) {
+      const float gb = raw_to_grad(raw, th_s, tl, rl, p + STEP_NT, inv_den);
+      g_s[p + STEP_NT] = gb;
+      ss_b = __builtin_fmaf(gb, gb, ss_b);
+    }
+  }
+  ss_a = step_wave_sum(ss_a);
+  ss_b = step_wave_sum(ss_b);
+  if ((tid & 63) == 0) {
+    sh[tid >> 6] = ss_a;
+    sh[(tid >> 6) + STEP_NT / 64] = ss_b;
+  }
+  __syncthreads();
+  const float total = step_norm(step_sum16(sh));
+  const float coef = clip_coef(hp, total);
+#pragma unroll
+  for (int k = 0; k < STEP_KMAX; ++k) {
+    const int p = tid + k * STEP_NT;
+    if (p < tl.total) {
+      float th = th_s[p];
+      const float gc = adam_element(g_s[p], coef, W.ad, K, th, m[k], v[k]);
+      th_s[p] = th;
+      if (writer) {
+        W.ad.grad[p] = gc;
+        W.ad.m[p] = m[k]; W.ad.v[p] = v[k]; W.ad.theta[p] = th;
+      }
+    }
+  }
+  if (writer && tid == 0 && S.info != nullptr) step_info(t, S.P.net, hp, st, den_p, den_v, total, S.info);
+}
+
+}
diff --git a/openrl_amd/csrc/orl_apply.hip b/openrl_amd/csrc/orl_apply.hip
--- a/openrl_amd/csrc/orl_apply.hip
+++ b/openrl_amd/csrc/orl_apply.hip
@@ -29,67 +29,26 @@
     sums[col] = (sh[0][threadIdx.x] + sh[1][threadIdx.x]) + (sh[2][threadIdx.x] + sh[3][threadIdx.x]);
 }
 
-struct ApplyTower {
-  orl_net_desc net;
-  orl_adam_state ad;
-  int sums_off;
-};
-
-__device__ inline void stage_dma(float* lds_dst, const float* __restrict__ src, int n) {
-  const int lane = threadIdx.x & 63;
-#pragma unroll 1
-  for (int e0 = (threadIdx.x & ~63); e0 < n; e0 += blockDim.x) {
-    if (e0 + lane < n)
-      __builtin_amdgcn_global_load_lds((const __attribute__((address_space(1))) void*)(src + e0 + lane),
-                                       (__attribute__((address_space(3))) void*)(lds_dst + e0), 4, 0, 0);
-  }
+typedef StepTower ApplyTower;
+
+static ApplyTower make_apply_tower(const orl_net_desc& net, const orl_adam_state& ad, int sums_off,
+                                   const orl_adam_src* src = nullptr) {
+  ApplyTower T;
+  T.net = net; T.ad = ad; T.sums_off = sums_off;
+  T.theta_src = src && src->theta ? src->theta : ad.theta;
+  T.m_src = src && src->m ? src->m : ad.m;
+  T.v_src = src && src->v ? src->v : ad.v;
+  return T;
 }
 
 __device__ inline float block_sum_1024(float v, float* sh) {
-  v = wave_sum_dpp(v);
+  v = step_wave_sum(v);
   const int w = threadIdx.x >> 6;
   if ((threadIdx.x & 63) == 0) sh[w] = v;
   __syncthreads();
-  float t = 0.f;
-  for (int k = 0; k < 16; ++k) t += sh[k];
+  const float t = step_sum16(sh);
   __syncthreads();
   return t;
-}
-
-__device__ inline float raw_to_grad(const float* __restrict__ raw, const float* __restrict__ theta,
-                                    const TowerLayout& tl, const RawLayout& rl, int p, float inv_den) {
-  const int H = HID;
-  float g;
-  if (p < tl.ob1) g = raw[rl.odW1 + (p - tl.oW1)];
-  else if (p < tl.og1) g = raw[rl.odb1 + (p - tl.ob1)];
-  else if (p < tl.obe1) {
-    const int i = p - tl.og1;
-    g = 0.f;
-#pragma unroll 8
-    for (int o = 0; o < H; ++o) g += theta[tl.oW2 + o * H + i] * raw[rl.oG + o * H + i];
-  } else if (p < tl.oW2) {
-    const int i = p - tl.obe1;
-    g = 0.f;
-#pragma unroll 8
-    for (int o = 0; o < H; ++o) g += theta[tl.oW2 + o * H + i] * raw[rl.odb2 + o];
-  } else if (p < tl.ob2) {
-    const int e = p - tl.oW2, o = e / H, i = e - o * H;
-    g = theta[tl.og1 + i] * raw[rl.oG + e] + theta[tl.obe1 + i] * raw[rl.odb2 + o];
-  } else if (p < tl.og2) g = raw[rl.odb2 + (p - tl.ob2)];
-  else if (p < tl.obe2) {
-    const int f = p - tl.og2;
-    g = 0.f;
-    for (int c = 0; c < tl.n_out; ++c) g += theta[tl.oW3 + c * H + f] * raw[rl.oS3 + c * H + f];
-  } else if (p < tl.oW3) {
-    const int f = p - tl.obe2;
-    g = 0.f;
-    for (int c = 0; c < tl.n_out; ++c) g += theta[tl.oW3 + c * H + f] * raw[rl.odb3 + c];
-  } else if (p < tl.ob3) {
-    const int e = p - tl.oW3, c = e / H, f = e - c * H;
-    g = theta[tl.og2 + f] * raw[rl.oS3 + e] + theta[tl.obe2 + f] * raw[rl.odb3 + c];
-  } else if (p < tl.ologstd) g = raw[rl.odb3 + (p - tl.ob3)];
-  else g = raw[rl.odlogstd + (p - tl.ologstd)];
-  return g * inv_den;
 }
 
 __device__ inline bool apply_tower_block(const int t, const ApplyTower& P, const ApplyTower& Cc, float* __restrict__ sums,
@@ -113,10 +72,10 @@
         const ApplyTower& W0 = t == 0 ? P : Cc;
         const TowerLayout& tl0 = t == 0 ? tlp : tlc;
         float* th0 = s_apply + rl0.total + ORL_N_STATS;
-        stage_dma(th0, W0.ad.theta, tl0.total);
+        stage_dma(th0, W0.theta_src, tl0.total);
         if (stage_mv) {
-          stage_dma(th0 + 2 * tl0.total, W0.ad.m, tl0.total);
-          stage_dma(th0 + 3 * tl0.total, W0.ad.v, tl0.total);
+          stage_dma(th0 + 2 * tl0.total, W0.m_src, tl0.total);
+          stage_dma(th0 + 3 * tl0.total, W0.v_src, tl0.total);
         }
         params_staged = true;
       }
@@ -168,15 +127,12 @@
       den_p = hp.use_policy_active_masks ? st[ST_ACTIVE_SUM] : st[ST_ROWS];
       const float* stp = st;
       for (int p = threadIdx.x; p < tl.total; p += blockDim.x) W.ad.grad[p] = 0.f;
-      if (threadIdx.x == 0 && info != nullptr) {
-        if (hp.reserved & 32) info[1] = info[2] = info[3] = info[5] = 0.f;
-        info[1] += stp[ST_PLOSS_SUM] / den_p;
-        float ent_den0 = den_p;
-        if (!hp.use_policy_active_masks && P.net.head_kind == ORL_HEAD_GAUSSIAN) ent_den0 = den_p * (float)P.net.n_out;
-        info[2] += stp[ST_ENT_SUM] / ent_den0;
-        const float aw0 = P.net.head_kind == ORL_HEAD_GAUSSIAN ? (float)P.net.n_out : 1.f;
-        info[5] += stp[ST_RATIO_SUM] / (stp[ST_ROWS] * aw0);
-      }
+      if (W.theta_src != W.ad.theta) {
+        for (int p = threadIdx.x; p < tl.total; p += blockDim.x) {
+          W.ad.theta[p] = W.theta_src[p]; W.ad.m[p] = W.m_src[p]; W.ad.v[p] = W.v_src[p];
+        }
+      }
+      if (threadIdx.x == 0 && info != nullptr) step_info_policy_off(P.net, hp, stp, den_p, info);
       return true;
     }
     float* th_s = s_apply + rl.total + ORL_N_STATS;
@@ -184,43 +140,31 @@
     float* m_s = g_s + tl.total;
     float* v_s = m_s + tl.total;
     if (!params_staged) {
-      stage_dma(th_s, W.ad.theta, tl.total);
+      stage_dma(th_s, W.theta_src, tl.total);
       if (stage_mv) {
-        stage_dma(m_s, W.ad.m, tl.total);
-        stage_dma(v_s, W.ad.v, tl.total);
-      }
-    }
-    const double b1d = 0.9, b2d = 0.999;
-    const float b2 = (float)b2d, omb1 = (float)(1.0 - b1d), omb2 = (float)(1.0 - b2d);
-    const double bc1 = 1.0 - powi_d(b1d, (long long)W.ad.step);
-    const double bc2 = 1.0 - powi_d(b2d, (long long)W.ad.step);
-    const float step_size = (float)((double)W.ad.lr / bc1);
-    const float bc2_sqrt = (float)sqrt(bc2);
+        stage_dma(m_s, W.m_src, tl.total);
+        stage_dma(v_s, W.v_src, tl.total);
+      }
+    }
+    const AdamCoef K = adam_coef(W.ad.lr, W.ad.step);
     asm volatile("s_waitcnt vmcnt(0)" ::: "memory");
     __syncthreads();
     den_p = hp.use_policy_active_masks ? st[ST_ACTIVE_SUM] : st[ST_ROWS];
     den_v = hp.use_value_active_masks ? st[ST_ACTIVE_SUM] : st[ST_ROWS];
-    const float inv_den = 1.0f / (t == 0 ? den_p : den_v);
+    const float inv_den = step_div(1.0f, t == 0 ? den_p : den_v);
     float ss = 0.f;
 #pragma unroll 1
     for (int p = threadIdx.x; p < tl.total; p += blockDim.x) {
       const float g = raw_to_grad(raw, th_s, tl, rl, p, inv_den);
       g_s[p] = g;
-      ss += g * g;
-    }
-    const float total = sqrtf(block_sum_1024(ss, sh));
+      ss = __builtin_fmaf(g, g, ss);
+    }
+    const float total = step_norm(block_sum_1024(ss, sh));
     norms[t] = total;
-    float coef = 1.f;
-    if (hp.use_max_grad_norm) coef = fminf(hp.max_grad_norm / (total + 1e-6f), 1.f);
+    const float coef = clip_coef(hp, total);
     auto adam = [&](int p, float m, float v) {
-      float g = g_s[p] * coef;
-      W.ad.grad[p] = g;
       float th = th_s[p];
-      if (W.ad.weight_decay != 0.f) g += W.ad.weight_decay * th;
-      m = m + (g - m) * omb1;
-      v = v * b2 + omb2 * (g * g);
-      const float denom = sqrtf(v) / bc2_sqrt + W.ad.eps;
-      th = th - step_size * (m / denom);
+      W.ad.grad[p] = adam_element(g_s[p], coef, W.ad, K, th, m, v);
       W.ad.m[p] = m; W.ad.v[p] = v; W.ad.theta[p] = th;
     };
     if (stage_mv) {
@@ -228,30 +172,10 @@
       for (int p = threadIdx.x; p < tl.total; p += blockDim.x) adam(p, m_s[p], v_s[p]);
     } else {
 #pragma unroll 1
-      for (int p = threadIdx.x; p < tl.total; p += blockDim.x) adam(p, W.ad.m[p], W.ad.v[p]);
-    }
-  }
-  if (threadIdx.x == 0 && info != nullptr) {
-    const float* stp = st;
-    const float* stc = st;
-    const bool first = (hp.reserved & 32) != 0;
-    auto acc = [&](int k, float x) {
-      if (first) info[k] = x;
-      else unsafeAtomicAdd(info + k, x);
-    };
-    if (t == 0) {
-      float ent_den = den_p;
-      if (!hp.use_policy_active_masks && P.net.head_kind == ORL_HEAD_GAUSSIAN) ent_den = den_p * (float)P.net.n_out;
-      acc(1, stp[ST_PLOSS_SUM] / den_p);
-      acc(2, stp[ST_ENT_SUM] / ent_den);
-      acc(3, norms[0]);
-      const float a_w = P.net.head_kind == ORL_HEAD_GAUSSIAN ? (float)P.net.n_out : 1.f;
-      acc(5, stp[ST_RATIO_SUM] / (stp[ST_ROWS] * a_w));
-    } else {
-      acc(0, stc[ST_VLOSS_SUM] / den_v);
-      acc(4, norms[1]);
-    }
-  }
+      for (int p = threadIdx.x; p < tl.total; p += blockDim.x) adam(p, W.m_src[p], W.v_src[p]);
+    }
+  }
+  if (threadIdx.x == 0 && info != nullptr) step_info(t, P.net, hp, st, den_p, den_v, norms[t], info);
   return true;
 }
 
@@ -394,6 +318,27 @@
                        pol ? sums : sums + wp, pol ? 0 : wp, CM, use_comm, sh);
 }
 
+__global__ __launch_bounds__(1024) void ppo_reduce_pair_step_kernel(const float* __restrict__ pp, int nb_p, int wp, int gp,
+                                                                    const float* __restrict__ pc, int nb_c, int wc, int gc,
+                                                                    float* __restrict__ sums, CommDev CM, PermJob J,
+                                                                    float lr_p, int step_p, float lr_c, int step_c,
+                                                                    float* __restrict__ coef) {
+  __shared__ float sh[16][64];
+  const int b = (int)blockIdx.x;
+  if (b >= gp + gc) {
+    if (b == gp + gc && threadIdx.x < 2) {
+      const AdamCoef K = adam_coef(threadIdx.x == 0 ? lr_p : lr_c, threadIdx.x == 0 ? step_p : step_c);
+      float* o = coef + 5 * threadIdx.x;
+      o[0] = K.b2; o[1] = K.omb1; o[2] = K.omb2; o[3] = K.step_size; o[4] = K.bc2_sqrt;
+    }
+    if (J.idx != nullptr) perm_job_block(J, b - (gp + gc), (int)gridDim.x - (gp + gc));
+    return;
+  }
+  const bool pol = b < gp;
+  reduce_columns_block(pol ? pp : pc, pol ? nb_p : nb_c, pol ? wp : wc, (pol ? b : b - gp) * 64, pol ? sums : sums + wp,
+                       pol ? 0 : wp, CM, 0, sh);
+}
+
 static int check_tower(const orl_net_desc* n, const char* who) {
   if (!n) return fail(ORL_E_INVALID, "%s: null net descriptor", who);
   if (n->hidden != HID) return fail(ORL_E_UNSUPPORTED, "%s: hidden_size %d not built (only 64)", who, n->hidden);
@@ -418,7 +363,8 @@
 
 static int launch_apply(const char* what, const orl_net_desc* pnet, const orl_net_desc* cnet, float* sums,
                         const orl_ppo_hparams* hp, const orl_adam_state* padam, const orl_adam_state* cadam,
-                        float* train_info_accum, const PermJob& J, void* stream, orl_comm* comm = nullptr) {
+                        float* train_info_accum, const PermJob& J, void* stream, orl_comm* comm = nullptr,
+                        const orl_adam_src* psrc = nullptr, const orl_adam_src* csrc = nullptr) {
   int rc = check_tower(pnet, what);
   if (rc) return rc;
   rc = check_tower(cnet, what);
@@ -427,9 +373,8 @@
   ORL_REQUIRE(padam->theta && padam->grad && padam->m && padam->v && cadam->theta && cadam->grad && cadam->m && cadam->v,
               "%s: null optimizer buffer", what);
   ORL_REQUIRE(padam->step >= 1 && cadam->step >= 1, "%s: Adam step counts are 1-based", what);
-  ApplyTower P, Cc;
-  P.net = *pnet; P.ad = *padam; P.sums_off = 0;
-  Cc.net = *cnet; Cc.ad = *cadam; Cc.sums_off = RawLayout(*pnet).total + ORL_N_STATS;
+  const ApplyTower P = make_apply_tower(*pnet, *padam, 0, psrc);
+  const ApplyTower Cc = make_apply_tower(*cnet, *cadam, RawLayout(*pnet).total + ORL_N_STATS, csrc);
   auto need = [&](int k) {
     const size_t lp = (size_t)(RawLayout(*pnet).total + ORL_N_STATS + k * TowerLayout(*pnet).total) * sizeof(float);
     const size_t lc = (size_t)(RawLayout(*cnet).total + ORL_N_STATS + k * TowerLayout(*cnet).total) * sizeof(float);
@@ -503,6 +448,7 @@
   return fail(ORL_E_UNSUPPORTED, "%s: the ticketed one-launch optimiser step lost its A/B (15.7 us against 4.4 + 9.3 us for "
               "orl_ppo_reduce_pair + orl_ppo_apply) and is only present in an ORL_BUILD_EXPERIMENTS library", what);
 #else
+  const orl_adam_src *psrc = nullptr, *csrc = nullptr;
   int rc = check_tower(pnet, what);
   if (rc) return rc;
   rc = check_tower(cnet, what);
@@ -512,9 +458,8 @@
   ORL_REQUIRE(padam->theta && padam->grad && padam->m && padam->v && cadam->theta && cadam->grad && cadam->m && cadam->v,
               "%s: null optimizer buffer", what);
   ORL_REQUIRE(padam->step >= 1 && cadam->step >= 1, "%s: Adam step counts are 1-based", what);
-  ApplyTower P, Cc;
-  P.net = *pnet; P.ad = *padam; P.sums_off = 0;
-  Cc.net = *cnet; Cc.ad = *cadam; Cc.sums_off = RawLayout(*pnet).total + ORL_N_STATS;
+  const ApplyTower P = make_apply_tower(*pnet, *padam, 0, psrc);
+  const ApplyTower Cc = make_apply_tower(*cnet, *cadam, RawLayout(*pnet).total + ORL_N_STATS, csrc);
   ORL_REQUIRE(width_policy == Cc.sums_off && width_critic == RawLayout(*cnet).total + ORL_N_STATS,
               "%s: partial widths %d / %d do not match the towers' raw vectors (%d / %d)", what, width_policy, width_critic,
               Cc.sums_off, RawLayout(*cnet).total + ORL_N_STATS);
@@ -564,6 +509,7 @@
                  float* train_info_accum, int64_t* next_idx, int64_t n, uint64_t seed, uint64_t stream_id, float* vn_state,
                  const double* moments, double beta, uint32_t* sync_ctr, void* stream) {
   const char* what = "orl_ppo_step";
+  const orl_adam_src *psrc = nullptr, *csrc = nullptr;
   int rc = check_tower(pnet, what);
   if (rc) return rc;
   rc = check_tower(cnet, what);
@@ -573,9 +519,8 @@
   ORL_REQUIRE(padam->theta && padam->grad && padam->m && padam->v && cadam->theta && cadam->grad && cadam->m && cadam->v,
               "%s: null optimizer buffer", what);
   ORL_REQUIRE(padam->step >= 1 && cadam->step >= 1, "%s: Adam step counts are 1-based", what);
-  ApplyTower P, Cc;
-  P.net = *pnet; P.ad = *padam; P.sums_off = 0;
-  Cc.net = *cnet; Cc.ad = *cadam; Cc.sums_off = RawLayout(*pnet).total + ORL_N_STATS;
+  const ApplyTower P = make_apply_tower(*pnet, *padam, 0, psrc);
+  const ApplyTower Cc = make_apply_tower(*cnet, *cadam, RawLayout(*pnet).total + ORL_N_STATS, csrc);
   ORL_REQUIRE(width_policy == Cc.sums_off && width_critic == RawLayout(*cnet).total + ORL_N_STATS,
               "%s: partial widths %d / %d do not match the towers' raw vectors (%d / %d)", what, width_policy, width_critic,
               Cc.sums_off, RawLayout(*cnet).total + ORL_N_STATS);
@@ -645,6 +590,45 @@
                             width_critic, sums, stream);
 }
 
+int orl_ppo_reduce_pair_step(const float* partials, int n_blocks_policy, int width_policy, int n_blocks_critic,
+                             int width_critic, float* sums, const orl_adam_state* padam, const orl_adam_state* cadam,
+                             float* step_coef, int64_t* next_idx, int64_t n, uint64_t seed, uint64_t stream_id,
+                             float* vn_state, const double* moments, double beta, void* stream) {
+  const char* what = "orl_ppo_reduce_pair_step";
+  ORL_REQUIRE(partials && sums && n_blocks_policy > 0 && n_blocks_critic > 0 && width_policy > 0 && width_critic > 0,
+              "%s: bad arguments", what);
+  ORL_REQUIRE(padam && cadam && step_coef, "%s: null pointer", what);
+  ORL_REQUIRE(padam->step >= 1 && cadam->step >= 1, "%s: Adam step counts are 1-based", what);
+  PermJob J;
+  memset(&J, 0, sizeof(J));
+  int perm_blocks = 1;
+  if (next_idx != nullptr) {
+    ORL_REQUIRE(n > 0 && n <= ((int64_t)1 << 62), "%s: bad permutation arguments", what);
+    ORL_REQUIRE(!vn_state || moments, "%s: vn_state needs moments", what);
+    J = make_perm_job(next_idx, n, seed, stream_id, vn_state, moments, beta);
+    perm_blocks = (int)((n + 1023) / 1024);
+    if (perm_blocks > 254) perm_blocks = 254;
+  }
+  CommDev CM;
+  memset(&CM, 0, sizeof(CM));
+  const int gp = (width_policy + 63) / 64, gc = (width_critic + 63) / 64;
+  hipLaunchKernelGGL(ppo_reduce_pair_step_kernel, dim3(gp + gc + perm_blocks), dim3(1024), 0, (hipStream_t)stream, partials,
+                     n_blocks_policy, width_policy, gp, partials + (size_t)PPO_MAX_BLOCKS * width_policy, n_blocks_critic,
+                     width_critic, gc, sums, CM, J, padam->lr, (int)padam->step, cadam->lr, (int)cadam->step, step_coef);
+  return launch_status(what);
+}
+
+int orl_ppo_apply_from(const orl_net_desc* pnet, const orl_net_desc* cnet, const float* sums, const orl_ppo_hparams* hp,
+                       const orl_adam_state* padam, const orl_adam_state* cadam, const orl_adam_src* psrc,
+                       const orl_adam_src* csrc, float* train_info_accum, void* stream) {
+  ORL_REQUIRE(psrc && csrc && psrc->theta && psrc->m && psrc->v && csrc->theta && csrc->m && csrc->v,
+              "orl_ppo_apply_from: null source buffer");
+  PermJob J;
+  memset(&J, 0, sizeof(J));
+  return launch_apply("orl_ppo_apply_from", pnet, cnet, (float*)sums, hp, padam, cadam, train_info_accum, J, stream, nullptr,
+                      psrc, csrc);
+}
+
 int orl_ppo_reduce_pair_comm(orl_comm* comm, const float* partials, int n_blocks_policy, int width_policy,
                              int n_blocks_critic, int width_critic, float* sums, void* stream) {
   ORL_REQUIRE(comm, "orl_ppo_reduce_pair_comm: null comm");
diff --git a/openrl_amd/csrc/orl_ppo.hip b/openrl_amd/csrc/orl_ppo.hip
--- a/openrl_amd/csrc/orl_ppo.hip
+++ b/openrl_amd/csrc/orl_ppo.hip
@@ -1,3 +1,4 @@
+#include <string.h>
 #include "orl_common.h"
 #include "orl_mlp.h"
 #include "orl_ppo_tower.h"
@@ -76,7 +77,8 @@
 }
 
 template <int HEADP, int NOP_, int ND>
-static int launch_pair_nd(const PpoArgs& P, const PpoArgs& Cc, int* gp_out, int* gc_out, hipStream_t s) {
+static int launch_pair_nd(const PpoArgs& P, const PpoArgs& Cc, int* gp_out, int* gc_out, hipStream_t s,
+                          PendingStep* S = nullptr, bool query = false) {
   constexpr int NOPP = NOP_ > 4 ? 16 : ((NOP_ + 3) & ~3);
 #if !ORL_BUILD_EXPERIMENTS
   if (P.hp.reserved & (4 | 8))
@@ -99,6 +101,25 @@
     if (lds > 160 * 1024) continue;
     P2.use_w2t = w2t; C2.use_w2t = w2t;
     P2.lds_floats = C2.lds_floats = (int)(lds / sizeof(float));
+    size_t lds_launch = lds;
+    if (S != nullptr) {
+      if (!(ND == 0 && sp && !spt)) return 0;
+      const size_t end_p = tower_lds_end(P.net, P.R, NOPP, ORL_PAIR_WAVES, HEADP == ORL_HEAD_GAUSSIAN, w2t != 0, sp, nch_p);
+      const size_t end_c = tower_lds_end(Cc.net, Cc.R, 4, ORL_PAIR_WAVES, false, w2t != 0, sp, nch_c);
+      const size_t th_off = ((end_p > end_c ? end_p : end_c) + 3) & ~(size_t)3;
+      const int tot_p = TowerLayout(P.net).total, tot_c = TowerLayout(Cc.net).total;
+      const int pw_p = RawLayout(P.net).total + ORL_N_STATS, pw_c = RawLayout(Cc.net).total + ORL_N_STATS;
+      const int img_p = TowerLds(P.net.obs_dim, P.net.n_out, HEADP == ORL_HEAD_GAUSSIAN, w2t != 0, NOPP == 16, sp).total;
+      const int img_c = TowerLds(Cc.net.obs_dim, Cc.net.n_out, false, w2t != 0, false, sp).total;
+      const size_t need = (th_off + (size_t)(tot_p > tot_c ? tot_p : tot_c)) * sizeof(float);
+      const int cap = STEP_KMAX * STEP_NT;
+      if (need > 160 * 1024 || pw_p + 20 + tot_p > img_p || pw_c + 20 + tot_c > img_c || tot_p > cap || tot_c > cap || pw_p > cap || pw_c > cap ||
+          ORL_PAIR_WAVES * 64 != STEP_NT)
+        return 0;
+      if (query) return 1;
+      S->th_off = (int)th_off;
+      if (need > lds_launch) lds_launch = need;
+    }
     const int n_tiles = (P.mb + TILE_B - 1) / TILE_B;
     int gp = (n_tiles + 7) / 8, gc = gp;
     if (gp > PPO_MAX_BLOCKS) gp = gc = PPO_MAX_BLOCKS;
@@ -133,10 +154,20 @@
       }
     } else if (sp) {
       if constexpr (HAVE_SP2) {
-        (void)hipFuncSetAttribute((const void*)ppo_tower_pair_kernel<HEADP, NOP_, ND, 2>,
-                                  hipFuncAttributeMaxDynamicSharedMemorySize, (int)lds);
-        hipLaunchKernelGGL((ppo_tower_pair_kernel<HEADP, NOP_, ND, 2>), dim3(gp + gc), dim3(64 * ORL_PAIR_WAVES), lds, s, P2, C2, gp);
-        launched = true;
+        if (S != nullptr) {
+          if constexpr (ND == 0) {
+            (void)hipFuncSetAttribute((const void*)ppo_tower_pair_step_kernel<HEADP, NOP_, ND, 2>,
+                                      hipFuncAttributeMaxDynamicSharedMemorySize, (int)lds_launch);
+            hipLaunchKernelGGL((ppo_tower_pair_step_kernel<HEADP, NOP_, ND, 2>), dim3(gp + gc), dim3(64 * ORL_PAIR_WAVES), lds_launch,
+                               s, P2, C2, gp, *S);
+            launched = true;
+          }
+        } else {
+          (void)hipFuncSetAttribute((const void*)ppo_tower_pair_kernel<HEADP, NOP_, ND, 2>,
+                                    hipFuncAttributeMaxDynamicSharedMemorySize, (int)lds);
+          hipLaunchKernelGGL((ppo_tower_pair_kernel<HEADP, NOP_, ND, 2>), dim3(gp + gc), dim3(64 * ORL_PAIR_WAVES), lds, s, P2, C2, gp);
+          launched = true;
+        }
       }
     } else {
       if (P.hp.reserved & 4) {
@@ -163,7 +194,8 @@
 }
 
 template <int HEADP, int NOP_>
-static int try_launch_pair(const PpoArgs& P, const PpoArgs& Cc, int* gp_out, int* gc_out, hipStream_t s) {
+static int try_launch_pair(const PpoArgs& P, const PpoArgs& Cc, int* gp_out, int* gc_out, hipStream_t s,
+                           PendingStep* S = nullptr, bool query = false) {
 #ifdef ORL_TOWER_MAXWAVES
   return 0;
 #endif
@@ -173,7 +205,8 @@
   };
   const int nd = nd_of(P);
   if (nd != nd_of(Cc)) return 0;
-  if (nd == 0) return launch_pair_nd<HEADP, NOP_, 0>(P, Cc, gp_out, gc_out, s);
+  if (S != nullptr && nd != 0) return 0;
+  if (nd == 0) return launch_pair_nd<HEADP, NOP_, 0>(P, Cc, gp_out, gc_out, s, S, query);
   if (nd == 1) return launch_pair_nd<HEADP, NOP_, 1>(P, Cc, gp_out, gc_out, s);
   if (nd == 2) return launch_pair_nd<HEADP, NOP_, 2>(P, Cc, gp_out, gc_out, s);
   return 0;
@@ -206,9 +239,10 @@
 }
 #endif
 
-int orl_ppo_fwd_bwd(const orl_net_desc* pnet, const float* ptheta, const orl_net_desc* cnet, const float* ctheta,
-                    const float* records, int rec_width, const int64_t* idx, int mb, const float* vn_state,
-                    const orl_ppo_hparams* hp, float* partials, int* n_blocks_out, void* stream) {
+static int fwd_bwd_impl(const orl_net_desc* pnet, const float* ptheta, const orl_net_desc* cnet, const float* ctheta,
+                        const float* records, int rec_width, const int64_t* idx, int mb, const float* vn_state,
+                        const orl_ppo_hparams* hp, float* partials, int* n_blocks_out, void* stream, PendingStep* S = nullptr,
+                        bool query = false) {
   int rc = check_tower(pnet, "orl_ppo_fwd_bwd(policy)");
   if (rc) return rc;
   rc = check_tower(cnet, "orl_ppo_fwd_bwd(critic)");
@@ -239,18 +273,19 @@
     int g1 = 0, g2 = 0, pr = 0;
     const int no_ = pnet->n_out;
     if (pnet->head_kind == ORL_HEAD_CATEGORICAL) {
-      if (no_ <= 2) pr = try_launch_pair<ORL_HEAD_CATEGORICAL, 2>(P, Cc, &g1, &g2, s);
-      else if (no_ <= 8) pr = try_launch_pair<ORL_HEAD_CATEGORICAL, 8>(P, Cc, &g1, &g2, s);
-      else pr = try_launch_pair<ORL_HEAD_CATEGORICAL, 16>(P, Cc, &g1, &g2, s);
+      if (no_ <= 2) pr = try_launch_pair<ORL_HEAD_CATEGORICAL, 2>(P, Cc, &g1, &g2, s, S, query);
+      else if (no_ <= 8) pr = try_launch_pair<ORL_HEAD_CATEGORICAL, 8>(P, Cc, &g1, &g2, s, S, query);
+      else pr = try_launch_pair<ORL_HEAD_CATEGORICAL, 16>(P, Cc, &g1, &g2, s, S, query);
     } else {
-      if (no_ <= 8) pr = try_launch_pair<ORL_HEAD_GAUSSIAN, 8>(P, Cc, &g1, &g2, s);
-      else pr = try_launch_pair<ORL_HEAD_GAUSSIAN, 16>(P, Cc, &g1, &g2, s);
+      if (no_ <= 8) pr = try_launch_pair<ORL_HEAD_GAUSSIAN, 8>(P, Cc, &g1, &g2, s, S, query);
+      else pr = try_launch_pair<ORL_HEAD_GAUSSIAN, 16>(P, Cc, &g1, &g2, s, S, query);
     }
     if (pr < 0) return -(pr + 1000);
     if (pr > 0) {
       if (n_blocks_out) { n_blocks_out[0] = g1; n_blocks_out[1] = g2; }
       return 0;
     }
+    if (S != nullptr) return 1;
   }
   A.net = *pnet; A.theta = ptheta; A.o_x = 0; A.partials = partials;
   const int no = pnet->n_out;
@@ -272,4 +307,49 @@
   return 0;
 }
 
-}
+int orl_ppo_fwd_bwd(const orl_net_desc* pnet, const float* ptheta, const orl_net_desc* cnet, const float* ctheta,
+                    const float* records, int rec_width, const int64_t* idx, int mb, const float* vn_state,
+                    const orl_ppo_hparams* hp, float* partials, int* n_blocks_out, void* stream) {
+  return fwd_bwd_impl(pnet, ptheta, cnet, ctheta, records, rec_width, idx, mb, vn_state, hp, partials, n_blocks_out, stream);
+}
+
+int orl_ppo_step_foldable(const orl_net_desc* pnet, const orl_net_desc* cnet, int rec_width) {
+  if (!pnet || !cnet) return 0;
+  static const float dummy = 0.f;
+  orl_ppo_hparams hp;
+  memset(&hp, 0, sizeof(hp));
+  PendingStep S;
+  memset(&S, 0, sizeof(S));
+  const int rc = fwd_bwd_impl(pnet, &dummy, cnet, &dummy, &dummy, rec_width, nullptr, TILE_B * 8 * PPO_MAX_BLOCKS, nullptr, &hp,
+                              (float*)&dummy, nullptr, nullptr, &S, true);
+  return rc == 0 ? 1 : 0;
+}
+
+int orl_ppo_fwd_bwd_step(const orl_net_desc* pnet, const orl_net_desc* cnet, const float* records, int rec_width,
+                         const int64_t* idx, int mb, const float* vn_state, const orl_ppo_hparams* hp, float* partials,
+                         int* n_blocks_out, const float* sums, const float* step_coef, const orl_ppo_hparams* step_hp,
+                         const orl_adam_state* padam,
+                         const orl_adam_state* cadam, const orl_adam_src* psrc, const orl_adam_src* csrc,
+                         float* train_info_accum, void* stream) {
+  const char* what = "orl_ppo_fwd_bwd_step";
+  ORL_REQUIRE(pnet && cnet && sums && step_coef && step_hp && padam && cadam && psrc && csrc, "%s: null pointer", what);
+  ORL_REQUIRE(padam->theta && padam->grad && padam->m && padam->v && cadam->theta && cadam->grad && cadam->m && cadam->v &&
+              psrc->theta && psrc->m && psrc->v && csrc->theta && csrc->m && csrc->v, "%s: null optimizer buffer", what);
+  ORL_REQUIRE(padam->step >= 1 && cadam->step >= 1, "%s: Adam step counts are 1-based", what);
+  ORL_REQUIRE(padam->theta != psrc->theta && padam->m != psrc->m && padam->v != psrc->v && cadam->theta != csrc->theta &&
+              cadam->m != csrc->m && cadam->v != csrc->v, "%s: the step's source and destination buffers must differ", what);
+  PendingStep S;
+  memset(&S, 0, sizeof(S));
+  S.sums = sums; S.coef = step_coef; S.info = train_info_accum; S.hp = *step_hp;
+  S.P.net = *pnet; S.P.ad = *padam; S.P.theta_src = psrc->theta; S.P.m_src = psrc->m; S.P.v_src = psrc->v; S.P.sums_off = 0;
+  S.Cc.net = *cnet; S.Cc.ad = *cadam; S.Cc.theta_src = csrc->theta; S.Cc.m_src = csrc->m; S.Cc.v_src = csrc->v;
+  S.Cc.sums_off = RawLayout(*pnet).total + ORL_N_STATS;
+  const int rc = fwd_bwd_impl(pnet, psrc->theta, cnet, csrc->theta, records, rec_width, idx, mb, vn_state, hp, partials,
+                              n_blocks_out, stream, &S);
+  if (rc == 1)
+    return fail(ORL_E_UNSUPPORTED, "%s: these towers do not take the small-observation pair launch that carries a pending "
+                "optimiser step (orl_ppo_step_foldable)", what);
+  return rc;
+}
+
+}
diff --git a/openrl_amd/csrc/orl_ppo_tower.h b/openrl_amd/csrc/orl_ppo_tower.h
--- a/openrl_amd/csrc/orl_ppo_tower.h
+++ b/openrl_amd/csrc/orl_ppo_tower.h
@@ -1,6 +1,7 @@
 #pragma once
 #include "orl_common.h"
 #include "orl_mlp.h"
+#include "orl_adam_step.h"
 
 namespace orl {
 
@@ -134,8 +135,8 @@
   }
 }
 
-template <int HEAD, int NO, int ND, int SP_ = 0>
-__device__ __forceinline__ void ppo_tower_body(const PpoArgs& A, const int bid, const int nblk) {
+template <int HEAD, int NO, int ND, int SP_ = 0, bool STEP = false>
+__device__ __forceinline__ void ppo_tower_body(const PpoArgs& A, const int bid, const int nblk, const PendingStep* S = nullptr) {
   extern __shared__ __attribute__((aligned(16))) float smem[];
 #ifdef ORL_PROF
   const unsigned long long t_entry = __builtin_readcyclecounter();
@@ -246,7 +247,15 @@
   row_next = row_of(wave_g);
   issue_dma(RR, row_next);
   row_next = row_of(wave_g + n_waves);
-  stage_tower(smem, A.theta, tl, tw, w2t, threadIdx.x, blockDim.x, HMM, SP, true);
+  const float* th_src = A.theta;
+  if constexpr (STEP) {
+    float* th_new = smem + S->th_off;
+    float* sh16 = smem + ((rl.total + ORL_N_STATS + 3) & ~3);
+    pending_step_tower(HEAD == ORL_HEAD_VALUE ? 1 : 0, *S, smem, sh16 + 16, th_new, sh16, bid == 0);
+    __syncthreads();
+    th_src = th_new;
+  }
+  stage_tower(smem, th_src, tl, tw, w2t, threadIdx.x, blockDim.x, HMM, SP, true);
   __syncthreads();
   constexpr bool F16W = SPW && ORL_TOWER_F16;
   constexpr bool F16G = SP && ORL_TOWER_F16;
@@ -1223,6 +1232,20 @@
   else ppo_tower_body<ORL_HEAD_VALUE, 1, ND, SP>(Cc, (int)blockIdx.x - gp, (int)gridDim.x - gp);
 }
 
+template <int HEADP, int NOP_, int ND, int SP = 0>
+__global__ __launch_bounds__(64 * ORL_PAIR_WAVES, (ORL_PAIR_WAVES + 3) / 4) void ppo_tower_pair_step_kernel(PpoArgs P, PpoArgs Cc, int gp,
+                                                                                                           PendingStep S) {
+  if ((int)blockIdx.x < gp) ppo_tower_body<HEADP, NOP_, ND, SP, true>(P, (int)blockIdx.x, gp, &S);
+  else ppo_tower_body<ORL_HEAD_VALUE, 1, ND, SP, true>(Cc, (int)blockIdx.x - gp, (int)gridDim.x - gp, &S);
+}
+
+inline size_t tower_lds_end(const orl_net_desc& net, int R, int nop, int waves, bool gaussian, bool w2t, bool split,
+                            int ring_nch) {
+  const TowerLds tw(net.obs_dim, net.n_out, gaussian, w2t, nop == 16, split);
+  const int rts = net.obs_dim <= 4 ? (((R >> 2) + 3) >> 2) * 256 : ring_nch * 64;
+  return (size_t)tw.total + (size_t)waves * (2 * SLAB + 2 * rts + TILE_B * nop);
+}
+
 inline size_t tower_lds_floats(const orl_net_desc& net, int R, int nop, int waves, bool gaussian, bool w2t = true,
                                bool split = false, int ring_nch = -1) {
   const TowerLds tw(net.obs_dim, net.n_out, gaussian, w2t, nop == 16, split);
diff --git a/openrl_amd/ops.py b/openrl_amd/ops.py
--- a/openrl_amd/ops.py
+++ b/openrl_amd/ops.py
@@ -211,6 +211,46 @@
                                 nb, stream_ptr(dev))
     nat.check(rc, "orl_ppo_fwd_bwd")
     return nb[0], nb[1]
+
+
+def ppo_step_foldable(pnet, cnet, rec_width: int) -> bool:
+    return bool(_lib().orl_ppo_step_foldable(C.byref(pnet), C.byref(cnet), int(rec_width)))
+
+
+def ppo_fwd_bwd_step(pnet, cnet, records, idx, mb: int, vn_state, hp: PPOHParams, partials, sums, step_coef,
+                     step_hp: PPOHParams,
+                     padam: AdamState, cadam: AdamState, psrc: nat.AdamSrc, csrc: nat.AdamSrc, train_info_accum):
+    dev = _dev(records)
+    nb = (C.c_int * 2)(0, 0)
+    rc = _lib().orl_ppo_fwd_bwd_step(C.byref(pnet), C.byref(cnet), fptr(records), records.shape[1], ptr(idx), mb,
+                                     fptr(vn_state), C.byref(hp), fptr(partials), nb, fptr(sums), fptr(step_coef), C.byref(step_hp),
+                                     C.byref(padam), C.byref(cadam), C.byref(psrc), C.byref(csrc),
+                                     fptr(train_info_accum), stream_ptr(dev))
+    nat.check(rc, "orl_ppo_fwd_bwd_step")
+    return nb[0], nb[1]
+
+
+def ppo_reduce_pair_step(partials, nb_p: int, width_p: int, nb_c: int, width_c: int, sums, padam: AdamState,
+                         cadam: AdamState, step_coef, next_perm=None):
+    dev = _dev(sums)
+    idx, n, seed, stream_id, vn = None, 0, 0, 0, None
+    if next_perm is not None:
+        n, seed, stream_id, vn = next_perm
+        idx = torch.empty(n, dtype=torch.int64, device=dev)
+    rc = _lib().orl_ppo_reduce_pair_step(fptr(partials), nb_p, width_p, nb_c, width_c, fptr(sums), C.byref(padam),
+                                         C.byref(cadam), fptr(step_coef), ptr(idx), n, seed & (2 ** 64 - 1),
+                                         stream_id & (2 ** 64 - 1), fptr(vn[0]) if vn else None,
+                                         ptr(vn[1]) if vn else None, float(vn[2]) if vn else 0.0, stream_ptr(dev))
+    nat.check(rc, "orl_ppo_reduce_pair_step")
+    return idx
+
+
+def ppo_apply_from(pnet, cnet, sums, hp: PPOHParams, padam: AdamState, cadam: AdamState, psrc: nat.AdamSrc,
+                   csrc: nat.AdamSrc, train_info_accum) -> None:
+    dev = _dev(sums)
+    rc = _lib().orl_ppo_apply_from(C.byref(pnet), C.byref(cnet), fptr(sums), C.byref(hp), C.byref(padam), C.byref(cadam),
+                                   C.byref(psrc), C.byref(csrc), fptr(train_info_accum), stream_ptr(dev))
+    nat.check(rc, "orl_ppo_apply_from")
 
 
 def ppo_reduce(partials_ptr: int, n_blocks: int, width: int, sums_ptr: int, dev) -> None:
```

New measurement: 254.4 million. 0.988x the previous value.
